# zsc/MOSS-TTSD

Measured on AMD Instinct MI355X. Metric: audio codec tokens/sec/node (decode, bf16, batch 32 @ 4k ctx), higher is better.
Workload: dtype bf16; 1 GPU; configs[2]: batch 32 synthetic dialogues/GPU, 4k-token KV context, top-k/top-p sampling on 8 channels, decode steps at full context; batch_per_gpu=32, context=4096, prompt=512, layers=28, hidden=2048, parallelism=dp1 (batch shard, no per-step collective)

## Files before the change

### include/mtts.h

```cpp
#ifndef MTTS_H
#define MTTS_H

#include <stdint.h>

#ifdef __cplusplus
extern "C" {
#endif

#define MTTS_OK 0
#define MTTS_EINVAL (-1)
#define MTTS_EHIP (-2)
#define MTTS_ENOMEM (-3)
#define MTTS_ESTATE (-4)

#define MTTS_CHANNELS 8

typedef struct MttsConfig {
    int32_t vocab_size;
    int32_t hidden_size;
    int32_t intermediate_size;
    int32_t num_hidden_layers;
    int32_t num_attention_heads;
    int32_t num_key_value_heads;
    int32_t head_dim;
// ... 83 lines not shown
                      const MttsSamplerCfg* sampler, uint64_t seed,
                      int64_t* host_out_ids, int32_t out_capacity, int32_t* out_len,
                      const int64_t* host_forced, int32_t forced_len, int64_t* host_decisions,
                      void* stream);

int32_t mtts_begin(MttsEngine* e, const int64_t* host_input_ids, const uint8_t* host_attention_mask,
                   int32_t B, int32_t T, int32_t max_length,
                   const MttsSamplerCfg* sampler, uint64_t seed, void* stream);
int32_t mtts_step(MttsEngine* e, int32_t n_steps, void* stream);
int32_t mtts_sync_state(MttsEngine* e, int32_t* steps_done, int32_t* all_finished, void* stream);
int32_t mtts_read_generated(MttsEngine* e, int64_t* host_gen, int32_t capacity_steps, int32_t* n_steps);
int32_t mtts_step_begin(MttsEngine* e, float* dev_scores0, float* dev_scores17, void* stream);
int32_t mtts_step_sample(MttsEngine* e, int64_t* dev_tokens, void* stream);
int32_t mtts_step_finish(MttsEngine* e, const uint8_t* host_stop, void* stream);
int32_t mtts_set_output_scores(MttsEngine* e, int32_t on);
int32_t mtts_read_scores(MttsEngine* e, float* host_lp, int32_t capacity_steps, int32_t* n_steps);
int32_t mtts_slot_read_scores(MttsEngine* e, int32_t slot, float* host_rows, int32_t capacity_steps, int32_t* n_steps);
int32_t mtts_set_top_logprobs(MttsEngine* e, int32_t k);
int32_t mtts_read_top_logprobs(MttsEngine* e, float* host_logp, int32_t* host_top_ids, float* host_top_logp,
                               int32_t capacity_steps, int32_t* n_steps);
int32_t mtts_slot_read_top_logprobs(MttsEngine* e, int32_t slot, float* host_logp, int32_t* host_top_ids, float* host_top_logp,
                                    int32_t capacity_steps, int32_t* n_steps);
int32_t mtts_score(MttsEngine* e, const int64_t* host_input_ids, const uint8_t* host_attention_mask,
                   const int64_t* host_labels, int32_t B, int32_t T, float* host_logp, void* stream);
#define MTTS_SCORE_MAX_TOPK 16
#define MTTS_SCORE_TOPK_ROWS 512
int32_t mtts_score_topk(MttsEngine* e, const int64_t* host_input_ids, const uint8_t* host_attention_mask,
                        const int64_t* host_labels, int32_t B, int32_t T, float* host_logp, int32_t k,
                        int32_t* host_top_ids, float* host_top_logp, void* stream);
int32_t mtts_read_logits(MttsEngine* e, uint16_t* host_logits0, uint16_t* host_logits17, void* stream);
int32_t mtts_read_logits_f32(MttsEngine* e, float* host_logits0, float* host_logits17, void* stream);
int32_t mtts_sched_open(MttsEngine* e, int32_t B, int32_t gen_cap, const MttsSamplerCfg* sampler, void* stream);
int32_t mtts_slot_submit(MttsEngine* e, int32_t slot, const int64_t* host_ids, int32_t T, int32_t max_length, uint64_t seed,
                         void* stream);
int32_t mtts_slot_submit_row(MttsEngine* e, int32_t slot, const int64_t* host_ids, int32_t T, int32_t max_length, uint64_t seed,
                             int32_t row_id, void* stream);
int32_t mtts_set_row_ids(MttsEngine* e, const int32_t* host_row_ids, int32_t n);
int32_t mtts_set_takes(MttsEngine* e, int32_t n);
int32_t mtts_set_sampler_floors(MttsEngine* e, const MttsSamplerFloors floors[8] );
int32_t mtts_set_sampler_bans(MttsEngine* e, const MttsSamplerBans bans[8] );
int32_t mtts_set_sampler_typical(MttsEngine* e, const float typical_p[8] );
int64_t mtts_debug_ban_launches(void);
int32_t mtts_set_sampler_bias(MttsEngine* e, const MttsSamplerBias bias[8] );
int64_t mtts_debug_bias_launches(void);
int32_t mtts_slot_fork(MttsEngine* e, int32_t src_slot, int32_t dst_slot, uint64_t seed, int32_t row_id, void* stream);
int32_t mtts_slot_states(MttsEngine* e, int32_t* host_state, void* stream);
int32_t mtts_slot_read(MttsEngine* e, int32_t slot, int64_t* host_rows, int32_t capacity_steps, int32_t* n_steps);
int32_t mtts_read_seq_state(MttsEngine* e, int32_t* host_nas, int32_t* host_unfinished, int32_t* host_kv_len, void* stream);
int32_t mtts_slot_evict(MttsEngine* e, int32_t slot, void* stream);
int32_t mtts_kv_pool_state(MttsEngine* e, int32_t* total_pages, int32_t* free_pages, int32_t* max_pages_per_seq);
int32_t mtts_read_page_table(MttsEngine* e, int32_t* host_table, int32_t* host_n_pages);
int32_t mtts_set_forced_mode(MttsEngine* e, int32_t as_draw);
int32_t mtts_debug_read_device_page_table(MttsEngine* e, int32_t* host_table, void* stream);
int32_t mtts_export_codes(MttsEngine* e, int32_t first, int32_t n, int64_t* dev_codes, void* stream);
int32_t mtts_profile_enable(MttsEngine* e, int32_t on);
int32_t mtts_profile_read(MttsEngine* e, int32_t which, double* total_ms, int64_t* launches, int64_t* bytes);

int32_t mtts_debug_set_kv_len(MttsEngine* e, int32_t kv_len);
int32_t mtts_debug_kv_pack_stats(MttsEngine* e, int64_t* out6);
int32_t mtts_debug_step_plan(MttsEngine* e, int32_t pages_bound, char* buf, int32_t cap);
int32_t mtts_k_attn_bench(MttsEngine* e, int32_t phase, int32_t iters, float* avg_ms, int64_t* bytes_per_launch);
int32_t mtts_k_gemm_bench(int32_t N, int32_t K, int32_t epi, int32_t ksplit, int32_t waves, int32_t copies,
                          int32_t iters, float* avg_us);

int32_t mtts_debug_wseal_stats(MttsEngine* e, int64_t* out12);
int64_t mtts_debug_wseal_launches(void);
int32_t mtts_k_gemm_sealed_bench(const void* dev_w, int32_t N, int32_t K, int32_t epi, int32_t ksplit, int32_t copies,
                                 int32_t iters, int32_t sealed, int32_t head_form, float* avg_us, int64_t* out2);

int32_t mtts_k_wseal(const void* dev_packed, int32_t ntiles, int32_t K, int32_t ktw, void* dev_sealed, void* stream);
int32_t mtts_k_gemm_sealed(const void* dev_w, const void* dev_x, void* dev_out, int32_t M, int32_t N, int32_t K, int32_t epi,
                           int32_t ksplit, int32_t sealed, int32_t head_form, int64_t* out2, void* stream);
int32_t mtts_k_gemm_bf16(const void* dev_w, const void* dev_x, void* dev_y,
                         int32_t M, int32_t N, int32_t K, int32_t ksplit, void* stream);
int64_t mtts_debug_gemm_depth_launches(void);
int64_t mtts_debug_fold_norm_launches(void);
int32_t mtts_k_oproj_resid(const void* dev_wo, const void* dev_attn, void* dev_x, void* dev_x_packed, int32_t R, int32_t N,
                           void* stream);
int32_t mtts_k_fold_pair(const void* dev_wo, const void* dev_attn, void* dev_x, const void* dev_norm_w, const void* dev_wgu,
                         float eps, int32_t R, int32_t N_gu, void* dev_y, void* stream);
int32_t mtts_k_bf16_round_check(int64_t* out2, void* stream);
int32_t mtts_k_fold_bench(int32_t N_gu, int32_t copies, int32_t iters, int32_t mode, float* avg_us);
int64_t mtts_debug_attn_row_launches(void);
int32_t mtts_k_attn_section(const float* dev_slabs, int32_t ksplit, const void* dev_qnw, const void* dev_knw, const void* dev_cos,
                            const void* dev_sin, float eps, const void* dev_k, const void* dev_v, const int32_t* host_lens,
                            const int32_t* host_page_table, int32_t R, int32_t Lmax, int32_t nq, int32_t nkv, int32_t sealed,
                            int32_t path, void* dev_out, void* dev_kcache, void* dev_vcache, void* dev_kpack, void* dev_vpack,
                            void* stream);
int32_t mtts_k_attn_prefill(const float* dev_slabs, int32_t ksplit, const void* dev_qnw, const void* dev_knw, const void* dev_cos,
                            const void* dev_sin, float eps, const void* dev_k, const void* dev_v, const int32_t* host_lens,
                            const int32_t* host_cached, const int32_t* host_page_table, int32_t B, int32_t Lmax, int32_t nq,
                            int32_t nkv, void* dev_out, void* dev_q, void* dev_kcache, void* dev_vcache, void* stream);
int32_t mtts_k_gemm_swiglu_bf16(const void* dev_w, const void* dev_x, void* dev_y,
                                int32_t M, int32_t N, int32_t K, void* stream);
int32_t mtts_k_rmsnorm(const void* dev_x, const void* dev_w, void* dev_y,
                       int32_t rows, int32_t n, float eps, void* stream);
int32_t mtts_k_embed_norm(const int32_t* host_tokens, const int32_t* host_seq, const void* const* host_tables,
                          const int32_t* host_vocab, const void* dev_norm_w, int32_t R, int32_t H, float eps,
                          void* dev_x, void* dev_xn, void* stream);
int32_t mtts_k_resid_norm(const float* dev_slabs, int32_t ksplit, int32_t Npad, void* dev_x, const void* dev_norm_w,
                          const int32_t* host_seq, const int32_t* host_last, int32_t R, int32_t H, int32_t nseq, float eps,
                          void* dev_xn, void* dev_hlast, void* stream);
int32_t mtts_k_gemv_small(int32_t epi, int32_t pro, const void* dev_w, int32_t rows, int32_t N, int32_t K, int32_t want_ksplit,
                          const void* dev_x_in, const float* dev_slabs, int32_t slab_ksplit, const void* dev_norm_w, float eps,
                          void* dev_x_out, const float* dev_opart, const int32_t* host_seq, const int32_t* host_pos, int32_t nq,
                          int32_t nchunks_max, const void* dev_xrows, void* dev_y, int32_t* out_plan, void* stream);
int32_t mtts_k_gemm_tile(int32_t epi, const void* dev_w, const void* dev_x, void* dev_y, int32_t M, int32_t N, int32_t K,
                         int32_t ksplit, void* stream);
int32_t mtts_k_rope_kvwrite(const void* dev_qkv, const int32_t* host_pos, const void* dev_qnorm, const void* dev_knorm,
                            const void* dev_cos, const void* dev_sin, int32_t R, int32_t nq, int32_t nkv, float eps,
                            void* dev_q, void* dev_k, void* dev_v, void* stream);
int32_t mtts_k_paged_attn_decode(const void* dev_q, const void* dev_k, const void* dev_v, const int32_t* host_lens,
                                 const int32_t* host_page_table, int32_t R, int32_t Lmax, int32_t nq, int32_t nkv,
                                 void* dev_out, void* stream);
int32_t mtts_k_kv_seal(const void* dev_pages, int32_t npages, void* dev_sealed, int32_t as_k, void* stream);
int32_t mtts_k_head_ce(const void* dev_w, const void* dev_x, const int32_t* host_labels, int32_t M, int32_t N, int32_t K,
                       int32_t n_valid, int32_t segments, float* dev_logp, void* stream);
int32_t mtts_k_head_topk(const void* dev_w, const void* dev_x, int32_t M, int32_t N, int32_t K, int32_t n_valid,
                         int32_t segments, int32_t k, int32_t* dev_ids, float* dev_logp, void* stream);
int32_t mtts_k_lora_pack(const void* dev_base, int32_t rows, int32_t cols, const float* dev_lora_a, const float* dev_lora_b,
                         int32_t r, float scaling, int32_t rows_pad, int32_t row_mul, int32_t row_off, int32_t dtype,
                         void* dev_out, void* stream);
int32_t mtts_k_lora_delta(const void* dev_x, int32_t R, int32_t K, int32_t Npad, int32_t nseg, const int32_t* host_segs,
                          int32_t n_adapters, const void* const* host_a, const void* const* host_b, const int32_t* host_r,
                          const float* host_scaling, const int32_t* host_row_adapter, float* dev_slabs, int32_t ks, void* stream);
int32_t mtts_k_swiglu_slabs(const void* dev_w, const void* dev_x, const float* dev_delta, void* dev_y, float* dev_slab0_out,
                            int32_t M, int32_t N, int32_t K, void* stream);
int32_t mtts_k_sample(const void* dev_logits_bf16, int32_t rows, int32_t vocab,
                      const void* dev_history_bitmap, const MttsSamplerCfg* cfg,
                      int32_t mask_id, uint64_t seed, int32_t step, int32_t channel,
                      int32_t* dev_tokens, void* stream);
int32_t mtts_k_sample_scores(const void* dev_logits_bf16, int32_t rows, int32_t vocab,
                             const void* dev_history_bitmap, const MttsSamplerCfg* cfg,
                             int32_t mask_id, uint64_t seed, int32_t step, int32_t channel,
                             int32_t* dev_tokens, float* dev_logp, void* stream);
int32_t mtts_k_sample_floors(const void* dev_logits_bf16, int32_t rows, int32_t vocab,
                             const void* dev_history_bitmap, const MttsSamplerCfg* cfg,
                             int32_t mask_id, uint64_t seed, int32_t step, int32_t channel,
                             int32_t* dev_tokens, float* dev_logp, const MttsSamplerFloors* floors, void* stream);
int32_t mtts_k_sample_bans(const void* dev_logits_bf16, int32_t rows, int32_t vocab,
                           const void* dev_history_bitmap, const MttsSamplerCfg* cfg,
                           int32_t mask_id, uint64_t seed, int32_t step, int32_t channel,
                           int32_t* dev_tokens, float* dev_logp, const MttsSamplerFloors* floors, const void* dev_ban,
                           void* stream);
int32_t mtts_k_sample_typical(const void* dev_logits_bf16, int32_t rows, int32_t vocab,
                              const void* dev_history_bitmap, const MttsSamplerCfg* cfg,
                              int32_t mask_id, uint64_t seed, int32_t step, int32_t channel,
                              int32_t* dev_tokens, float* dev_logp, const MttsSamplerFloors* floors, const void* dev_ban,
                              float typical_p, void* stream);
int32_t mtts_k_ngram_ban(const int32_t* dev_hist, const int32_t* dev_lens, int32_t rows, int32_t cap, int32_t n,
                         const int32_t* host_static, int32_t n_static, int32_t vocab, int32_t eos_id, int32_t eos_on,
                         void* dev_ban, void* stream);
int32_t mtts_k_seq_bias(const int32_t* dev_hist, const int32_t* dev_lens, int32_t rows, int32_t cap,
                        const MttsSamplerBias* host_rules, int32_t vocab, void* dev_ban, void* dev_bias_words,
                        MttsBiasTable* dev_bias_tab, void* stream);
int32_t mtts_k_sample_bias(const void* dev_logits_bf16, int32_t rows, int32_t vocab,
                           const void* dev_history_bitmap, const MttsSamplerCfg* cfg,
                           int32_t mask_id, uint64_t seed, int32_t step, int32_t channel,
                           int32_t* dev_tokens, float* dev_logp, const MttsSamplerFloors* floors, const void* dev_ban,
                           float typical_p, const void* dev_bias_words, const MttsBiasTable* dev_bias_tab, void* stream);
int32_t mtts_k_scores_materialize(const void* dev_logits_bf16, int32_t rows, int32_t vocab, const void* dev_history_bitmap,
                                  const MttsSamplerCfg* cfg, int32_t mask_id, int32_t step, int32_t channel, const void* dev_ban,
                                  const void* dev_bias_words, const MttsBiasTable* dev_bias_tab, float* dev_scores, void* stream);
int32_t mtts_k_gen_topk(const void* dev_logits, int32_t is_f32, int32_t rows, int32_t vocab, int32_t mask_id,
                        const int32_t* dev_decisions, int32_t k, float* dev_logp, int32_t* dev_top_ids, float* dev_top_logp,
                        void* stream);

typedef struct MttsCodecConfig {
    int32_t nq, codebook_size, rvq_dim, quant_out_dim;
    int32_t adapter_layers, adapter_dim, adapter_heads, adapter_ffn, adapter_max_pos;
    int32_t up_stride;
    int32_t dec_layers, dec_dim, dec_heads, dec_ffn, dec_max_pos, mel_bins;
    int32_t voc_dim, voc_inter, voc_layers, n_fft, hop;
    int32_t mel_n_fft, mel_hop, mel_frames;
    int32_t enc_layers, enc_dim, enc_heads, enc_ffn, enc_max_pos;
    int32_t sem_adapter_layers, pre_rvq_layers, down_pool;
} MttsCodecConfig;

typedef struct MttsCodec MttsCodec;
const char* mtts_codec_last_error(void);
int32_t mtts_codec_create(const MttsCodecConfig* cfg, int32_t device, MttsCodec** out);
int32_t mtts_codec_destroy(MttsCodec* c);
int32_t mtts_codec_bind(MttsCodec* c, const char* role, const float* dev_f32, int64_t n, void* stream);
int32_t mtts_codec_detokenize(MttsCodec* c, const int64_t* dev_codes, const int32_t* host_lens, int32_t B, int32_t T,
                              float* dev_wav, void* stream);
int32_t mtts_codec_detokenize_async(MttsCodec* c, const int64_t* dev_codes, const int32_t* host_lens, int32_t B, int32_t T,
                                    float* dev_wav, void* stream);
int32_t mtts_codec_check(MttsCodec* c, void* stream);
int32_t mtts_codec_tokenize(MttsCodec* c, const float* dev_wav, const int32_t* host_lens, int32_t B, int32_t nsamp,
                            int64_t* dev_codes, int32_t* host_code_lens, void* stream);
int32_t mtts_k_gemm_f32(const float* dev_a, const float* dev_w, const float* dev_bias, float* dev_c,
                        int32_t M, int32_t N, int32_t K, int32_t act, void* stream);
int32_t mtts_k_gemm_planes_bench(int32_t M, int32_t N, int32_t K, int32_t flags, int32_t tile_code, int32_t iters,
                                 float* avg_us, int32_t* code_used);

int32_t mtts_k_codec_attn(const float* dev_qkv, const int32_t* host_lens, float* dev_att, int32_t B, int32_t T, int32_t heads,
                          int32_t mode, int32_t planes, void* stream);
int32_t mtts_k_codec_gemm_planes(const float* dev_a, const float* dev_w, const float* dev_bias, const float* dev_gamma,
                                 const float* dev_res, float* dev_c, int32_t M, int32_t N, int32_t K, int32_t ldc, int32_t flags,
                                 int32_t tile, int32_t row0, int32_t plane_rows, int32_t nt_out, void* stream);
int32_t mtts_k_codec_vocos_pw(const float* dev_xn, const float* dev_w1, const float* dev_b1, const float* dev_w2,
                              const float* dev_b2, const float* dev_gamma, float* dev_h, int32_t M, void* stream);
int32_t mtts_k_codec_layernorm(const float* dev_x, const float* dev_w, const float* dev_b, float* dev_y, int32_t rows, int32_t C,
                               float eps, const int32_t* host_lens, int32_t T, int32_t ldy, int32_t planes, void* stream);
int32_t mtts_k_codec_layernorm_wide(const float* dev_x, const float* dev_w, const float* dev_b, float* dev_y, int32_t rows,
                                    int32_t C, float eps, void* stream);
int32_t mtts_k_codec_dwconv_ln(const float* dev_h, const float* dev_dw, const float* dev_dwb, const float* dev_lw,
                               const float* dev_lb, float* dev_y, int32_t B, int32_t T, int32_t C, float eps, int32_t kernel,
                               int32_t planes, void* stream);
int32_t mtts_k_codec_softmax_mask(float* dev_s, const int32_t* host_lens, int32_t B, int32_t heads, int32_t T, int32_t ldT,
                                  void* stream);
int32_t mtts_k_codec_vq_argmin_update(const float* dev_dot, const float* dev_cb, const float* dev_cc, float* dev_residual,
                                      int64_t* dev_codes, const int32_t* host_lens, int32_t B, int32_t T, int32_t K, int32_t D,
                                      void* stream);
int32_t mtts_k_codec_gemm_f32_ex(const float* dev_a, const float* dev_w, float* dev_c, const float* dev_bias,
                                 const float* dev_gamma, const float* dev_res, int32_t M, int32_t N, int32_t K, int32_t b_kn,
                                 int64_t lda, int64_t ldw, int64_t ldc, int64_t ldres, int32_t res_rows, int32_t act, float scale,
                                 int32_t batch, int32_t batch_inner, const int64_t* host_strides, void* stream);
// ... 6 lines not shown
```

### moss-ttsd_amd/csrc/attn.hip

```cpp
#include "launch.h"
#include <algorithm>
#include <atomic>
#include <cstdlib>
#ifndef MTTS_PK_WAVES
#define MTTS_PK_WAVES 0
#endif
#if MTTS_PK_WAVES
#define PK_OCC(PK) __attribute__((amdgpu_waves_per_eu((PK) ? MTTS_PK_WAVES : 1, (PK) ? MTTS_PK_WAVES : 8)))
#else
#define PK_OCC(PK)
#endif

#include "seal.h"

__device__ bool seal_lane_k(const u32x4_t* __restrict__ raw, u32x4_t* __restrict__ pk, uint8_t* __restrict__ lds, int lane) {
    u32x4_t v[16];
#pragma unroll
    for (int j = 0; j < 16; ++j) v[j] = raw[j * 64];
    __builtin_amdgcn_wave_barrier();
    uint32_t* row = (uint32_t*)(lds + lane * 128);
#pragma unroll
    for (int j = 0; j < 16; ++j)
#pragma unroll
        for (int c = 0; c < 4; c += 2) {
// ... 60 lines not shown
                cnt += e ? 1u : 0u;
            }
            row[2 * it + h] = sum | (cnt << 16);
        }
    __builtin_amdgcn_wave_barrier();
    int mean;
    {
        const int t = lane, st = (t >> 1) & 1, j = 2 * (t >> 2) + (t & 1);
        uint32_t tot = 0u, cn = 0u;
        for (int d = 0; d < 32; ++d) {
            const uint32_t w = ((const uint32_t*)(lds + (st * 32 + d) * 128))[j];
            tot += w & 0xffffu;
            cn += w >> 16;
        }
        mean = cn ? (int)((tot + cn / 2) / cn) : 0;
    }
    int* means = (int*)(lds + 8192);
    int8_t* sv = (int8_t*)(lds + 8192 + 256);
    means[lane] = mean;
    __builtin_amdgcn_wave_barrier();
    int ref = 255;
    for (int t = 0; t < 64; ++t) { const int m = means[t]; if (m > 0) ref = min(ref, m); }
    const int s_own = mean > 0 ? min((mean - ref) & ~1, 126) : 0;
    sv[lane] = (int8_t)s_own;
    __builtin_amdgcn_wave_barrier();
    bool unfit = false;
#pragma unroll
    for (int it = 0; it < 16; ++it) {
        const int s0 = sv[4 * it + 2 * sub], s1 = sv[4 * it + 2 * sub + 1];
        uint32_t w[4] = {v[it].x, v[it].y, v[it].z, v[it].w};
#pragma unroll
        for (int c = 0; c < 4; ++c) {
            uint32_t out = 0u;
#pragma unroll
            for (int h = 0; h < 2; ++h) {
                uint32_t b = (w[c] >> (16 * h)) & 0xffffu;
                const int sft = h ? s1 : s0;
                const int e = (int)((b >> 7) & 0xffu);
                if (e == 0) {
                    if ((b & 0x7fu) && sft) unfit = true;
                } else {
                    const int e2 = e - sft;
                    if (e == 255 ? sft != 0 : e2 < 1) unfit = true;
                    else b = (b - ((uint32_t)sft << 7)) & 0xffffu;
                }
                out |= b << (16 * h);
            }
            w[c] = out;
        }
        v[it] = u32x4_t{w[0], w[1], w[2], w[3]};
    }
    return seal_encode(v, pk, (uint32_t)s_own & 0xffu, unfit);
}
__device__ __forceinline__ void seal_count(bool fit, unsigned long long* __restrict__ cnt, int layer, int wave, int lane) {
    const bool all = !__any(!fit);
    if (cnt && lane == 0) atomicAdd(cnt + layer * 4 + wave * 2 + (all ? 0 : 1), 1ull);
}

__global__ __launch_bounds__(128) void kv_seal_scan_kernel(const u32x4_t* __restrict__ kcache, const u32x4_t* __restrict__ vcache,
                                                           u32x4_t* __restrict__ kpack, u32x4_t* __restrict__ vpack,
                                                           const int32_t* __restrict__ page_table, const RowMeta* __restrict__ meta, int R,
                                                           int max_pages, int total_pages, size_t raw_layer, size_t pk_layer,
                                                           unsigned long long* __restrict__ cnt) {
    __shared__ __attribute__((aligned(16))) uint8_t klds[8192 + 128];
    __shared__ __attribute__((aligned(16))) uint8_t vlds[8192 + 320];
    const int kvh = blockIdx.y, layer = blockIdx.z, wave = threadIdx.x >> 6, lane = threadIdx.x & 63;
    const int r = blockIdx.x * 64 + lane;
    RowMeta m{-1, 0, 0, 0};
    if (r < R) m = meta[r];
    unsigned long long todo = __ballot(m.seq >= 0 && (m.pos & 63) == 63);
    while (todo) {
        const int i = __ffsll((long long)todo) - 1;
        todo &= todo - 1;
        const int seq = __shfl(m.seq, i, 64), pos = __shfl(m.pos, i, 64);
        const int page = page_table[(size_t)seq * max_pages + (pos >> 6)];
        const size_t pi = (size_t)kvh * total_pages + page;
        const bool fit = wave ? seal_lane_v(vcache + layer * raw_layer + pi * (MTTS_PAGE * MTTS_HD / 8) + lane,
                                            vpack + layer * pk_layer + pi * (MTTS_PKU * 64) + lane, vlds, lane)
                              : seal_lane_k(kcache + layer * raw_layer + pi * (MTTS_PAGE * MTTS_HD / 8) + lane,
                                            kpack + layer * pk_layer + pi * (MTTS_PKU * 64) + lane, klds, lane);
        seal_count(fit, cnt, layer, wave, lane);
    }
}
__global__ __launch_bounds__(128) void kv_seal_all_kernel(const u32x4_t* __restrict__ kcache, const u32x4_t* __restrict__ vcache,
                                                          u32x4_t* __restrict__ kpack, u32x4_t* __restrict__ vpack, int total_pages,
                                                          size_t raw_layer, size_t pk_layer, unsigned long long* __restrict__ cnt) {
    __shared__ __attribute__((aligned(16))) uint8_t klds[8192 + 128];
    __shared__ __attribute__((aligned(16))) uint8_t vlds[8192 + 320];
    const int kvh = blockIdx.y, layer = blockIdx.z, wave = threadIdx.x >> 6, lane = threadIdx.x & 63;
    const size_t pi = (size_t)kvh * total_pages + blockIdx.x;
    const bool fit = wave ? seal_lane_v(vcache + layer * raw_layer + pi * (MTTS_PAGE * MTTS_HD / 8) + lane,
                                        vpack + layer * pk_layer + pi * (MTTS_PKU * 64) + lane, vlds, lane)
                          : seal_lane_k(kcache + layer * raw_layer + pi * (MTTS_PAGE * MTTS_HD / 8) + lane,
                                        kpack + layer * pk_layer + pi * (MTTS_PKU * 64) + lane, klds, lane);
    seal_count(fit, cnt, layer, wave, lane);
}
__global__ __launch_bounds__(64) void kv_seal_pages_kernel(const u32x4_t* __restrict__ raw, u32x4_t* __restrict__ pk, int as_k) {
    __shared__ __attribute__((aligned(16))) uint8_t klds[8192 + 320];
    const u32x4_t* src = raw + (size_t)blockIdx.x * (MTTS_PAGE * MTTS_HD / 8) + threadIdx.x;
    u32x4_t* dst = pk + (size_t)blockIdx.x * (MTTS_PKU * 64) + threadIdx.x;
    if (as_k == 1) seal_lane_k(src, dst, klds, threadIdx.x);
    else if (as_k == 2) seal_lane_v(src, dst, klds, threadIdx.x);
    else seal_lane(src, dst);
}
void launch_kv_seal_pages(const void* raw, void* pk, int npages, int as_k, hipStream_t st) {
    hipLaunchKernelGGL(kv_seal_pages_kernel, dim3(npages), dim3(64), 0, st, (const u32x4_t*)raw, (u32x4_t*)pk, as_k);
}
__global__ __launch_bounds__(64) void kv_pack_count_kernel(const u32x4_t* __restrict__ kpack, const u32x4_t* __restrict__ vpack,
                                                           const int32_t* __restrict__ page_table, const int32_t* __restrict__ complete,
                                                           int max_pages, int total_pages, size_t pk_layer, unsigned long long* __restrict__ out) {
    const int b = blockIdx.x, kvh = blockIdx.y, layer = blockIdx.z, lane = threadIdx.x;
    unsigned long long n = 0, dk = 0, dv = 0;
    for (int pg = 0; pg < complete[b]; ++pg) {
        const size_t pi = (size_t)kvh * total_pages + page_table[(size_t)b * max_pages + pg];
        const u32x4_t fk = kpack[layer * pk_layer + pi * (MTTS_PKU * 64) + 12 * 64 + lane];
        const u32x4_t fv = vpack[layer * pk_layer + pi * (MTTS_PKU * 64) + 12 * 64 + lane];
        n += 1;
        dk += __any(fk.w != 0u) ? 1 : 0;
        dv += __any(fv.w != 0u) ? 1 : 0;
    }
    if (lane == 0 && n) {
        atomicAdd(out + 0, n); atomicAdd(out + 1, dk); atomicAdd(out + 2, n); atomicAdd(out + 3, dv);
    }
}
void launch_kv_pack_count(const void* kpack, const void* vpack, const int32_t* page_table, const int32_t* complete, int B, int max_pages,
                          int total_pages, int nkv, int L, unsigned long long* out, hipStream_t st) {
    const size_t pk_layer = (size_t)total_pages * nkv * (MTTS_PKU * 64);
    hipLaunchKernelGGL(kv_pack_count_kernel, dim3(B, nkv, L), dim3(64), 0, st, (const u32x4_t*)kpack, (const u32x4_t*)vpack, page_table,
                       complete, max_pages, total_pages, pk_layer, out);
}
void launch_kv_seal_rows(const void* kcache, const void* vcache, void* kpack, void* vpack, const int32_t* page_table,
                         const RowMeta* meta, int R, int max_pages, int total_pages, int nkv, int L, unsigned long long* cnt, hipStream_t st) {
    const size_t raw_layer = (size_t)total_pages * nkv * (MTTS_PAGE * MTTS_HD / 8), pk_layer = (size_t)total_pages * nkv * (MTTS_PKU * 64);
    hipLaunchKernelGGL(kv_seal_scan_kernel, dim3((R + 63) / 64, nkv, L), dim3(128), 0, st, (const u32x4_t*)kcache, (const u32x4_t*)vcache,
                       (u32x4_t*)kpack, (u32x4_t*)vpack, page_table, meta, R, max_pages, total_pages, raw_layer, pk_layer, cnt);
}
void launch_kv_seal_all(const void* kcache, const void* vcache, void* kpack, void* vpack, int total_pages, int nkv, int L,
                        unsigned long long* cnt, hipStream_t st) {
    const size_t raw_layer = (size_t)total_pages * nkv * (MTTS_PAGE * MTTS_HD / 8), pk_layer = (size_t)total_pages * nkv * (MTTS_PKU * 64);
    hipLaunchKernelGGL(kv_seal_all_kernel, dim3(total_pages, nkv, L), dim3(128), 0, st, (const u32x4_t*)kcache, (const u32x4_t*)vcache,
                       (u32x4_t*)kpack, (u32x4_t*)vpack, total_pages, raw_layer, pk_layer, cnt);
}


__device__ __forceinline__ void fuse_reduce(const QkvFuse& f, int r, int col, int lane, float& a, float& b) {
    const size_t kstride = (size_t)MTTS_PFCAP * f.Npad;
    const float* p0 = f.partial + (size_t)r * f.Npad + col + lane;
    a = 0.f; b = 0.f;
    for (int k0 = 0; k0 < f.ksplit; k0 += 8) {
        float ta[8], tb[8];
#pragma unroll
        for (int j = 0; j < 8; ++j) {
            const float* pk = p0 + (size_t)min(k0 + j, f.ksplit - 1) * kstride;
            ta[j] = pk[0];
            tb[j] = pk[64];
        }
        if (k0 == 0) { a = ta[0]; b = tb[0]; }
#pragma unroll
        for (int j = 0; j < 8; ++j)
            if (k0 + j < f.ksplit && k0 + j > 0) { a += ta[j]; b += tb[j]; }
    }
    a = rbf(a);
    b = rbf(b);
}

__device__ __forceinline__ void fuse_reduce_request(const QkvFuse& f, int r, int col, int lane, float (&ta)[8], float (&tb)[8]) {
    const size_t kstride = (size_t)MTTS_PFCAP * f.Npad;
    const float* p0 = f.partial + (size_t)r * f.Npad + col + lane;
#pragma unroll
    for (int j = 0; j < 8; ++j) {
        const float* pk = p0 + (size_t)min(j, f.ksplit - 1) * kstride;
        ta[j] = pk[0];
        tb[j] = pk[64];
    }
}
__device__ __forceinline__ void fuse_reduce_sum(const QkvFuse& f, const float (&ta)[8], const float (&tb)[8], float& a, float& b) {
    a = ta[0]; b = tb[0];
#pragma unroll
    for (int j = 1; j < 8; ++j)
        if (j < f.ksplit) { a += ta[j]; b += tb[j]; }
    a = rbf(a);
    b = rbf(b);
}

struct FuseVec { float w0, w1, c, s; };
__device__ __forceinline__ FuseVec fuse_load_vec(const QkvFuse& f, const uint16_t* __restrict__ nw, int pos, int lane) {
    FuseVec v;
    v.w0 = bf2f(nw[lane]);
    v.w1 = bf2f(nw[lane + 64]);
    v.c = bf2f(f.rope_cos[(size_t)pos * 64 + lane]);
    v.s = bf2f(f.rope_sin[(size_t)pos * 64 + lane]);
    return v;
}
__device__ __forceinline__ void fuse_norm_rope(const QkvFuse& f, const FuseVec& v, float a, float b, float& o1, float& o2) {
    const float ss = wave_sum(a * a + b * b);
    const float inv = 1.0f / sqrtf(ss / (float)MTTS_HD + f.eps);
    a = rbf(v.w0 * rbf(a * inv));
    b = rbf(v.w1 * rbf(b * inv));
    o1 = rbf(rbf(a * v.c) + rbf(-b * v.s));
    o2 = rbf(rbf(b * v.c) + rbf(a * v.s));
}

template <int G, bool FUSED, bool PK>
__global__ __launch_bounds__(256) PK_OCC(PK) void attn_scores_kernel(
    const uint16_t* __restrict__ qbuf, u32x4_t* __restrict__ kcache, const int32_t* __restrict__ page_table,
    const RowMeta* __restrict__ meta, uint16_t* __restrict__ scores, float* __restrict__ stats, int max_pages,
    int total_pages, int nq, int nkv, float scale, QkvFuse f, const u32x4_t* __restrict__ kpack) {
    __shared__ __attribute__((aligned(16))) uint32_t qs[G][MTTS_HD / 2];
    __shared__ __attribute__((aligned(16))) uint16_t knew[MTTS_HD];
    __shared__ __attribute__((aligned(16))) uint32_t qw[PK ? 4 : 1][G][MTTS_HD / 2];
    const int r = blockIdx.z, kvh = blockIdx.y;
    const RowMeta m = meta[r];
    if (m.seq < 0) return;
    const int len = m.pos + 1;
    const int npages = (len + MTTS_PAGE - 1) / MTTS_PAGE;
    if ((int)blockIdx.x * 4 >= npages) return;
    const int wave = __builtin_amdgcn_readfirstlane(threadIdx.x >> 6), lane = threadIdx.x & 63;
    const int pg = blockIdx.x * 4 + wave;
// ... 999 lines not shown
```

### moss-ttsd_amd/csrc/engine.h

```cpp
#pragma once
#include <hip/hip_runtime.h>

#include <algorithm>
#include <cstdarg>
#include <cstdio>
#include <cstdlib>
#include <cstring>
#include <memory>
#include <string>
#include <vector>

#include "launch.h"
#include "runstate.h"
#include "stepplan.h"

static_assert(RUN_EINVAL == MTTS_EINVAL, "runstate.h reports with MTTS_EINVAL");

#define MTTS_LOCAL __attribute__((visibility("hidden")))
extern MTTS_LOCAL thread_local char g_err[512];
#define HIPCHK(x)                                                                          \
    do {                                                                                   \
        hipError_t _e = (x);                                                               \
        if (_e != hipSuccess) return fail(MTTS_EHIP, "%s: %s (%s:%d)", #x, hipGetErrorString(_e), __FILE__, __LINE__); \
    } while (0)
// ... 131 lines not shown
    int h16 = 0;
    struct LayerF32 { float *wqkv = nullptr, *wo = nullptr, *wgu = nullptr, *wd = nullptr, *ln_in = nullptr, *ln_post = nullptr, *qn = nullptr, *kn = nullptr; };
    std::vector<LayerF32> lf;
    float* embf[8] = {nullptr};
    const float** d_tables_f = nullptr;
    float* final_norm_f = nullptr;
    float *kcache_f = nullptr, *vcache_f = nullptr;
    float *xf = nullptr, *xnf = nullptr, *qkvf = nullptr, *qbuf_f = nullptr, *attnf = nullptr, *yf = nullptr, *guf = nullptr,
          *actf = nullptr, *hlast_f = nullptr, *scores_f = nullptr;
    SeqState* d_seqs = nullptr;
    RowMeta* d_meta = nullptr;
    LoopState* d_ls = nullptr;
    LoopState* h_ls = nullptr;
    SeqState* h_seqs = nullptr;
    int32_t *d_decisions = nullptr, *d_cur = nullptr, *d_tf = nullptr;
    uint32_t* d_bitmaps = nullptr;
    int bm_words = 0;
    MttsSamplerCfg* d_scfg = nullptr;
    MttsSamplerFloors* d_floors = nullptr;
    int floors_on = 0;
    float* d_typical = nullptr;
    int typical_on = 0;
    BanCfg* d_bancfg = nullptr;
    int bans_on = 0;
    int ban_ngram_on = 0;
    int ban_begin_on = 0;
    int bias_on = 0, bias_terms = 0;
    int hist_on = 0;
    SampleScratch sscr;
    int ch0_sampled = 0;
    int scores_on = 0;
    bool run_open = false;
    int topk_on = 0;
    int32_t* d_sc_labels = nullptr;
    float* d_sc_logp = nullptr;
    size_t sc_cap_rows = 0;
    float* sc_part = nullptr;
    float* sc_logits = nullptr;
    int32_t* d_sc_top_ids = nullptr;
    float* d_sc_top_logp = nullptr;
    size_t sc_top_cap = 0;
    uint32_t* sc_cand = nullptr;
    std::vector<LoraEnt> bank;
    int bank_pairs[MTTS_MAX_ADAPTERS] = {0};
    std::vector<int32_t> seq_adapter = std::vector<int32_t>(MTTS_RCAP, -1);
    int32_t* d_pf_tokens = nullptr;
    RowMeta* d_pf_meta = nullptr;
    size_t pf_cap_rows = 0;
    int B = 0, T = 0, base_length = 0, max_length = 0, max_steps = 0, steps_issued = 0;
    bool continuous = false;
    std::vector<int> join_step;
    std::vector<int> n_real;
    int max_real = 0;
    uint64_t seed = 0;
    bool began = false, has_forced = false;
    int split_phase = 0;
    float *split_scores0 = nullptr, *split_scores17 = nullptr;
    struct DestroyExec { void operator()(hipGraphExec_t g) const { hipGraphExecDestroy(g); } };
    StepGraphs<hipGraphExec_t, DestroyExec> graphs;
    hipStream_t cap_stream = nullptr;
    void *kpack = nullptr, *vpack = nullptr;
    size_t pk_layer_stride = 0;
    unsigned long long *d_seal_cnt = nullptr, *h_seal_cnt = nullptr;
    std::vector<char> pack_k_on, pack_v_on;
    bool prof = false;
    std::vector<std::pair<hipEvent_t, hipEvent_t>> ev[PROF_N];
    int64_t prof_bytes[PROF_N] = {0, 0, 0, 0, 0};
};

static inline bool rows_carry_adapters(const MttsEngine* e) {
    for (int b = 0; b < e->B; ++b)
        if (e->seq_adapter[b] >= 0) return true;
    return false;
}
static inline StepState step_state(const MttsEngine* e, int heads, int R, int pages_bound, bool lora, bool split = false) {
    StepState s;
    s.heads = heads; s.B = e->B; s.R = R; s.pages_bound = pages_bound; s.lora = lora;
    s.forced = e->has_forced; s.ch0_sampled = e->ch0_sampled != 0; s.scores_on = e->scores_on != 0; s.floors_on = e->floors_on != 0; s.typical_on = e->typical_on != 0;
    s.bans_on = e->bans_on != 0; s.bias_on = e->bias_on != 0; s.bias_terms = e->bias_terms != 0;
    s.topk = e->topk_on; s.split = split;
    for (int k = 0; k < WSEAL_KINDS; ++k) s.wseal_on[k] = e->wseal_on[k] != 0;
    if (e->kpack) s.pack_k_on = e->pack_k_on.data();
    if (e->vpack) s.pack_v_on = e->pack_v_on.data();
    return s;
}
static inline StepPlan decode_plan(const MttsEngine* e, int pages_bound, bool split = false) {
    return plan_step(e->knobs, e->caps, step_state(e, 1, round_up(e->B, 32), pages_bound, rows_carry_adapters(e), split));
}

static inline KvPack layer_pack(const MttsEngine* e, const StepPlan& plan, int n) {
    const LayerPlan& l = plan.layers[n];
    return KvPack{l.k_sealed ? (uint8_t*)e->kpack + e->pk_layer_stride * n : nullptr,
                  l.v_sealed ? (uint8_t*)e->vpack + e->pk_layer_stride * n : nullptr};
}
```

### moss-ttsd_amd/csrc/engine.hip

```cpp
#include "engine.h"
#include "staging.h"

#define FLUSH_STEPS 7
#define LINGER_STEPS 14
static inline int linger_bound(int B) { return 6 * B + 8; }

thread_local char g_err[512] = "";
int fail(int code, const char* fmt, ...) {
    va_list ap;
    va_start(ap, fmt);
    vsnprintf(g_err, sizeof(g_err), fmt, ap);
    va_end(ap);
    return code;
}

const char* mtts_last_error(void) { return g_err; }
int32_t mtts_version(void) { return 202; }

static auto ship_on(MttsEngine* e, hipStream_t st) {
    return [e, st](const PageEdits& ed) -> int {
        launch_set_pages(e->d_page_table, ed, st);
        HIPCHK(hipGetLastError());
        return 0;
    };
}

static int create_f32(MttsEngine* e) {
    const size_t H = e->H, I = e->I, D = MTTS_HD;
    e->lf.resize(e->L);
    for (auto& l : e->lf) {
        TRY(e->mem.get(&l.wqkv, (size_t)e->qkv_rows * H, false));
        TRY(e->mem.get(&l.wo, H * e->nq * D, false));
        TRY(e->mem.get(&l.wgu, 2 * I * H, false));
        TRY(e->mem.get(&l.wd, H * I, false));
        TRY(e->mem.get(&l.ln_in, H)); TRY(e->mem.get(&l.ln_post, H)); TRY(e->mem.get(&l.qn, D)); TRY(e->mem.get(&l.kn, D));
    }
    TRY(e->mem.get(&e->embf[0], (size_t)e->V0 * H, false));
    for (int ch = 1; ch < 8; ++ch) TRY(e->mem.get(&e->embf[ch], (size_t)e->Vs * H, false));
    TRY(e->mem.get(&e->final_norm_f, H));
    TRY(e->mem.get(&e->d_tables_f, 8));
    HIPCHK(hipMemcpy((void*)e->d_tables_f, e->embf, 8 * sizeof(void*), hipMemcpyHostToDevice));
    const size_t P = MTTS_PF32CAP;
    TRY(e->mem.get(&e->xf, P * H)); TRY(e->mem.get(&e->xnf, P * H)); TRY(e->mem.get(&e->yf, P * H));
    TRY(e->mem.get(&e->qkvf, P * e->qkv_rows)); TRY(e->mem.get(&e->qbuf_f, P * e->nq * D)); TRY(e->mem.get(&e->attnf, P * e->nq * D));
    TRY(e->mem.get(&e->guf, P * 2 * I)); TRY(e->mem.get(&e->actf, P * I));
    TRY(e->mem.get(&e->hlast_f, (size_t)MTTS_RCAP * H));
    TRY(e->mem.get((float**)&e->logits0, (size_t)MTTS_RCAP * e->V0_pad));
    TRY(e->mem.get((float**)&e->logits17, (size_t)MTTS_RCAP * 7 * e->Vs_pad));
    return 0;
}

static int forward_rows_f32(MttsEngine* e, const int32_t* d_tokens, const RowMeta* d_meta, int R, int heads, hipStream_t st) {
    const int H = e->H, I = e->I, nq = e->nq, nkv = e->nkv;
    const float eps = e->cfg.rms_norm_eps, scale = 1.0f / sqrtf((float)MTTS_HD);
    const int Lmax = e->max_pages * MTTS_PAGE, h16 = e->h16;
    const bool dec = heads == 1;
    launch_f32_embed_norm(d_tokens, d_meta, e->d_tables_f, e->lf[0].ln_in, e->xf, e->xnf, R, H, eps, h16, st);
    for (int n = 0; n < e->L; ++n) {
        auto& l = e->lf[n];
        float* kc = e->kcache_f + e->layer_stride * n;
        float* vc = e->vcache_f + e->layer_stride * n;
        launch_f32_linear(l.wqkv, e->xnf, e->qkvf, R, e->qkv_rows, H, e->qkv_rows, h16, dec, st);
        launch_f32_qkv_post(e->qkvf, e->qkv_rows, d_meta, l.qn, l.kn, e->bufs.rope_cos_f, e->bufs.rope_sin_f, e->qbuf_f, kc, vc,
                            e->d_page_table, e->max_pages, e->total_pages, R, nq, nkv, eps, h16, st);
        launch_f32_attn(e->qbuf_f, kc, vc, e->d_page_table, d_meta, e->scores_f, e->attnf, R, e->max_pages, e->total_pages, nq,
                        nkv, scale, Lmax, h16, st);
        launch_f32_linear(l.wo, e->attnf, e->yf, R, H, nq * MTTS_HD, H, h16, dec, st);
        launch_f32_resid_norm(e->yf, e->xf, l.ln_post, e->xnf, nullptr, d_meta, R, H, eps, h16, st);
        launch_f32_linear(l.wgu, e->xnf, e->guf, R, 2 * I, H, 2 * I, h16, dec, st);
        launch_f32_swiglu(e->guf, e->actf, R, I, h16, st);
        launch_f32_linear(l.wd, e->actf, e->yf, R, H, I, H, h16, dec, st);
        const bool lastl = n == e->L - 1;
        launch_f32_resid_norm(e->yf, e->xf, lastl ? e->final_norm_f : e->lf[n + 1].ln_in, e->xnf, lastl ? e->hlast_f : nullptr,
                              d_meta, R, H, eps, h16, st);
    }
    if (heads) {
        const float* xin = heads == 1 ? e->xnf : e->hlast_f;
        launch_f32_linear(e->embf[0], xin, (float*)e->logits0, e->B, e->V0, H, e->V0_pad, h16, true, st);
        for (int c = 1; c < 8; ++c)
            launch_f32_linear(e->embf[c], xin, (float*)e->logits17 + (size_t)(c - 1) * e->Vs_pad, e->B, e->Vs, H, 7 * e->Vs_pad, h16, true, st);
    }
    HIPCHK(hipGetLastError());
    return MTTS_OK;
// ... 473 lines not shown
    HIPCHK(hipGetLastError());
    HIPCHK(hipMemcpyAsync(e->h_wseal_cnt, e->d_wseal_cnt, WSEAL_KINDS * 2 * sizeof(unsigned long long), hipMemcpyDeviceToHost, nullptr));
    HIPCHK(hipStreamSynchronize(nullptr));
    for (int k = 0; k < WSEAL_KINDS; ++k) {
        const unsigned long long groups = e->h_wseal_cnt[2 * k], bad = e->h_wseal_cnt[2 * k + 1];
        e->wseal_on[k] = e->wseal_ktw[k] && groups && (e->knobs.w_seal == 2 || (double)bad <= WSEAL_MAX_UNSEALED[k] * (double)groups);
    }
    e->wseal_dirty = false;
    return MTTS_OK;
}

int32_t mtts_weights_ready(MttsEngine* e) {
    if (!e) return fail(MTTS_EINVAL, "null engine");
    if (e->emb_bound != 0xff) return fail(MTTS_ESTATE, "embedding tables missing (mask %x)", e->emb_bound);
    if (!e->norm_bound) return fail(MTTS_ESTATE, "final norm missing");
    if (!e->bufs.rope_rows) return fail(MTTS_ESTATE, "rope table missing");
    for (int n = 0; n < e->L; ++n)
        if (e->layers[n].bound != 2047) return fail(MTTS_ESTATE, "layer %d incomplete (mask %x)", n, e->layers[n].bound);
    return wseal_policy(e);
}

static void prof_begin(MttsEngine* e, int which, hipStream_t st, hipEvent_t* a) {
    if (!e->prof) return;
    hipEvent_t s0, s1;
    hipEventCreate(&s0); hipEventCreate(&s1);
    hipEventRecord(s0, st);
    e->ev[which].push_back({s0, s1});
    *a = s1;
}
static void prof_end(MttsEngine* e, hipStream_t st, hipEvent_t a) {
    if (!e->prof) return;
    hipEventRecord(a, st);
}

static int pack_policy_reset(MttsEngine* e, hipStream_t st) {
    if (!e->d_seal_cnt) return 0;
    HIPCHK(hipMemsetAsync(e->d_seal_cnt, 0, (size_t)e->L * 4 * sizeof(unsigned long long), st));
    e->pack_k_on.assign(e->L, 1);
    e->pack_v_on.assign(e->L, 1);
    return 0;
}
static int attend_layer(MttsEngine* e, const StepPlan& plan, int n, const RowMeta* d_meta, int R, int pages_bound, int ks_qkv,
                        hipStream_t st, int64_t kv_tokens_hint) {
    static const AttnPhase decode_ph[3] = {ATTN_SCORES, ATTN_PV, ATTN_COMBINE}, prefill_ph[3] = {ATTN_PF_SCORES, ATTN_PF_PV, ATTN_PF_COMBINE};
    Layer& l = e->layers[n];
    const AttnForm form = plan.layers[n].attn;
    const float eps = e->cfg.rms_norm_eps, scale = 1.0f / sqrtf((float)MTTS_HD);
    uint16_t* kc = (uint16_t*)e->kcache + e->layer_stride * n;
    uint16_t* vc = (uint16_t*)e->vcache + e->layer_stride * n;
    const QkvFuse fz{e->bufs.partial, ks_qkv, e->qkv_rows, (const uint16_t*)l.qn, (const uint16_t*)l.kn, e->bufs.rope_cos, e->bufs.rope_sin, eps};
    const KvPack pk = layer_pack(e, plan, n);
    const KvPack* pkp = (pk.k || pk.v) ? &pk : nullptr;
    if (form == ATTN_FORM_ROW) {
        hipEvent_t ev = nullptr;
        prof_begin(e, PROF_SCORES, st, &ev);
        if (const int rc = launch_attn(e->qbuf, kc, vc, e->d_page_table, d_meta, e->scores, e->stats, e->opart, e->attn_p, R, pages_bound,
                                       e->max_pages, e->total_pages, e->nchunks_max, e->nq, e->nkv, scale, &fz, ATTN_ROW, st, pkp))
            return fail(MTTS_EINVAL, rc == -2 ? "the whole-row attention kernel does not take this launch" : "attention group size not built");
        prof_end(e, st, ev);
        if (e->prof) e->prof_bytes[PROF_SCORES] += 2 * kv_tokens_hint * e->nkv * MTTS_HD * 2;
        return 0;
    }
    const bool fused = form == ATTN_FORM_TWO_PASS_FUSED;
    const AttnPhase* ph = form == ATTN_FORM_PREFILL_MFMA ? prefill_ph : decode_ph;
    const int nphases = plan.path == PATH_SMALL ? 2 : 3;
    if (!fused)
        launch_qkv_post(e->bufs.partial, ks_qkv, e->qkv_rows, d_meta, l.qn, l.kn, e->bufs.rope_cos, e->bufs.rope_sin, e->qbuf,
                        kc, vc, e->d_page_table, e->max_pages, e->total_pages, R, e->nq, e->nkv, eps, st);
    for (int i = 0; i < nphases; ++i) {
        hipEvent_t ev = nullptr;
        if (i < 2) prof_begin(e, i == 0 ? PROF_SCORES : PROF_PV, st, &ev);
        if (launch_attn(e->qbuf, kc, vc, e->d_page_table, d_meta, e->scores, e->stats, e->opart, e->attn_p, R,
                        pages_bound, e->max_pages, e->total_pages, e->nchunks_max, e->nq, e->nkv, scale,
                        fused ? &fz : nullptr, ph[i], st, pkp))
            return fail(MTTS_EINVAL, "attention group size not built");
        if (i < 2) prof_end(e, st, ev);
    }
    if (e->prof) {
        e->prof_bytes[PROF_SCORES] += kv_tokens_hint * e->nkv * MTTS_HD * 2;
        e->prof_bytes[PROF_PV] += kv_tokens_hint * e->nkv * MTTS_HD * 2;
    }
    return 0;
}
static void seal_completed_pages(MttsEngine* e, const RowMeta* d_meta, int R, hipStream_t st) {
    if (e->kpack)
        launch_kv_seal_rows(e->kcache, e->vcache, e->kpack, e->vpack, e->d_page_table, d_meta, R, e->max_pages, e->total_pages, e->nkv, e->L, e->d_seal_cnt, st);
}

static int forward_small(MttsEngine* e, const StepPlan& plan, const RowMeta* d_meta, int pages_bound, hipStream_t st, int64_t kv_tokens_hint) {
    const int H = e->H, I = e->I, nq = e->nq, Hp = round_up(H, 32), R = MTTS_MAXR;
    const float eps = e->cfg.rms_norm_eps;
    uint16_t* xa = (uint16_t*)e->x;
    uint16_t* xb = (uint16_t*)e->x2;
    SmallPro base{};
    base.rows = plan.B; base.eps = eps; base.slab_npad = Hp;
    for (int n = 0; n < e->L; ++n) {
        Layer& l = e->layers[n];
        SmallPro pq = base;
        pq.x_in = xa; pq.x_out = xb; pq.slabs = e->partial2; pq.ksplit = n ? e->p_d.ksplit : 0; pq.norm_w = (const uint16_t*)l.ln_in;
        launch_gemv_small(EPI_PARTIAL, PRO_NORM, e->p_qkv, l.wqkv, H, e->qkv_rows, e->qkv_rows, e->bufs.partial, nullptr, pq, st);
        TRY(attend_layer(e, plan, n, d_meta, R, pages_bound, e->p_qkv.ksplit, st, kv_tokens_hint));
        SmallPro po = base;
        po.opart = e->opart; po.meta = d_meta; po.nchunks_max = e->nchunks_max; po.nq = nq; po.pages_per_chunk = ATT_PB;
        launch_gemv_small(EPI_PARTIAL, PRO_COMBINE, e->p_o, l.wo, nq * MTTS_HD, Hp, Hp, e->partial2, nullptr, po, st);
        SmallPro pg = base;
        pg.x_in = xb; pg.x_out = xa; pg.slabs = e->partial2; pg.ksplit = e->p_o.ksplit; pg.norm_w = (const uint16_t*)l.ln_post;
        launch_gemv_small(EPI_SILU_RM, PRO_NORM, e->p_gu, l.wgu, H, 2 * I, 2 * I, nullptr, (uint16_t*)e->act_rm, pg, st);
        SmallPro pd = base;
        pd.xrows = (const uint16_t*)e->act_rm;
        launch_gemv_small(EPI_PARTIAL, PRO_ROWS, e->p_d, l.wd, I, Hp, Hp, e->partial2, nullptr, pd, st);
    }
    seal_completed_pages(e, d_meta, R, st);
    SmallPro ph = base;
    ph.x_in = xa; ph.x_out = nullptr; ph.slabs = e->partial2; ph.ksplit = e->p_d.ksplit; ph.norm_w = (const uint16_t*)e->final_norm;
    launch_gemv_small(EPI_BF16, PRO_NORM, e->p_h0, e->head0, H, e->V0_pad, e->V0, nullptr, (uint16_t*)e->logits0, ph, st);
    launch_gemv_small(EPI_BF16, PRO_NORM, e->p_h17, e->heads17, H, 7 * e->Vs_pad, 7 * e->Vs_pad, nullptr, (uint16_t*)e->logits17, ph, st);
    HIPCHK(hipGetLastError());
    return MTTS_OK;
}

static int run_gemm(int epi, bool tiled, int R, int ks, bool sealed, int head_form, const GemmPlan& p, const void* Ws, const void* Wp,
                    const void* Xp, int K, int Npad, int n_valid, float* partial, uint16_t* out, hipStream_t st) {
    const int mb = (R + 31) / 32;
    if (tiled) launch_gemm_tile(epi, R, ks, Wp, Xp, K, Npad, n_valid, partial, out, st);
    else if (!sealed) launch_gemm(epi, mb, p, Wp, Xp, K, Npad, n_valid, partial, out, st);
    else if (!launch_gemm_sealed(epi, mb, p, Ws, Wp, Xp, K, Npad, n_valid, partial, out, head_form, st))
        return fail(MTTS_ESTATE, "the plan asks for a sealed weight read that the launcher does not take (K %d, N %d, %d row tiles)", K, Npad, mb);
    return 0;
}

static int forward_rows(MttsEngine* e, const StepPlan& plan, const int32_t* d_tokens, const RowMeta* d_meta, int pages_bound,
                        hipStream_t st, int64_t kv_tokens_hint) {
    const int H = e->H, I = e->I, nq = e->nq, nkv = e->nkv, R = plan.R, mb = plan.mb;
    const float eps = e->cfg.rms_norm_eps;
    const int Hp = round_up(H, 32);
    const bool tiled = plan.tiled, lora = plan.lora;
    if (plan.path == PATH_F32) return forward_rows_f32(e, d_tokens, d_meta, plan.heads == 1 ? plan.B : R, plan.heads, st);
    launch_embed_norm(d_tokens, d_meta, e->d_tables, e->layers[0].ln_in, e->x, e->xn, R, H, eps, st);
    if (plan.path == PATH_SMALL) return forward_small(e, plan, d_meta, pages_bound, st, kv_tokens_hint);
    if (lora && !e->bufs.d_bank) return fail(MTTS_ESTATE, "a pass with adapters on an engine without a bank");
    const int QD = nq * MTTS_HD, KD = nkv * MTTS_HD, EL = e->L * 7;
    const LoraJob j_qkv{3, e->qkv_rows, H, EL, {{0, QD, 1, 0}, {QD, KD, 1, 1}, {QD + KD, KD, 1, 2}}};
    const LoraJob j_o{1, Hp, QD, EL, {{0, H, 1, 3}}}, j_gu{2, 2 * I, H, EL, {{0, I, 2, 4}, {1, I, 2, 5}}}, j_d{1, Hp, I, EL, {{0, H, 1, 6}}};
    const int ks_qkv = tiled ? mtts_tile_ksplit(e->qkv_rows, H, 1024) : e->p_qkv.ksplit;
    const int ks_o = tiled ? mtts_tile_ksplit(Hp, QD, 1024) : e->p_o.ksplit;
    const int ks_d = tiled ? mtts_tile_ksplit(Hp, I, 1024) : e->p_d.ksplit;
    const int ex = lora ? 1 : 0;
    const int gu_epi = lora ? EPI_PARTIAL : EPI_SILU;
    float* gu_slab = lora ? e->bufs.partial : nullptr;
    for (int n = 0; n < e->L; ++n) {
        Layer& l = e->layers[n];
        auto delta = [&](const LoraJob& job, const void* xp, int ks) {
            launch_lora_delta(xp, d_meta, e->bufs.d_seq_adapter, e->bufs.d_bank + (size_t)n * 7, job, e->bufs.partial + (size_t)ks * MTTS_PFCAP * job.Npad, R, st);
        };
        TRY(run_gemm(EPI_PARTIAL, tiled, R, ks_qkv, false, 0, e->p_qkv, nullptr, l.wqkv, e->xn, H, e->qkv_rows, e->qkv_rows, e->bufs.partial, nullptr, st));
        if (lora) delta(j_qkv, e->xn, ks_qkv);
        TRY(attend_layer(e, plan, n, d_meta, R, pages_bound, ks_qkv + ex, st, kv_tokens_hint));
        if (plan.fold) {
            launch_oproj_resid(l.wo, e->attn_p, e->x, e->xres_p, R, Hp, st);
            launch_gateup_norm(l.wgu, e->xres_p, l.ln_post, eps, e->act_p, 2 * I, st);
        } else {
            TRY(run_gemm(EPI_PARTIAL, tiled, R, ks_o, false, 0, e->p_o, nullptr, l.wo, e->attn_p, QD, Hp, Hp, e->bufs.partial, nullptr, st));
            if (lora) delta(j_o, e->attn_p, ks_o);
            launch_resid_norm(e->bufs.partial, ks_o + ex, Hp, e->x, l.ln_post, e->xn, nullptr, d_meta, R, H, eps, st);
            TRY(run_gemm(gu_epi, tiled, R, 1, plan.sealed[WSEAL_GU], 0, e->p_gu, l.wgu_s, l.wgu, e->xn, H, 2 * I, 2 * I, gu_slab, (uint16_t*)e->act_p, st));
        }
        if (lora) {
            delta(j_gu, e->xn, 1);
            launch_swiglu_slabs(e->bufs.partial, e->bufs.partial + (size_t)MTTS_PFCAP * 2 * I, e->act_p, mb * 32, I, st);
        }
        TRY(run_gemm(EPI_PARTIAL, tiled, R, ks_d, plan.sealed[WSEAL_DOWN], 0, e->p_d, l.wd_s, l.wd, e->act_p, I, Hp, Hp, e->bufs.partial, nullptr, st));
        if (lora) delta(j_d, e->act_p, ks_d);
        const bool lastl = (n == e->L - 1);
        const void* nw = lastl ? e->final_norm : e->layers[n + 1].ln_in;
        launch_resid_norm(e->bufs.partial, ks_d + ex, Hp, e->x, nw, e->xn, lastl ? e->hlast : nullptr, d_meta, R, H, eps, st);
    }
    seal_completed_pages(e, d_meta, R, st);
    if (plan.heads) {
        const void* xin = e->xn;
        if (plan.heads == 2) {
            launch_pack_rows(e->hlast, e->xh, plan.B, H, plan.hmb, st);
            xin = e->xh;
        }
        const int hr = plan.hmb * 32, form = plan.head_persistent ? 1 : 0;
        TRY(run_gemm(EPI_BF16, false, hr, 0, plan.sealed[WSEAL_HEAD0], form, e->p_h0, e->head0_s, e->head0, xin, H, e->V0_pad, e->V0, nullptr, (uint16_t*)e->logits0, st));
        TRY(run_gemm(EPI_BF16, false, hr, 0, plan.sealed[WSEAL_HEADS], form, e->p_h17, e->heads17_s, e->heads17, xin, H, 7 * e->Vs_pad, 7 * e->Vs_pad, nullptr, (uint16_t*)e->logits17, st));
    }
    HIPCHK(hipGetLastError());
    return MTTS_OK;
}
static int forward_staged(MttsEngine* e, const int32_t* d_tokens, const RowMeta* d_meta, int R, int pages_bound, int heads, bool lora, hipStream_t st) {
    return forward_rows(e, plan_step(e->knobs, e->caps, step_state(e, heads, R, pages_bound, lora)), d_tokens, d_meta, pages_bound, st, 0);
}

static int prefill_staged(MttsEngine* e, size_t Mpad, int pages_bound, int last_heads, bool lora, hipStream_t st) {
    const size_t pfcap = e->f32 ? MTTS_PF32CAP : MTTS_PFCAP;
    for (size_t off = 0; off < Mpad; off += pfcap) {
        const int rows = (int)std::min<size_t>(pfcap, Mpad - off);
        TRY(forward_staged(e, e->d_pf_tokens + off * 8, e->d_pf_meta + off, rows, pages_bound, off + rows >= Mpad ? last_heads : 0, lora, st));
    }
    return 0;
}

static int start_outputs(MttsEngine* e, int steps, hipStream_t st) {
    StepBufs& b = e->bufs;
    DevBufs& m = e->mem;
    const int k = e->topk_on, rows = e->cfg.max_batch;
    const bool scores = e->scores_on != 0, grown = steps > b.gen_cap, restrided = k && k != b.gt_stride;
    if (grown) b.gen_cap = steps;
    if (restrided) b.gt_stride = k;
    if (scores && !b.sscr_lp) {
        TRY(m.get(&b.sscr_slice_sum, (size_t)rows * SAMP_NS));
        TRY(m.get(&b.sscr_lp, (size_t)rows * 8));
    }
    if (k > b.gt_scr_cap) {
        m.release(b.gt_cand); m.release(b.gt_smax); m.release(b.gt_ssum);
        b.gt_scr_cap = 0;
        TRY(m.get(&b.gt_cand, (size_t)rows * SAMP_NS * k));
        TRY(m.get(&b.gt_smax, (size_t)rows * SAMP_NS));
        TRY(m.get(&b.gt_ssum, (size_t)rows * SAMP_NS));
        b.gt_scr_cap = k;
    }
    const auto store = [&](auto*& p, bool per_k, bool wanted, bool zeroed, bool filled) -> int {
        const size_t n = (size_t)rows * b.gen_cap * 8 * (per_k ? k : 1);
        if (grown || (per_k && restrided)) m.release(p);
        if (wanted && !p) TRY(m.get(&p, n, zeroed));
        if (wanted && filled) HIPCHK(hipMemsetAsync(p, 0xff, n * sizeof(*p), st));
        return 0;
    };
    TRY(store(b.d_gen, false, true, true, false));
    TRY(store(b.d_declog, false, true, true, false));
    TRY(store(b.d_forced, false, true, false, false));
    TRY(store(b.d_lp, false, scores, false, true));
    TRY(store(b.d_gt_logp, false, k > 0, false, true));
    TRY(store(b.d_gt_ids, true, k > 0, false, true));
    TRY(store(b.d_gt_tlp, true, k > 0, false, true));
    return 0;
}

static int start_bans(MttsEngine* e, const RunBans& bans, const RunBias& bias, hipStream_t st) {
    StepBufs& b = e->bufs;
    e->bans_on = (bans.any() || bias.bans()) ? 1 : 0;
    e->ban_ngram_on = bans.ngram() ? 1 : 0;
    e->ban_begin_on = bias.begin() ? 1 : 0;
    e->bias_on = bias.rules() ? 1 : 0;
    e->bias_terms = bias.finite() ? 1 : 0;
    e->hist_on = (e->ban_ngram_on || bias.history()) ? 1 : 0;
    if (!e->bans_on && !e->bias_on) return 0;
    const int rows = e->cfg.max_batch, words = e->bm_words;
    if (e->bans_on && !b.d_ban) {
        TRY(e->mem.get(&b.d_ban, (size_t)rows * 8 * words));
        TRY(e->mem.get(&b.d_ban_static, (size_t)8 * words));
    }
    if (e->ban_begin_on && !b.d_ban_begin) TRY(e->mem.get(&b.d_ban_begin, (size_t)8 * words));
    if (e->bias_on && !b.d_bias_rules) TRY(e->mem.get(&b.d_bias_rules, 8));
    if (e->bias_terms && !b.d_bias_w) {
        TRY(e->mem.get(&b.d_bias_w, (size_t)rows * 8 * words));
        TRY(e->mem.get(&b.d_bias_static, (size_t)8 * words));
        TRY(e->mem.get(&b.d_bias_tab, (size_t)rows * 8));
    }
// ... 212 lines not shown
        TRY(reset_run_state(e, ss, false, sampler, opt.floors, opt.typical, st));
    }
    TRY(prefill_staged(e, sr.Mpad, pages_for(e->max_real), 2, lora, st));
    if (fork.nr) TRY(launch_fork_job(e, fork, false, st));
    e->began = true;
    e->run_open = true;
    return MTTS_OK;
}

int32_t mtts_set_takes(MttsEngine* e, int32_t n) {
    if (!e) return fail(MTTS_EINVAL, "null engine");
    if (n < 1 || n > MTTS_RCAP) return fail(MTTS_EINVAL, "takes must be 1..%d (got %d)", MTTS_RCAP, n);
    e->pending.set_takes(n);
    return MTTS_OK;
}
int32_t mtts_set_sampler_floors(MttsEngine* e, const MttsSamplerFloors* floors) {
    if (!e) return fail(MTTS_EINVAL, "null engine");
    return e->pending.set_floors(floors);
}
int32_t mtts_set_sampler_typical(MttsEngine* e, const float* typical_p) {
    if (!e) return fail(MTTS_EINVAL, "null engine");
    return e->pending.set_typical(typical_p);
}
int32_t mtts_set_sampler_bans(MttsEngine* e, const MttsSamplerBans* bans) {
    if (!e) return fail(MTTS_EINVAL, "null engine");
    return e->pending.set_bans(bans);
}
int32_t mtts_set_sampler_bias(MttsEngine* e, const MttsSamplerBias* bias) {
    if (!e) return fail(MTTS_EINVAL, "null engine");
    return e->pending.set_bias(bias);
}
static int take_options(MttsEngine* e, int B, bool forced, RunOptions* opt) {
    *opt = e->pending.take(B);
    return opt->check(e->cfg.max_batch, forced);
}

int32_t mtts_begin(MttsEngine* e, const int64_t* ids, const uint8_t* mask, int32_t B, int32_t T, int32_t max_length,
                   const MttsSamplerCfg* sampler, uint64_t seed, void* stream) {
    if (!e) return fail(MTTS_EINVAL, "null argument");
    RunOptions opt;
    TRY(take_options(e, B, false, &opt));
    return begin_run(e, ids, mask, B, T, max_length, sampler, seed, opt, stream);
}

static SampleScratch step_front(MttsEngine* e, const StepPlan& plan, hipStream_t st) {
    const StepBufs& b = e->bufs;
    SampleScratch sscr = e->sscr;
    sscr.slice_sum = b.sscr_slice_sum; sscr.lp = b.sscr_lp;
    if (plan.bans_on) {
        launch_ban(b.d_ban, b.d_ban_static, b.d_ban_begin, b.ban_words, e->d_bancfg, b.d_hist, b.hist_cap, b.d_gen, e->V0, e->Vs, e->cfg.eos_token_id,
                   e->d_ls, e->d_seqs, plan.B, st);
        sscr.ban = b.d_ban;
    }
    if (plan.bias_on) {
        launch_bias(plan.bans_on ? b.d_ban : nullptr, plan.bias_terms ? b.d_bias_w : nullptr, b.d_bias_static, plan.bias_terms ? b.d_bias_tab : nullptr,
                    b.ban_words, b.d_bias_rules, b.d_hist, b.hist_cap, b.d_gen, e->V0, e->Vs, e->d_ls, e->d_seqs, plan.B, st);
        if (plan.bias_terms) { sscr.bias_w = b.d_bias_w; sscr.bias_t = b.d_bias_tab; }
    }
    return sscr;
}
static void step_decide(MttsEngine* e, const StepPlan& plan, const SampleScratch& sscr, const void* l0, const void* l17, hipStream_t st) {
    const StepBufs& b = e->bufs;
    launch_sample(l0, l17, e->V0, e->Vs, e->Vs_pad, e->d_bitmaps, e->bm_words, e->d_scfg, e->d_ls,
                  e->d_seqs, e->seed, e->d_decisions, &e->d_ls->error, plan.B, sscr, plan.ch0_sampled,
                  full_cap_for(e->V0), plan.scores_on, (plan.floors_on || plan.typical_on) ? e->d_floors : nullptr,
                  plan.typical_on ? e->d_typical : nullptr, st);
    GenTopkOut gt;
    if (plan.topk) {
        gt = GenTopkOut{plan.topk, b.d_gt_logp, b.d_gt_ids, b.d_gt_tlp};
        launch_gen_topk(e->logits0, e->logits17, e->V0, e->Vs, e->Vs_pad, e->d_scfg, e->d_ls, e->d_seqs, e->d_decisions, plan.B,
                        GenTopkScratch{b.gt_cand, b.gt_smax, b.gt_ssum, b.gt_scr_cap}, gt, st);
    }
    launch_update(e->d_decisions, b.d_declog, plan.forced ? b.d_forced : nullptr, e->d_tf, b.d_gen, e->d_cur,
                  e->d_seqs, e->d_meta, e->d_bitmaps, e->bm_words, e->d_ls, e->cfg.eos_token_id,
                  e->cfg.speech_pad_token, e->cfg.speech_range_lo, e->cfg.speech_range_hi,
                  plan.scores_on ? b.sscr_lp : nullptr, plan.scores_on ? b.d_lp : nullptr, gt, st);
}
static int step_body(MttsEngine* e, const StepPlan& plan, int pages_bound, hipStream_t st, int64_t kvtok) {
    const SampleScratch sscr = step_front(e, plan, st);
    step_decide(e, plan, sscr, e->logits0, e->logits17, st);
    return forward_rows(e, plan, e->d_cur, e->d_meta, pages_bound, st, kvtok);
}

static int step_graph(MttsEngine* e, int pages, hipGraphExec_t* out) {
    StepPlan plan = decode_plan(e, pages);
    if (const hipGraphExec_t* hit = e->graphs.find(plan, pages, e->bufs)) {
        *out = *hit;
        return MTTS_OK;
    }
    if (!e->cap_stream) HIPCHK(hipStreamCreateWithFlags(&e->cap_stream, hipStreamNonBlocking));
    hipGraph_t g = nullptr;
    HIPCHK(hipStreamBeginCapture(e->cap_stream, hipStreamCaptureModeRelaxed));
    int rc = step_body(e, plan, pages, e->cap_stream, 0);
    hipError_t ce = hipStreamEndCapture(e->cap_stream, &g);
    if (rc) { if (g) hipGraphDestroy(g); return rc; }
    HIPCHK(ce);
    hipGraphExec_t exec = nullptr;
    hipError_t ie = hipGraphInstantiate(&exec, g, nullptr, nullptr, 0);
    hipGraphDestroy(g);
    HIPCHK(ie);
    e->graphs.insert(std::move(plan), pages, e->bufs, exec);
    *out = exec;
    return MTTS_OK;
}

static int step_pages(MttsEngine* e, hipStream_t st, int* pages_bound) {
    int len_bound = 1;
    const auto ship = ship_on(e, st);
    for (int b = 0; b < e->B; ++b) {
        if (!e->slot_live[b]) continue;
        const int len = e->n_real[b] + e->steps_issued + 1;
        len_bound = std::max(len_bound, len);
        TRY(e->pool.grow(b, pages_for(len), ship));
    }
    TRY(e->pool.flush(ship));
    *pages_bound = pages_for(len_bound);
    return MTTS_OK;
}

static int issue_steps(MttsEngine* e, int n, hipStream_t st) {
    for (int i = 0; i < n; ++i) {
        if (e->steps_issued >= e->max_steps) break;
        int pages_bound = 0;
        TRY(step_pages(e, st, &pages_bound));
        if (e->knobs.use_graphs && !e->prof) {
            hipGraphExec_t exec = nullptr;
            TRY(step_graph(e, std::min(round_up(pages_bound, ATT_PB), e->max_pages), &exec));
            HIPCHK(hipGraphLaunch(exec, st));
        } else {
            hipEvent_t ev = nullptr;
            prof_begin(e, PROF_STEP, st, &ev);
            int64_t kvtok = 0;
            for (int b = 0; b < e->B; ++b) if (e->slot_live[b]) kvtok += e->n_real[b] + e->steps_issued + 1;
            TRY(step_body(e, decode_plan(e, pages_bound), pages_bound, st, kvtok));
            prof_end(e, st, ev);
        }
        e->steps_issued++;
    }
    return MTTS_OK;
}

int32_t mtts_step(MttsEngine* e, int32_t n_steps, void* stream) {
    if (!e || !e->began) return fail(MTTS_ESTATE, "mtts_begin has not run");
    if (e->split_phase) return fail(MTTS_ESTATE, "mtts_step in the middle of a split step: mtts_step_finish first");
    HIPCHK(hipSetDevice(e->device));
    return issue_steps(e, n_steps, S(stream));
}

static int split_check(MttsEngine* e, const char* who) {
    if (!e || !e->began) return fail(MTTS_ESTATE, "%s: mtts_begin has not run", who);
    if (e->continuous) return fail(MTTS_ESTATE, "%s: the scheduler's steps are not split (mtts_sched_open is running)", who);
    return MTTS_OK;
}
int32_t mtts_step_begin(MttsEngine* e, float* dev_scores0, float* dev_scores17, void* stream) {
    TRY(split_check(e, "mtts_step_begin"));
    if (e->split_phase) return fail(MTTS_ESTATE, "mtts_step_begin: a split step is in flight, mtts_step_finish first");
    if (!dev_scores0 || !dev_scores17 || ((uintptr_t)dev_scores0 & 15) || ((uintptr_t)dev_scores17 & 15))
        return fail(MTTS_EINVAL, "mtts_step_begin: the score buffers are null or not 16-byte aligned");
    if (e->steps_issued >= e->max_steps) return fail(MTTS_ESTATE, "mtts_step_begin: the run has no step left (%d issued)", e->steps_issued);
    HIPCHK(hipSetDevice(e->device));
    hipStream_t st = S(stream);
    const StepPlan plan = decode_plan(e, 1, true);
    const SampleScratch sscr = step_front(e, plan, st);
    launch_scores_materialize(e->logits0, e->logits17, e->V0, e->Vs, e->Vs_pad, e->d_bitmaps, e->bm_words, e->d_scfg, e->d_ls, e->d_seqs,
                              plan.B, sscr, dev_scores0, dev_scores17, st);
    HIPCHK(hipGetLastError());
    e->split_scores0 = dev_scores0; e->split_scores17 = dev_scores17;
    e->split_phase = 1;
    return MTTS_OK;
}
int32_t mtts_step_sample(MttsEngine* e, int64_t* dev_tokens, void* stream) {
    TRY(split_check(e, "mtts_step_sample"));
    if (e->split_phase != 1) return fail(MTTS_ESTATE, "mtts_step_sample: mtts_step_begin has not run for this step");
    HIPCHK(hipSetDevice(e->device));
    hipStream_t st = S(stream);
    const StepPlan plan = decode_plan(e, 1, true);
    SampleScratch sscr = e->sscr;
    sscr.slice_sum = e->bufs.sscr_slice_sum; sscr.lp = e->bufs.sscr_lp;
    sscr.ext = 1;
    step_decide(e, plan, sscr, e->split_scores0, e->split_scores17, st);
    if (dev_tokens) launch_step_tokens(e->d_cur, dev_tokens, e->d_ls, st);
    HIPCHK(hipGetLastError());
    e->split_phase = 2;
    return MTTS_OK;
}
int32_t mtts_step_finish(MttsEngine* e, const uint8_t* host_stop, void* stream) {
    TRY(split_check(e, "mtts_step_finish"));
    if (!e->split_phase) return fail(MTTS_ESTATE, "mtts_step_finish: mtts_step_begin has not run for this step");
    if (e->split_phase == 1) TRY(mtts_step_sample(e, nullptr, stream));
    HIPCHK(hipSetDevice(e->device));
    hipStream_t st = S(stream);
    if (host_stop) {
        StopMask m;
        memset(m.row, 0, sizeof(m.row));
        memcpy(m.row, host_stop, (size_t)e->B);
        launch_stop_rows(m, e->d_seqs, e->d_meta, e->d_ls, st);
    }
    int pages_bound = 0;
    TRY(step_pages(e, st, &pages_bound));
    int64_t kvtok = 0;
    for (int b = 0; b < e->B; ++b) if (e->slot_live[b]) kvtok += e->n_real[b] + e->steps_issued + 1;
    TRY(forward_rows(e, decode_plan(e, pages_bound, true), e->d_cur, e->d_meta, pages_bound, st, kvtok));
    e->steps_issued++;
    e->split_phase = 0;
    return MTTS_OK;
}

int32_t mtts_sync_state(MttsEngine* e, int32_t* steps_done, int32_t* all_finished, void* stream) {
    if (!e || !e->began) return fail(MTTS_ESTATE, "mtts_begin has not run");
    HIPCHK(hipSetDevice(e->device));
    HIPCHK(hipMemcpyAsync(e->h_ls, e->d_ls, sizeof(LoopState), hipMemcpyDeviceToHost, S(stream)));
    if (!e->continuous) HIPCHK(hipMemcpyAsync(e->h_seqs, e->d_seqs, e->B * sizeof(SeqState), hipMemcpyDeviceToHost, S(stream)));
    if (e->d_seal_cnt) HIPCHK(hipMemcpyAsync(e->h_seal_cnt, e->d_seal_cnt, (size_t)e->L * 4 * sizeof(unsigned long long), hipMemcpyDeviceToHost, S(stream)));
    HIPCHK(hipStreamSynchronize(S(stream)));
    if (e->d_seal_cnt && e->knobs.kv_pack == 1) {
        for (int n = 0; n < e->L; ++n) {
            const unsigned long long* c = e->h_seal_cnt + (size_t)n * 4;
            e->pack_k_on[n] = c[0] + c[1] < 16 || c[1] * 8 <= c[0] + c[1];
            e->pack_v_on[n] = c[2] + c[3] < 16 || c[3] * 8 <= c[2] + c[3];
        }
    }
    if (e->h_ls->error) return fail(MTTS_EINVAL, "device sampler error %d: more than 4096 candidate tokens (set top_k so that the k-th score's radix bin holds <= 4096 tokens)", e->h_ls->error);
    if (!e->continuous) {
        const SeqState* ss = e->h_seqs;
        for (int b = 0; b < e->B; ++b)
            if (e->slot_live[b] && ss[b].step > 0 && !ss[b].unfinished && ss[b].active != 2) { e->slot_live[b] = 0; e->pool.release(b); }
    }
    if (steps_done) *steps_done = e->h_ls->step;
    if (all_finished) *all_finished = e->h_ls->done;
    if (e->h_ls->done && !e->continuous) e->run_open = false;
    return MTTS_OK;
}

template <typename Src, typename Dst>
static int read_slots(MttsEngine* e, const Src* d_src, int slot0, int nslots, int steps, Dst* host, int w = 8) {
    std::vector<Src> tmp((size_t)std::max(steps, 1) * w);
    for (int b = 0; b < nslots; ++b) {
        if (steps) HIPCHK(hipMemcpy(tmp.data(), d_src + (size_t)(slot0 + b) * e->bufs.gen_cap * w, (size_t)steps * w * sizeof(Src), hipMemcpyDeviceToHost));
        for (int s = 0; s < steps; ++s)
            for (int c = 0; c < w; ++c) host[((size_t)s * nslots + b) * w + c] = tmp[(size_t)s * w + c];
    }
    return MTTS_OK;
}
template <typename Src, typename Dst>
static int read_rows(MttsEngine* e, const Src* d_src, Dst* host, int capacity_steps, int* n_steps, int w = 8) {
    const int steps = e->h_ls->step;
    if (steps > capacity_steps) return fail(MTTS_EINVAL, "output buffer holds %d steps, need %d", capacity_steps, steps);
    TRY(read_slots(e, d_src, 0, e->B, steps, host, w));
    if (n_steps) *n_steps = steps;
    return MTTS_OK;
}
template <typename Src, typename Dst>
static int slot_read(MttsEngine* e, const Src* d_src, int slot, Dst* host_rows, int capacity_steps, int* n_steps, int w = 8) {
    HIPCHK(hipSetDevice(e->device));
    HIPCHK(hipDeviceSynchronize());
    SeqState cur;
    HIPCHK(hipMemcpy(&cur, e->d_seqs + slot, sizeof(cur), hipMemcpyDeviceToHost));
    if (cur.step > capacity_steps) return fail(MTTS_EINVAL, "buffer holds %d steps, need %d", capacity_steps, cur.step);
    TRY(read_slots(e, d_src, slot, 1, cur.step, host_rows, w));
    if (n_steps) *n_steps = cur.step;
    return MTTS_OK;
}
template <typename T>
static int read_logits(MttsEngine* e, T* l0, T* l17, void* stream) {
    HIPCHK(hipSetDevice(e->device));
    HIPCHK(hipStreamSynchronize(S(stream)));
    if (l0) HIPCHK(hipMemcpy2D(l0, (size_t)e->V0 * sizeof(T), e->logits0, (size_t)e->V0_pad * sizeof(T), (size_t)e->V0 * sizeof(T), e->B, hipMemcpyDeviceToHost));
    if (l17) {
        std::vector<T> tmp((size_t)MTTS_RCAP * 7 * e->Vs_pad);
        HIPCHK(hipMemcpy(tmp.data(), e->logits17, tmp.size() * sizeof(T), hipMemcpyDeviceToHost));
        for (int c = 0; c < 7; ++c)
            for (int b = 0; b < e->B; ++b)
                memcpy(l17 + ((size_t)c * e->B + b) * e->Vs, tmp.data() + ((size_t)b * 7 + c) * e->Vs_pad, (size_t)e->Vs * sizeof(T));
    }
    return MTTS_OK;
}

int32_t mtts_read_generated(MttsEngine* e, int64_t* host_gen, int32_t capacity_steps, int32_t* n_steps) {
    if (!e || !e->began || !host_gen) return fail(MTTS_ESTATE, "nothing generated");
    HIPCHK(hipSetDevice(e->device));
    TRY(mtts_sync_state(e, nullptr, nullptr, nullptr));
    return read_rows(e, e->bufs.d_gen, host_gen, capacity_steps, n_steps);
}

static int run_still_open(MttsEngine* e, bool* open) {
// ... 584 lines not shown
```

### moss-ttsd_amd/csrc/hooks.hip

```cpp
#include "engine.h"
#include "staging.h"

int32_t mtts_k_gemm_bf16(const void* w, const void* x, void* y, int32_t M, int32_t N, int32_t K, int32_t ksplit, void* stream) {
    if (!w || !x || !y || M < 1 || M > MTTS_PFCAP || K % 16 || N < 1) return fail(MTTS_EINVAL, "gemm: need 1<=M<=MTTS_PFCAP, K%%16==0");
    hipStream_t st = S(stream);
    int Npad = round_up(N, 32);
    void *wp = nullptr, *xp = nullptr;
    float* part = nullptr;
    GemmPlan p = mtts_plan_gemm(Npad, K, ksplit);
    p.depth = gemm_depth_env();
    DevBufs hb;
    TRY(hb.get((uint16_t**)&wp, (size_t)Npad * K));
    const bool tiled = M > MTTS_RCAP;
    const int ks = tiled ? (ksplit > 0 ? ksplit : mtts_tile_ksplit(Npad, K, M)) : p.ksplit;
    TRY(hb.get((uint16_t**)&xp, (size_t)MTTS_PFCAP * K));
    TRY(hb.get(&part, (size_t)ks * MTTS_PFCAP * Npad));
    launch_pack_weight(w, wp, N, K, Npad, 1, 0, st);
    const int tiles = (M + 31) / 32;
    launch_pack_rows(x, xp, M, K, tiles == 3 ? 4 : tiles, st);
    if (tiled) launch_gemm_tile(EPI_PARTIAL, M, ks, wp, xp, K, Npad, Npad, part, nullptr, st);
    else launch_gemm(EPI_PARTIAL, tiles, p, wp, xp, K, Npad, Npad, part, nullptr, st);
    launch_reduce_partial_bf16(part, y, ks, Npad, N, M, st);
    HIPCHK(hipGetLastError());
    HIPCHK(hipStreamSynchronize(st));
// ... 259 lines not shown
    if (epi != EPI_PARTIAL && want_ksplit != 1) return fail(MTTS_EINVAL, "gemv_small: only the fp32 slab epilogue takes a split-K");
    if (want_ksplit < 0 || want_ksplit > 16 || want_ksplit > K / 16) return fail(MTTS_EINVAL, "gemv_small: split-K %d outside 0..min(16, K/16)", want_ksplit);
    const int Npad = round_up(N, 32), Kp = round_up(K, 32);
    if (pro == PRO_NORM) {
        if (!dev_x_in || !dev_norm_w || dev_x_in == dev_x_out || slab_ksplit < 0 || slab_ksplit > 16 || (slab_ksplit && !dev_slabs))
            return fail(MTTS_EINVAL, "gemv_small: norm prologue needs x_in != x_out, norm_w, 0<=slab_ksplit<=16 slabs");
    } else if (pro == PRO_COMBINE) {
        if (!dev_opart || !host_seq || !host_pos || nq < 1 || K != nq * MTTS_HD || nchunks_max < 1)
            return fail(MTTS_EINVAL, "gemv_small: combine prologue needs opart, seq, pos, K==nq*128, nchunks_max>=1");
        for (int r = 0; r < rows; ++r) {
            if (host_seq[r] < 0) continue;
            const int npages = host_pos[r] < 0 ? -1 : host_pos[r] / MTTS_PAGE + 1;
            if (npages < 0 || (npages + ATT_PB - 1) / ATT_PB > nchunks_max)
                return fail(MTTS_EINVAL, "gemv_small: row %d: position %d needs more than %d chunks", r, host_pos[r], nchunks_max);
        }
    } else if (!dev_xrows) return fail(MTTS_EINVAL, "gemv_small: rows prologue needs xrows");
    const GemmPlan p0 = mtts_plan_gemm(Npad, K, want_ksplit);
    if (mtts_small_lds_bytes(p0, K, pro) > 64 * 1024 - 33 * 1024)
        return fail(MTTS_EINVAL, "gemv_small: the prologue's %d bytes of LDS exceed the small path's budget", mtts_small_lds_bytes(p0, K, pro));
    hipStream_t st = S(stream);
    uint16_t* wp = nullptr; float *part = nullptr, *slabs = nullptr; RowMeta* meta = nullptr;
    DevBufs hb;
    TRY(hb.get(&wp, (size_t)Npad * K));
    launch_pack_weight(dev_w, wp, N, K, Npad, 1, 0, st);
    SmallPro pr{};
    pr.rows = rows; pr.eps = eps;
    if (pro == PRO_NORM) {
        if (slab_ksplit) TRY(stage_slabs(hb, dev_slabs, slab_ksplit, rows, Kp, &slabs, st));
        pr.x_in = (const uint16_t*)dev_x_in; pr.x_out = (uint16_t*)dev_x_out; pr.slabs = slabs; pr.ksplit = slab_ksplit; pr.slab_npad = Kp;
        pr.norm_w = (const uint16_t*)dev_norm_w;
    } else if (pro == PRO_COMBINE) {
        TRY(hb.get(&meta, SMALL_RP));
        std::vector<RowMeta> hm(SMALL_RP, RowMeta{-1, 0, 0, 0});
        for (int r = 0; r < rows; ++r)
            if (host_seq[r] >= 0) hm[r] = RowMeta{host_seq[r], host_pos[r], 1, 0};
        HIPCHK(hipMemcpyAsync(meta, hm.data(), hm.size() * sizeof(RowMeta), hipMemcpyHostToDevice, st));
        pr.opart = dev_opart; pr.meta = meta; pr.nchunks_max = nchunks_max; pr.nq = nq; pr.pages_per_chunk = ATT_PB;
    } else pr.xrows = (const uint16_t*)dev_xrows;
    if (epi == EPI_PARTIAL) {
        TRY(hb.get(&part, (size_t)p0.ksplit * MTTS_PFCAP * Npad, false));
        for (int k = 0; k < p0.ksplit; ++k) HIPCHK(hipMemsetAsync(part + (size_t)k * MTTS_PFCAP * Npad, 0xff, (size_t)SMALL_RP * Npad * 4, st));
    }
    launch_gemv_small(epi, pro, p0, wp, K, Npad, N, part, epi == EPI_PARTIAL ? nullptr : (uint16_t*)dev_y, pr, st);
    if (epi == EPI_PARTIAL) launch_reduce_partial_bf16(part, dev_y, p0.ksplit, Npad, N, rows, st);
    HIPCHK(hipGetLastError());
    HIPCHK(hipStreamSynchronize(st));
    if (out_plan) { out_plan[0] = std::max(p0.waves, 4); out_plan[1] = p0.ksplit; }
    return MTTS_OK;
}

int32_t mtts_k_gemm_tile(int32_t epi, const void* dev_w, const void* dev_x, void* dev_y, int32_t M, int32_t N, int32_t K,
                         int32_t ksplit, void* stream) {
    if ((epi != EPI_PARTIAL && epi != EPI_SILU) || !dev_w || !dev_x || !dev_y || M < 1 || M > MTTS_PFCAP || N < 1 || K < 16 || K % 16)
        return fail(MTTS_EINVAL, "gemm_tile: need epi 0 or 2, 1<=M<=MTTS_PFCAP, N>=1, K%%16==0");
    if (epi == EPI_SILU && (N % 32 || ksplit < 0 || ksplit > 1)) return fail(MTTS_EINVAL, "gemm_tile: the SwiGLU epilogue needs N%%32==0 and no split-K");
    if (ksplit < 0 || ksplit > 16 || ksplit > K / 16) return fail(MTTS_EINVAL, "gemm_tile: split-K %d outside 0..min(16, K/16)", ksplit);
    hipStream_t st = S(stream);
    const int Npad = round_up(N, 32), tiles = (M + 31) / 32;
    const int ks = epi == EPI_SILU ? 1 : (ksplit > 0 ? ksplit : mtts_tile_ksplit(Npad, K, M));
    uint16_t *wp = nullptr, *xp = nullptr, *op = nullptr;
    float* part = nullptr;
    DevBufs hb;
    TRY(hb.get(&wp, (size_t)Npad * K));
    TRY(hb.get(&xp, (size_t)tiles * 32 * K));
    launch_pack_weight(dev_w, wp, N, K, Npad, 1, 0, st);
    launch_pack_rows(dev_x, xp, M, K, tiles, st);
    if (epi == EPI_PARTIAL) {
        TRY(hb.get(&part, (size_t)ks * MTTS_PFCAP * Npad));
        launch_gemm_tile(EPI_PARTIAL, M, ks, wp, xp, K, Npad, Npad, part, nullptr, st);
        launch_reduce_partial_bf16(part, dev_y, ks, Npad, N, M, st);
    } else {
        TRY(hb.get(&op, (size_t)tiles * 32 * (N / 2)));
        launch_gemm_tile(EPI_SILU, M, 1, wp, xp, K, N, N, nullptr, op, st);
        launch_unpack_rows(op, dev_y, M, N / 2, st);
    }
    HIPCHK(hipGetLastError());
    HIPCHK(hipStreamSynchronize(st));
    return MTTS_OK;
}

static int k_sample(const void* logits, int32_t rows, int32_t vocab, const void* bitmap, const MttsSamplerCfg* cfg,
                    int32_t mask_id, uint64_t seed, int32_t step, int32_t channel, int32_t* dev_tokens, float* dev_logp,
                    const MttsSamplerFloors* floors, const void* ban, float typical_p, void* stream, const void* bias_w = nullptr,
                    const MttsBiasTable* bias_t = nullptr) {
    if ((bias_w == nullptr) != (bias_t == nullptr)) return fail(MTTS_EINVAL, "sample: bias words and bias tables come together");
    if (!logits || !cfg || !dev_tokens || rows < 1 || vocab < 1 || channel < 0 || channel > 7) return fail(MTTS_EINVAL, "sample: bad argument");
    hipStream_t st = S(stream);
    MttsSamplerCfg h[8];
    for (int i = 0; i < 8; ++i) h[i] = *cfg;
    MttsSamplerCfg* d = nullptr;
    int32_t *err = nullptr, *dec = nullptr;
    if (rows > MTTS_RCAP) return fail(MTTS_EINVAL, "sample: at most 128 rows");
    DevBufs hb;
    TRY(hb.get(&d, 8));
    TRY(hb.get(&err, 1));
    TRY(hb.get(&dec, (size_t)rows * 8));
    HIPCHK(hipMemcpy(d, h, sizeof(h), hipMemcpyHostToDevice));
    MttsSamplerFloors* dfl = nullptr;
    if (floors) {
        MttsSamplerFloors hf[8];
        for (int i = 0; i < 8; ++i) hf[i] = *floors;
        PendingRun chk;
        TRY(chk.set_floors(hf));
        if (cfg->do_sample && (floors->min_p > 0.f || floors->epsilon_cutoff > 0.f || floors->eta_cutoff > 0.f)) {
            TRY(hb.get(&dfl, 8));
            HIPCHK(hipMemcpy(dfl, hf, sizeof(hf), hipMemcpyHostToDevice));
        }
    }
    float* dty = nullptr;
    {
        float ht[8];
        for (int i = 0; i < 8; ++i) ht[i] = typical_p;
        PendingRun chk;
        TRY(chk.set_typical(ht));
        if (cfg->do_sample && typical_p > 0.f && typical_p < 1.f) {
            TRY(hb.get(&dty, 8));
            HIPCHK(hipMemcpy(dty, ht, sizeof(ht), hipMemcpyHostToDevice));
        }
    }
    SampleScratch sc;
    TRY(alloc_scratch(hb, sc, rows, vocab));
    sc.ban = (const uint32_t*)ban;
    sc.bias_w = (const uint32_t*)bias_w; sc.bias_t = bias_t;
    if (dev_logp) {
        TRY(hb.get(&sc.slice_sum, (size_t)rows * SAMP_NS));
        TRY(hb.get(&sc.lp, (size_t)rows * 8));
    }
    launch_sample_single(logits, rows, vocab, (const uint32_t*)bitmap, (vocab + 31) / 32, d, mask_id, seed, step, channel, dec, err, sc,
                         full_cap_for(vocab), dev_logp ? 1 : 0, dfl, dty, st);
    HIPCHK(hipGetLastError());
    HIPCHK(hipStreamSynchronize(st));
    std::vector<int32_t> hd((size_t)rows * 8);
    int32_t herr = 0;
    HIPCHK(hipMemcpy(hd.data(), dec, hd.size() * 4, hipMemcpyDeviceToHost));
    HIPCHK(hipMemcpy(&herr, err, 4, hipMemcpyDeviceToHost));
    std::vector<int32_t> outv(rows);
    for (int r = 0; r < rows; ++r) outv[r] = hd[(size_t)r * 8 + channel];
    HIPCHK(hipMemcpy(dev_tokens, outv.data(), rows * 4, hipMemcpyHostToDevice));
    if (dev_logp) {
        std::vector<float> hl((size_t)rows * 8), outl(rows);
        HIPCHK(hipMemcpy(hl.data(), sc.lp, hl.size() * 4, hipMemcpyDeviceToHost));
        for (int r = 0; r < rows; ++r) outl[r] = hl[(size_t)r * 8 + channel];
        HIPCHK(hipMemcpy(dev_logp, outl.data(), rows * 4, hipMemcpyHostToDevice));
    }
    if (herr) return fail(MTTS_EINVAL, "sample: more than 4096 candidate tokens");
    return MTTS_OK;
}

int32_t mtts_k_sample(const void* logits, int32_t rows, int32_t vocab, const void* bitmap, const MttsSamplerCfg* cfg,
                      int32_t mask_id, uint64_t seed, int32_t step, int32_t channel, int32_t* dev_tokens, void* stream) {
    return k_sample(logits, rows, vocab, bitmap, cfg, mask_id, seed, step, channel, dev_tokens, nullptr, nullptr, nullptr, 0.f, stream);
}

int32_t mtts_k_sample_scores(const void* logits, int32_t rows, int32_t vocab, const void* bitmap, const MttsSamplerCfg* cfg,
                             int32_t mask_id, uint64_t seed, int32_t step, int32_t channel, int32_t* dev_tokens, float* dev_logp,
                             void* stream) {
    if (!dev_logp) return fail(MTTS_EINVAL, "sample: null dev_logp");
    return k_sample(logits, rows, vocab, bitmap, cfg, mask_id, seed, step, channel, dev_tokens, dev_logp, nullptr, nullptr, 0.f, stream);
}

int32_t mtts_k_sample_floors(const void* logits, int32_t rows, int32_t vocab, const void* bitmap, const MttsSamplerCfg* cfg,
                             int32_t mask_id, uint64_t seed, int32_t step, int32_t channel, int32_t* dev_tokens, float* dev_logp,
                             const MttsSamplerFloors* floors, void* stream) {
    return k_sample(logits, rows, vocab, bitmap, cfg, mask_id, seed, step, channel, dev_tokens, dev_logp, floors, nullptr, 0.f, stream);
}

int32_t mtts_k_sample_bans(const void* logits, int32_t rows, int32_t vocab, const void* bitmap, const MttsSamplerCfg* cfg,
                           int32_t mask_id, uint64_t seed, int32_t step, int32_t channel, int32_t* dev_tokens, float* dev_logp,
                           const MttsSamplerFloors* floors, const void* dev_ban, void* stream) {
    return k_sample(logits, rows, vocab, bitmap, cfg, mask_id, seed, step, channel, dev_tokens, dev_logp, floors, dev_ban, 0.f, stream);
}

int32_t mtts_k_sample_typical(const void* logits, int32_t rows, int32_t vocab, const void* bitmap, const MttsSamplerCfg* cfg,
                              int32_t mask_id, uint64_t seed, int32_t step, int32_t channel, int32_t* dev_tokens, float* dev_logp,
                              const MttsSamplerFloors* floors, const void* dev_ban, float typical_p, void* stream) {
    return k_sample(logits, rows, vocab, bitmap, cfg, mask_id, seed, step, channel, dev_tokens, dev_logp, floors, dev_ban, typical_p, stream);
}

int32_t mtts_k_sample_bias(const void* logits, int32_t rows, int32_t vocab, const void* bitmap, const MttsSamplerCfg* cfg,
                           int32_t mask_id, uint64_t seed, int32_t step, int32_t channel, int32_t* dev_tokens, float* dev_logp,
                           const MttsSamplerFloors* floors, const void* dev_ban, float typical_p, const void* dev_bias_words,
                           const MttsBiasTable* dev_bias_tab, void* stream) {
    return k_sample(logits, rows, vocab, bitmap, cfg, mask_id, seed, step, channel, dev_tokens, dev_logp, floors, dev_ban, typical_p, stream,
                    dev_bias_words, dev_bias_tab);
}

int32_t mtts_k_scores_materialize(const void* logits, int32_t rows, int32_t vocab, const void* bitmap, const MttsSamplerCfg* cfg,
                                  int32_t mask_id, int32_t step, int32_t channel, const void* dev_ban, const void* dev_bias_words,
                                  const MttsBiasTable* dev_bias_tab, float* dev_scores, void* stream) {
    if (!logits || !cfg || !dev_scores || rows < 1 || rows > MTTS_RCAP || vocab < 1 || channel < 0 || channel > 7 || mask_id >= vocab)
        return fail(MTTS_EINVAL, "scores_materialize: bad argument");
    if ((dev_bias_words == nullptr) != (dev_bias_tab == nullptr)) return fail(MTTS_EINVAL, "scores_materialize: bias words and bias tables come together");
    if ((uintptr_t)dev_scores & 15) return fail(MTTS_EINVAL, "scores_materialize: dev_scores is not 16-byte aligned");
    hipStream_t st = S(stream);
    MttsSamplerCfg h[8];
    for (int i = 0; i < 8; ++i) h[i] = *cfg;
    DevBufs hb;
    MttsSamplerCfg* d = nullptr;
    TRY(hb.get(&d, 8));
    HIPCHK(hipMemcpy(d, h, sizeof(h), hipMemcpyHostToDevice));
    SampleScratch sc;
    sc.ban = (const uint32_t*)dev_ban;
    sc.bias_w = (const uint32_t*)dev_bias_words; sc.bias_t = dev_bias_tab;
    launch_scores_materialize_single(logits, rows, vocab, (const uint32_t*)bitmap, (vocab + 31) / 32, d, mask_id, step, channel, sc, dev_scores, st);
    HIPCHK(hipGetLastError());
    HIPCHK(hipStreamSynchronize(st));
    return MTTS_OK;
}

int32_t mtts_k_ngram_ban(const int32_t* dev_hist, const int32_t* dev_lens, int32_t rows, int32_t cap, int32_t n,
                         const int32_t* host_static, int32_t n_static, int32_t vocab, int32_t eos_id, int32_t eos_on,
                         void* dev_ban, void* stream) {
    if (!dev_lens || !dev_ban || rows < 1 || rows > MTTS_RCAP || cap < 0 || (cap > 0 && !dev_hist) || vocab < 1 || n_static < 0 ||
        (n_static > 0 && !host_static))
        return fail(MTTS_EINVAL, "ngram_ban: bad argument");
    MttsSamplerBans hbans[8];
    for (int i = 0; i < 8; ++i) hbans[i] = MttsSamplerBans{n, 0, n_static, host_static};
    PendingRun chk;
    TRY(chk.set_bans(hbans));
    hipStream_t st = S(stream);
    HIPCHK(hipStreamSynchronize(st));
    std::vector<int32_t> lens(rows);
    HIPCHK(hipMemcpy(lens.data(), dev_lens, (size_t)rows * 4, hipMemcpyDeviceToHost));
    for (int r = 0; r < rows; ++r)
        if (lens[r] < 0 || lens[r] > cap) return fail(MTTS_EINVAL, "ngram_ban: row %d has length %d, the histories hold %d", r, lens[r], cap);
    const int words = (vocab + 31) / 32;
    std::vector<uint32_t> stat(words);
    stage_ban_static(host_static, n_static, vocab, words, stat.data());
    const BanCfg hc{n, eos_on ? 1 : 0};
    DevBufs hb;
    BanCfg* dc = nullptr;
    uint32_t* ds = nullptr;
    TRY(hb.get(&dc, 1));
    TRY(hb.get(&ds, (size_t)words));
    HIPCHK(hipMemcpy(dc, &hc, sizeof(hc), hipMemcpyHostToDevice));
    HIPCHK(hipMemcpy(ds, stat.data(), stat.size() * 4, hipMemcpyHostToDevice));
    launch_ban_single((uint32_t*)dev_ban, ds, dc, dev_hist, dev_lens, rows, cap, vocab, eos_id, st);
    HIPCHK(hipGetLastError());
    HIPCHK(hipStreamSynchronize(st));
    return MTTS_OK;
}
// ... 143 lines not shown
    }
    const float scale = 1.0f / sqrtf((float)MTTS_HD);
    if (launch_attn(dev_q, kc, vc, pt, meta, scores, stats, opart, outp, MTTS_MAXR, pages_bound, max_pages, total_pages, nch, nq, nkv,
                    scale, nullptr, ATTN_ALL, st, pk.k ? &pk : nullptr))
        return fail(MTTS_EINVAL, "attention group size not built (1, 2, 4)");
    launch_unpack_rows(outp, dev_out, R, nq * MTTS_HD, st);
    HIPCHK(hipGetLastError());
    HIPCHK(hipStreamSynchronize(st));
    return MTTS_OK;
}

int32_t mtts_k_attn_section(const float* dev_slabs, int32_t ksplit, const void* dev_qnw, const void* dev_knw, const void* dev_cos,
                            const void* dev_sin, float eps, const void* dev_k, const void* dev_v, const int32_t* host_lens,
                            const int32_t* host_page_table, int32_t R, int32_t Lmax, int32_t nq, int32_t nkv, int32_t sealed,
                            int32_t path, void* dev_out, void* dev_kcache, void* dev_vcache, void* dev_kpack, void* dev_vpack,
                            void* stream) {
    if (!dev_slabs || !dev_qnw || !dev_knw || !dev_cos || !dev_sin || !dev_k || !dev_v || !host_lens || !dev_out || !dev_kcache ||
        !dev_vcache || R < 1 || R > MTTS_MAXR || Lmax < 1 || nq < 1 || nkv < 1 || nq % nkv || ksplit < 1 || (path != 0 && path != 1))
        return fail(MTTS_EINVAL, "attn_section: bad argument (1..32 rows, path 0 or 1)");
    hipStream_t st = S(stream);
    const int max_pages = pages_for(Lmax), total_pages = R * max_pages, nch = (max_pages + ATT_PB - 1) / ATT_PB;
    const int Npad = (nq + 2 * nkv) * MTTS_HD;
    std::vector<int32_t> hpt((size_t)R * max_pages);
    std::vector<char> seen(total_pages, 0);
    for (size_t i = 0; i < hpt.size(); ++i) {
        hpt[i] = host_page_table ? host_page_table[i] : (int32_t)i;
        if (hpt[i] < 0 || hpt[i] >= total_pages || seen[hpt[i]]) return fail(MTTS_EINVAL, "page table must be a permutation of 0..%d", total_pages - 1);
        seen[hpt[i]] = 1;
    }
    std::vector<RowMeta> hm(MTTS_MAXR, RowMeta{-1, 0, 0, 0});
    std::vector<int32_t> cached(R, 0);
    int pages_bound = 1;
    for (int r = 0; r < R; ++r) {
        if (host_lens[r] < 0 || host_lens[r] > Lmax) return fail(MTTS_EINVAL, "row %d: length %d outside 0..%d", r, host_lens[r], Lmax);
        if (!host_lens[r]) continue;
        hm[r] = RowMeta{r, host_lens[r] - 1, 1, 0};
        cached[r] = host_lens[r] - 1;
        pages_bound = std::max(pages_bound, pages_for(host_lens[r]));
    }
    pages_bound = std::min(round_up(pages_bound, ATT_PB), max_pages);
    RowMeta* meta = nullptr; int32_t *pt = nullptr, *lens = nullptr; uint16_t *kc = nullptr, *vc = nullptr, *scores = nullptr, *outp = nullptr;
    float *stats = nullptr, *opart = nullptr, *slabs = nullptr;
    uint8_t *kp = nullptr, *vp = nullptr;
    const size_t cache_n = (size_t)total_pages * nkv * MTTS_PAGE * MTTS_HD, pk_n = (size_t)total_pages * nkv * MTTS_PKU * 64 * 16;
    DevBufs hb;
    TRY(hb.get(&meta, MTTS_MAXR)); TRY(hb.get(&pt, hpt.size())); TRY(hb.get(&lens, R));
    TRY(hb.get(&kc, cache_n)); TRY(hb.get(&vc, cache_n));
    TRY(hb.get(&scores, (size_t)MTTS_MAXR * nq * max_pages * MTTS_PAGE));
    TRY(hb.get(&stats, (size_t)MTTS_MAXR * nq * max_pages * 2));
    TRY(hb.get(&opart, (size_t)MTTS_MAXR * nq * nch * MTTS_HD));
    TRY(hb.get(&outp, (size_t)MTTS_MAXR * nq * MTTS_HD));
    TRY(hb.get(&slabs, (size_t)ksplit * MTTS_PFCAP * Npad, false));
    HIPCHK(hipMemcpyAsync(meta, hm.data(), hm.size() * sizeof(RowMeta), hipMemcpyHostToDevice, st));
    HIPCHK(hipMemcpyAsync(pt, hpt.data(), hpt.size() * 4, hipMemcpyHostToDevice, st));
    HIPCHK(hipMemcpyAsync(lens, cached.data(), R * 4, hipMemcpyHostToDevice, st));
    for (int k = 0; k < ksplit; ++k)
        HIPCHK(hipMemcpyAsync(slabs + (size_t)k * MTTS_PFCAP * Npad, dev_slabs + (size_t)k * R * Npad, (size_t)R * Npad * 4, hipMemcpyDeviceToDevice, st));
    launch_pack_kv_pages(dev_k, dev_v, kc, vc, pt, lens, R, Lmax, nkv, max_pages, total_pages, st);
    KvPack pk{nullptr, nullptr};
    if (sealed) {
        TRY(hb.get(&kp, pk_n)); TRY(hb.get(&vp, pk_n));
        launch_kv_seal_all(kc, vc, kp, vp, total_pages, nkv, 1, nullptr, st);
        pk = KvPack{kp, vp};
    }
    const QkvFuse fz{slabs, ksplit, Npad, (const uint16_t*)dev_qnw, (const uint16_t*)dev_knw, (const uint16_t*)dev_cos, (const uint16_t*)dev_sin, eps};
    const float scale = 1.0f / sqrtf((float)MTTS_HD);
    if (path == 1) {
        if (attn_row_prepare()) return fail(MTTS_EINVAL, "attn_row_kernel: the dynamic LDS limit could not be raised");
        if (!attn_row_fits(nq / nkv, &fz, sealed ? &pk : nullptr, pages_bound)) return fail(MTTS_EINVAL, "attn_section: the whole-row kernel does not take this shape");
    }
    if (const int rc = launch_attn(nullptr, kc, vc, pt, meta, scores, stats, opart, outp, MTTS_MAXR, pages_bound, max_pages, total_pages, nch,
                                   nq, nkv, scale, &fz, path == 1 ? ATTN_ROW : ATTN_ALL, st, sealed ? &pk : nullptr))
        return fail(MTTS_EINVAL, rc == -2 ? "attn_section: the whole-row kernel does not take this shape" : "attention group size not built (1, 2, 4)");
    HIPCHK(hipGetLastError());
    HIPCHK(hipMemcpyAsync(dev_out, outp, (size_t)MTTS_MAXR * nq * MTTS_HD * 2, hipMemcpyDeviceToDevice, st));
    HIPCHK(hipMemcpyAsync(dev_kcache, kc, cache_n * 2, hipMemcpyDeviceToDevice, st));
    HIPCHK(hipMemcpyAsync(dev_vcache, vc, cache_n * 2, hipMemcpyDeviceToDevice, st));
    if (sealed && dev_kpack) HIPCHK(hipMemcpyAsync(dev_kpack, kp, pk_n, hipMemcpyDeviceToDevice, st));
    if (sealed && dev_vpack) HIPCHK(hipMemcpyAsync(dev_vpack, vp, pk_n, hipMemcpyDeviceToDevice, st));
    HIPCHK(hipStreamSynchronize(st));
    return MTTS_OK;
}
int64_t mtts_debug_attn_row_launches(void) { return (int64_t)mtts_attn_row_launches(); }

int32_t mtts_k_attn_prefill(const float* dev_slabs, int32_t ksplit, const void* dev_qnw, const void* dev_knw, const void* dev_cos,
                            const void* dev_sin, float eps, const void* dev_k, const void* dev_v, const int32_t* host_lens,
                            const int32_t* host_cached, const int32_t* host_page_table, int32_t B, int32_t Lmax, int32_t nq,
                            int32_t nkv, void* dev_out, void* dev_q, void* dev_kcache, void* dev_vcache, void* stream) {
    if (!dev_slabs || !dev_qnw || !dev_knw || !dev_cos || !dev_sin || !dev_k || !dev_v || !host_lens || !host_cached || !dev_out ||
        !dev_q || !dev_kcache || !dev_vcache || B < 1 || B > MTTS_RCAP || Lmax < 1 || nq < 1 || nkv < 1 || nq % nkv || ksplit < 1 || ksplit > 8)
        return fail(MTTS_EINVAL, "attn_prefill: bad argument (1..%d dialogues, nq %% nkv == 0, 1 <= ksplit <= 8)", MTTS_RCAP);
    if (const int G = nq / nkv; G != 1 && G != 2 && G != 4) return fail(MTTS_EINVAL, "attention group size not built (1, 2, 4)");
    const int max_pages = pages_for(Lmax), total_pages = B * max_pages, nch = (max_pages + ATT_PB - 1) / ATT_PB;
    const int nch_pf = (max_pages + ATT_PF - 1) / ATT_PF, Npad = (nq + 2 * nkv) * MTTS_HD;
    int64_t M = 0;
    int pages_bound = 1;
    for (int b = 0; b < B; ++b) {
        const int n = host_lens[b], c = host_cached[b];
        if (c < 0 || c % MTTS_MAXR || c >= n || n > Lmax)
            return fail(MTTS_EINVAL, "attn_prefill: dialogue %d: need cached %% 32 == 0 and 0 <= cached (%d) < lens (%d) <= Lmax (%d)", b, c, n, Lmax);
        M += round_up(n - c, MTTS_MAXR);
        pages_bound = std::max(pages_bound, pages_for(n));
    }
    if (M > MTTS_PFCAP) return fail(MTTS_EINVAL, "attn_prefill: %lld staged rows, a pass holds %d", (long long)M, MTTS_PFCAP);
    std::vector<int32_t> hpt((size_t)total_pages);
    std::vector<char> seen(total_pages, 0);
    for (size_t i = 0; i < hpt.size(); ++i) {
        hpt[i] = host_page_table ? host_page_table[i] : (int32_t)i;
        if (hpt[i] < 0 || hpt[i] >= total_pages || seen[hpt[i]]) return fail(MTTS_EINVAL, "page table must be a permutation of 0..%d", total_pages - 1);
        seen[hpt[i]] = 1;
    }
    const int R = round_up((int)M, MTTS_RCAP);
    std::vector<RowMeta> hm(R, RowMeta{-1, 0, 0, 0});
    {
        int r = 0;
        for (int b = 0; b < B; r = round_up(r, MTTS_MAXR), ++b)
            for (int i = host_cached[b]; i < host_lens[b]; ++i, ++r) hm[r] = RowMeta{b, i, i == host_lens[b] - 1 ? 1 : 0, 0};
    }
    hipStream_t st = S(stream);
    RowMeta* meta = nullptr; int32_t *pt = nullptr, *lens = nullptr; uint16_t *kc = nullptr, *vc = nullptr, *qbuf = nullptr, *scores = nullptr, *outp = nullptr;
    float *stats = nullptr, *opart = nullptr, *slabs = nullptr;
    const size_t cache_n = (size_t)total_pages * nkv * MTTS_PAGE * MTTS_HD;
    const size_t q_n = (size_t)R * nq * MTTS_HD, sc_n = (size_t)R * nq * max_pages * MTTS_PAGE, st_n = (size_t)R * nq * max_pages * 2;
    const size_t op_n = (size_t)R * nq * nch_pf * MTTS_HD, sl_n = (size_t)ksplit * MTTS_PFCAP * Npad;
    DevBufs hb;
    TRY(hb.get(&meta, (size_t)R, false)); TRY(hb.get(&pt, hpt.size(), false)); TRY(hb.get(&lens, (size_t)B, false));
    TRY(hb.get(&kc, cache_n)); TRY(hb.get(&vc, cache_n));
    TRY(hb.get(&qbuf, q_n, false)); TRY(hb.get(&scores, sc_n, false)); TRY(hb.get(&stats, st_n, false)); TRY(hb.get(&opart, op_n, false));
    TRY(hb.get(&outp, q_n, false)); TRY(hb.get(&slabs, sl_n, false));
    HIPCHK(hipMemsetAsync(qbuf, 0xff, q_n * 2, st)); HIPCHK(hipMemsetAsync(scores, 0xff, sc_n * 2, st));
    HIPCHK(hipMemsetAsync(stats, 0xff, st_n * 4, st)); HIPCHK(hipMemsetAsync(opart, 0xff, op_n * 4, st));
    HIPCHK(hipMemsetAsync(outp, 0xff, q_n * 2, st)); HIPCHK(hipMemsetAsync(slabs, 0xff, sl_n * 4, st));
    std::vector<int32_t> full(B, Lmax);
    HIPCHK(hipMemcpyAsync(meta, hm.data(), hm.size() * sizeof(RowMeta), hipMemcpyHostToDevice, st));
    HIPCHK(hipMemcpyAsync(pt, hpt.data(), hpt.size() * 4, hipMemcpyHostToDevice, st));
    HIPCHK(hipMemcpyAsync(lens, full.data(), (size_t)B * 4, hipMemcpyHostToDevice, st));
    for (int k = 0; k < ksplit; ++k)
        HIPCHK(hipMemcpyAsync(slabs + (size_t)k * MTTS_PFCAP * Npad, dev_slabs + (size_t)k * M * Npad, (size_t)M * Npad * 4, hipMemcpyDeviceToDevice, st));
    launch_pack_kv_pages(dev_k, dev_v, kc, vc, pt, lens, B, Lmax, nkv, max_pages, total_pages, st);
    const float scale = 1.0f / sqrtf((float)MTTS_HD);
    launch_qkv_post(slabs, ksplit, Npad, meta, dev_qnw, dev_knw, dev_cos, dev_sin, qbuf, kc, vc, pt, max_pages, total_pages, R, nq, nkv, eps, st);
    static const AttnPhase prefill_ph[3] = {ATTN_PF_SCORES, ATTN_PF_PV, ATTN_PF_COMBINE};
    for (int i = 0; i < 3; ++i)
        if (launch_attn(qbuf, kc, vc, pt, meta, scores, stats, opart, outp, R, pages_bound, max_pages, total_pages, nch, nq, nkv, scale,
                        nullptr, prefill_ph[i], st, nullptr))
            return fail(MTTS_EINVAL, "attention group size not built (1, 2, 4)");
    launch_unpack_rows(outp, dev_out, (int)M, nq * MTTS_HD, st);
    HIPCHK(hipGetLastError());
    HIPCHK(hipMemcpyAsync(dev_q, qbuf, (size_t)M * nq * MTTS_HD * 2, hipMemcpyDeviceToDevice, st));
    HIPCHK(hipMemcpyAsync(dev_kcache, kc, cache_n * 2, hipMemcpyDeviceToDevice, st));
    HIPCHK(hipMemcpyAsync(dev_vcache, vc, cache_n * 2, hipMemcpyDeviceToDevice, st));
    HIPCHK(hipStreamSynchronize(st));
    return MTTS_OK;
}

int32_t mtts_k_kv_seal(const void* dev_pages, int32_t npages, void* dev_sealed, int32_t as_k, void* stream) {
    if (!dev_pages || !dev_sealed || npages < 1) return fail(MTTS_EINVAL, "kv_seal: bad argument");
    launch_kv_seal_pages(dev_pages, dev_sealed, npages, as_k, S(stream));
    HIPCHK(hipGetLastError());
    HIPCHK(hipStreamSynchronize(S(stream)));
    return MTTS_OK;
}

int32_t mtts_debug_kv_pack_stats(MttsEngine* e, int64_t* out6) {
    if (!e || !out6) return fail(MTTS_EINVAL, "null argument");
    if (!e->kpack) return fail(MTTS_ESTATE, "the engine keeps no sealed pages (fp32 / fp16 engine, or MTTS_KV_PACK=0)");
// ... 384 lines not shown
```

### moss-ttsd_amd/csrc/launch.h

```cpp
#pragma once
#include <type_traits>

#include "../../include/mtts.h"
#include "common.h"
#include "kvpool.h"

enum { EPI_PARTIAL = 0, EPI_BF16 = 1, EPI_SILU = 2,
       EPI_SILU_RM = 3 };
struct GemmPlan {
    int waves, ksplit, kt_per_split, kt_per_wave;
    int depth;
};
GemmPlan mtts_plan_gemm(int Npad, int K, int want_ksplit);
GemmPlan mtts_plan_gemm_forced(int Npad, int K, int ksplit, int waves);
void launch_gemm(int epi, int mb, const GemmPlan& p, const void* Wp, const void* Xp, int K, int Npad, int n_valid,
                 float* partial, uint16_t* out, hipStream_t st);
int mtts_gemm_form(int epi, int mb, const GemmPlan& p, int K, int Npad, int n_valid);
int mtts_tile_ksplit(int Npad, int K, int R);
void launch_gemm_tile(int epi, int R, int ksplit, const void* Wp, const void* Xp, int K, int Npad, int n_valid,
                      float* partial, uint16_t* out, hipStream_t st);
int mtts_small_lds_bytes(const GemmPlan& p, int K, int pro);
void launch_gemv_small(int epi, int pro, const GemmPlan& p, const void* Wp, int K, int Npad, int n_valid, float* partial,
                       uint16_t* out, const SmallPro& pr, hipStream_t st);
long long mtts_gemm_depth_launches();
void mtts_gemm_depth_note();
void launch_pack_weight(const void* src, void* dst, int rows, int cols, int rows_pad, int row_mul, int row_off, hipStream_t st);
void launch_pack_rows(const void* src, void* dst, int R, int K, int tiles, hipStream_t st);
void launch_reduce_partial_bf16(const float* partial, void* out, int ksplit, int Npad, int n_valid, int R, hipStream_t st);

bool wseal_shape(const GemmPlan& p, int K, int Npad, int epi);
size_t wseal_bytes(int Npad, int K, int ktw);
void launch_wseal(const void* Wp, void* Ws, int K, int ktw, int nt0, int ntiles, hipStream_t st);
void launch_wseal_count(const void* Ws, int Npad, int K, int ktw, unsigned long long* out2, hipStream_t st);
bool launch_gemm_sealed(int epi, int mb, const GemmPlan& p, const void* Ws, const void* Wp, const void* Xp, int K, int Npad,
                        int n_valid, float* partial, uint16_t* out, int head_form, hipStream_t st);
long long mtts_wseal_launches();

bool fold_norm_shape(const GemmPlan& p_o, int K_o, const GemmPlan& p_gu, int H, int N_gu);
void launch_oproj_resid(const void* Wp, const void* Xp, void* x, void* x_packed, int R, int N, hipStream_t st);
void launch_gateup_norm(const void* Wp, const void* x_packed, const void* norm_w, float eps, void* out, int Npad, hipStream_t st);
long long mtts_fold_norm_launches();

void launch_embed_norm(const int32_t* tokens, const RowMeta* meta, const uint16_t* const* tables, const void* norm_w,
                       void* x, void* xn_packed, int R, int H, float eps, hipStream_t st);
void launch_resid_norm(const float* partial, int ksplit, int Npad, void* x, const void* norm_w, void* xn_packed,
                       void* hlast, const RowMeta* meta, int R, int H, float eps, hipStream_t st);
void launch_qkv_post(const float* partial, int ksplit, int Npad, const RowMeta* meta, const void* qnw, const void* knw,
                     const void* cosb, const void* sinb, void* qbuf, void* kcache, void* vcache,
                     const int32_t* page_table, int max_pages, int total_pages, int R, int nq, int nkv, float eps,
                     hipStream_t st);
void launch_rmsnorm_rows(const void* x, const void* w, void* y, int rows, int n, float eps, hipStream_t st);
void launch_fill_random_bf16(void* p, size_t n, uint32_t seed, hipStream_t st);
void launch_set_pages(int32_t* table, const PageEdits& ed, hipStream_t st);
void launch_fork(void* kc, void* vc, size_t layer_bytes, size_t head_bytes, int blk_bytes, int L, int nkv, const ForkJob& job,
                 hipStream_t st);
void launch_pack_kv_pages(const void* K, const void* V, void* kcache, void* vcache, const int32_t* page_table, const int32_t* lens,
                          int S, int Lmax, int nkv, int max_pages, int total_pages, hipStream_t st);
void launch_bf16_to_f32(const void* a, float* b, size_t n, hipStream_t st);
void launch_unpack_rows(const void* packed, void* out, int R, int K, hipStream_t st);
void launch_bf16_round_check(unsigned long long* cnt2, hipStream_t st);

enum AttnPhase { ATTN_ALL = 0, ATTN_SCORES = 1, ATTN_PV = 2, ATTN_COMBINE = 3,
                 ATTN_ROW = 4,
                 ATTN_PF_SCORES = 11, ATTN_PF_PV = 12, ATTN_PF_COMBINE = 13 };
int launch_attn(const void* qbuf, void* kcache, void* vcache, const int32_t* page_table,
                const RowMeta* meta, void* scores, float* stats, float* opart, void* out_packed, int R,
                int pages_bound, int max_pages, int total_pages, int nchunks_max, int nq, int nkv, float scale,
                const QkvFuse* fuse, AttnPhase phase, hipStream_t st, const KvPack* pack = nullptr);
bool attn_row_fits(int G, const QkvFuse* fuse, const KvPack* pack, int pages_bound);
int attn_row_prepare();
int attn_row_lds_limit();
long long mtts_attn_row_launches();
void launch_kv_seal_rows(const void* kcache, const void* vcache, void* kpack, void* vpack, const int32_t* page_table,
                         const RowMeta* meta, int R, int max_pages, int total_pages, int nkv, int L, unsigned long long* cnt, hipStream_t st);
void launch_kv_seal_all(const void* kcache, const void* vcache, void* kpack, void* vpack, int total_pages, int nkv, int L,
                        unsigned long long* cnt, hipStream_t st);
void launch_kv_seal_pages(const void* raw, void* pk, int npages, int as_k, hipStream_t st);
void launch_kv_pack_count(const void* kpack, const void* vpack, const int32_t* page_table, const int32_t* complete, int B, int max_pages,
                          int total_pages, int nkv, int L, unsigned long long* out, hipStream_t st);

struct SeqState {
    int32_t nas;
    int32_t unfinished;
    int32_t kv_len;
    int32_t step;
    int32_t base_length;
    int32_t max_length;
    int32_t row_id;
    int32_t active;
    uint64_t seed;
};

struct LoopState {
    int32_t step;
    int32_t done;
    int32_t continuous;
    int32_t B;
    int32_t error;
    int32_t gen_cap;
    int32_t forced_draw;
    int32_t logits_f32;
};
static_assert(sizeof(SeqState) == 40 && std::is_trivially_copyable<SeqState>::value, "SeqState layout");
static_assert(sizeof(LoopState) == 32 && std::is_trivially_copyable<LoopState>::value, "LoopState layout");

#define SAMP_CAND 4096
#define SAMP_NS 32
struct SampleScratch {
    uint32_t* hist = nullptr;
    float* slice_val = nullptr;
    int32_t* slice_idx = nullptr;
    float* cand_val = nullptr;
    int32_t* cand_idx = nullptr;
    uint32_t* cand_n = nullptr;
    int32_t* overflow = nullptr;
    float* full_val = nullptr;
    int32_t* full_idx = nullptr;
    uint32_t* nuc_cnt = nullptr;
    unsigned long long* nuc_mass = nullptr;
    float* slice_sum = nullptr;
    float* lp = nullptr;
    const uint32_t* ban = nullptr;
    const uint32_t* bias_w = nullptr;
    const MttsBiasTable* bias_t = nullptr;
    int ext = 0;
};
void launch_sample(const void* logits0, const void* logits17, int V0, int Vs, int Vs_pad, const uint32_t* bitmaps,
                   int bm_words, const MttsSamplerCfg* cfgs, const LoopState* ls, const SeqState* seqs, uint64_t seed,
                   int32_t* decisions, int32_t* err, int B, const SampleScratch& sc, int ch0_sampled, int full_cap,
                   int emit_lp, const MttsSamplerFloors* floors ,
                   const float* typical , hipStream_t st);
void launch_sample_single(const void* logits, int rows, int vocab, const uint32_t* bitmap, int bm_words,
                          const MttsSamplerCfg* cfgs8, int mask_id, uint64_t seed, int step, int channel,
                          int32_t* decisions, int32_t* err, const SampleScratch& sc, int full_cap, int emit_lp,
                          const MttsSamplerFloors* floors8, const float* typical8, hipStream_t st);
struct BanCfg { int32_t ngram, eos_below, min_length; };
void launch_ban(uint32_t* ban, const uint32_t* stat, const uint32_t* begin, int words, const BanCfg* cfgs, const int32_t* hist, int hist_cap,
                const int32_t* gen, int V0, int Vs, int eos, const LoopState* ls, const SeqState* seqs, int B, hipStream_t st);
void launch_ban_single(uint32_t* ban, const uint32_t* stat, const BanCfg* cfg1, const int32_t* hist, const int32_t* lens, int rows,
                       int cap, int vocab, int eos, hipStream_t st);
long long mtts_ban_launches();
void launch_bias(uint32_t* ban, uint32_t* bias_w, const uint32_t* bias_stat, MttsBiasTable* tabs, int words, const BiasRules* rules,
                 const int32_t* hist, int hist_cap, const int32_t* gen, int V0, int Vs, const LoopState* ls, const SeqState* seqs,
                 int B, hipStream_t st);
void launch_bias_single(uint32_t* ban, uint32_t* bias_w, const uint32_t* bias_stat, MttsBiasTable* tabs, const BiasRules* rules1,
                        const int32_t* hist, const int32_t* lens, int rows, int cap, int vocab, hipStream_t st);
long long mtts_bias_launches();
struct GenTopkOut {
    int32_t k = 0;
    float* logp = nullptr;
    int32_t* ids = nullptr;
    float* tlp = nullptr;
};
void launch_update(const int32_t* decisions, int32_t* dec_log, const int32_t* forced, const int32_t* tf_tail,
                   int32_t* gen, int32_t* cur_tokens, SeqState* seqs, RowMeta* meta, uint32_t* bitmaps, int bm_words,
                   LoopState* ls, int eos, int spad, int sp_lo, int sp_hi, const float* lp_in, float* lp_out,
// ... 72 lines not shown
```

### moss-ttsd_amd/csrc/sampler.hip

```cpp
#include "launch.h"
#include "sample_ctx.h"

__device__ __forceinline__ void philox4x32_10(uint32_t c0, uint32_t c1, uint32_t c2, uint32_t c3, uint32_t k0,
                                              uint32_t k1, uint32_t* out) {
#pragma unroll
    for (int i = 0; i < 10; ++i) {
        uint64_t p0 = (uint64_t)0xD2511F53u * c0;
        uint64_t p1 = (uint64_t)0xCD9E8D57u * c2;
        uint32_t n0 = (uint32_t)(p1 >> 32) ^ c1 ^ k0;
        uint32_t n1 = (uint32_t)p1;
        uint32_t n2 = (uint32_t)(p0 >> 32) ^ c3 ^ k1;
        uint32_t n3 = (uint32_t)p0;
        c0 = n0; c1 = n1; c2 = n2; c3 = n3;
        k0 += 0x9E3779B9u;
        k1 += 0xBB67AE85u;
    }
    out[0] = c0; out[1] = c1; out[2] = c2; out[3] = c3;
}

__device__ __forceinline__ uint32_t fkey(float f) {
    uint32_t u = __float_as_uint(f);
    return (u & 0x80000000u) ? ~u : (u | 0x80000000u);
}

__device__ __forceinline__ float bias_term(const MttsBiasTable* __restrict__ t, int i) {
    int lo = 0, hi = min(t->n, MTTS_BIAS_RULES_MAX);
    while (lo < hi) {
        const int mid = (lo + hi) >> 1;
        if (t->ids[mid] < i) lo = mid + 1; else hi = mid;
    }
    return (lo < MTTS_BIAS_RULES_MAX && lo < t->n && t->ids[lo] == i) ? t->term[lo] : 0.f;
}
__device__ __forceinline__ float proc_score(const SampleCtx& x, int i) {
    if (i == x.mask_id) return -INFINITY;
    if (x.ban && (x.ban[i >> 5] >> (i & 31)) & 1u) return -INFINITY;
    float s = x.lg.f32 ? ((const float*)x.lg.p)[i] : bf2f(((const uint16_t*)x.lg.p)[i]);
    if (x.bias_w && (x.bias_w[i >> 5] >> (i & 31)) & 1u) s = s + bias_term(x.bias_t, i);
    if (x.penalty > 0.f && (x.bm[i >> 5] >> (i & 31)) & 1u) s = (s < 0.f) ? s * x.penalty : s / x.penalty;
    if (x.temp > 0.f) s = s / x.temp;
    return s;
}

#define SAMP_T 256

__device__ __forceinline__ void argmax_merge(float& bv, int& bi, float ov, int oi) {
    if (ov > bv || (ov == bv && oi < bi)) { bv = ov; bi = oi; }
}

__device__ __forceinline__ void block_argmax(float& bv, int& bi, float* shf, int* shi) {
#pragma unroll
    for (int o = 32; o > 0; o >>= 1) argmax_merge(bv, bi, __shfl_xor(bv, o, 64), __shfl_xor(bi, o, 64));
    const int wid = threadIdx.x >> 6, nw = blockDim.x >> 6;
    __syncthreads();
    if ((threadIdx.x & 63) == 0) { shf[wid] = bv; shi[wid] = bi; }
    __syncthreads();
    bv = shf[0]; bi = shi[0];
    for (int w = 1; w < nw; ++w) argmax_merge(bv, bi, shf[w], shi[w]);
    __syncthreads();
}

template <int NT>
__device__ __forceinline__ double block_excl_scan(double v, double* sh, double& total) {
    const int lane = threadIdx.x & 63, wid = threadIdx.x >> 6;
    double inc = v;
#pragma unroll
    for (int o = 1; o < 64; o <<= 1) {
        double t = __shfl_up(inc, o, 64);
        if (lane >= o) inc += t;
    }
    __syncthreads();
    if (lane == 63) sh[wid] = inc;
    __syncthreads();
    double base = 0.0, tot = 0.0;
    for (int w = 0; w < NT / 64; ++w) { if (w < wid) base += sh[w]; tot += sh[w]; }
    total = tot;
    __syncthreads();
    return base + inc - v;
}

template <bool LP>
__global__ __launch_bounds__(SAMP_T) void sample_scan_kernel(
    const uint16_t* __restrict__ logits0, int V0, const uint32_t* __restrict__ bitmaps, int bm_words,
    const MttsSamplerCfg* __restrict__ cfgs, const LoopState* __restrict__ ls, const SeqState* __restrict__ seqs,
    SampleScratch sc, int single_vocab,
    int single_mask, int single_step, int single_channel) {
    __shared__ uint32_t hist[2048];
    __shared__ float shf[SAMP_T / 64];
    __shared__ int shi[SAMP_T / 64];
    __shared__ double shd[SAMP_T / 64];
    const int b = blockIdx.y, slice = blockIdx.x, tid = threadIdx.x;
    SampleCtx x;
    if (!sample_ctx(x, b, 0, logits0, nullptr, V0, 0, 0, bitmaps, bm_words, cfgs, ls, seqs, single_vocab, single_mask,
                    single_step, single_channel, sc.ban, sc.bias_w, sc.bias_t, sc.ext)) return;
    const MttsSamplerCfg cfg = cfgs[x.c];
    const bool want_hist = cfg.do_sample && cfg.top_k > 0 && cfg.top_k < x.V;
    for (int i = tid; i < 2048; i += SAMP_T) hist[i] = 0;
    __syncthreads();
    const int per = (x.V + SAMP_NS - 1) / SAMP_NS;
    const int i0 = slice * per, i1 = min(x.V, i0 + per);
    float bv = -INFINITY;
    int bi = 0x7fffffff;
    for (int i = i0 + tid; i < i1; i += SAMP_T) {
        float s = proc_score(x, i);
        argmax_merge(bv, bi, s, i);
        if (want_hist) atomicAdd(&hist[fkey(s) >> 21], 1u);
    }
    block_argmax(bv, bi, shf, shi);
    if (tid == 0) { sc.slice_val[b * SAMP_NS + slice] = bv; sc.slice_idx[b * SAMP_NS + slice] = bi; }
    if (LP && !cfg.do_sample) {
        float loc = 0.f;
        if (bv > -INFINITY)
            for (int i = i0 + tid; i < i1; i += SAMP_T) {
                const float s = proc_score(x, i);
                if (s > -INFINITY) loc += expf(s - bv);
            }
        double tot;
        (void)block_excl_scan<SAMP_T>((double)loc, shd, tot);
        if (tid == 0) sc.slice_sum[b * SAMP_NS + slice] = (float)tot;
    }
    if (want_hist)
        for (int i = tid; i < 2048; i += SAMP_T)
            if (hist[i]) atomicAdd(&sc.hist[(size_t)b * 2048 + i], hist[i]);
}

#define SAMP_FT 1024
#define NUC_BINS 2048
#define NUC_SCALE 35184372088832.0
typedef unsigned long long u64;

struct NucSel {
    uint32_t kmin;
    uint32_t kp;
    int idp;
    uint32_t kmax = 0xffffffffu;
};
__device__ __forceinline__ float unfkey(uint32_t k) { return __uint_as_float((k & 0x80000000u) ? (k & 0x7fffffffu) : ~k); }
__device__ __forceinline__ bool nuc_in(const NucSel& z, uint32_t key, int id) {
    return key > 0x007fffffu  && key >= z.kmin && key <= z.kmax && (key > z.kp || (key == z.kp && id >= z.idp));
}
__device__ __forceinline__ int nuc_bin(uint32_t key, float lo) {
    const int b = (int)((unfkey(key) - lo) * ((float)(NUC_BINS - 1) / 32.0f));
    return min(max(b, 0), NUC_BINS - 1);
}

__device__ __forceinline__ u64 nuc_q(uint32_t key, float smax) { return (u64)((double)expf(unfkey(key) - smax) * NUC_SCALE); }

__device__ __forceinline__ void nuc_pass_a(const SampleCtx& x, float smax, float lo, uint32_t* __restrict__ keys,
                                           uint16_t* __restrict__ bins, unsigned int* cnt, u64* mass, int i0, int i1, int step) {
    for (int i = i0; i < i1; i += step) {
        const float s = proc_score(x, i) + 0.0f;
        const uint32_t key = fkey(s);
        keys[i] = key;
        if (s > -INFINITY) {
            const int d = nuc_bin(key, lo);
            bins[i] = (uint16_t)d;
            atomicAdd(&cnt[d], 1u);
            atomicAdd(&mass[d], nuc_q(key, smax));
        } else bins[i] = 0xffffu;
    }
}


__device__ __forceinline__ int topk_bin(const uint32_t* hist, uint32_t k, uint32_t* wsum, int* sh_b0) {
    const int tid = threadIdx.x, lane = tid & 63, wid = tid >> 6;
    const uint32_t* h = hist + tid * 8;
    uint32_t cnt[8], mine = 0;
#pragma unroll
    for (int j = 0; j < 8; ++j) { cnt[j] = h[j]; mine += cnt[j]; }
    uint32_t suf = mine;
#pragma unroll
    for (int o = 1; o < 64; o <<= 1) {
        uint32_t t = __shfl_down(suf, o, 64);
        if (lane + o < 64) suf += t;
    }
    if (lane == 0) wsum[wid] = suf;
    if (tid == 0) *sh_b0 = 0;
    __syncthreads();
    uint32_t above_waves = 0;
    for (int w = wid + 1; w < SAMP_T / 64; ++w) above_waves += wsum[w];
    const uint32_t above = above_waves + suf - mine;
    if (above < k && above + mine >= k) {
        uint32_t run = above;
        for (int j = 7; j >= 0; --j) {
            run += cnt[j];
            if (run >= k) { *sh_b0 = tid * 8 + j; break; }
        }
    }
    __syncthreads();
    return *sh_b0;
}

__global__ __launch_bounds__(SAMP_T) void sample_collect_kernel(
    const uint16_t* __restrict__ logits0, int V0, const uint32_t* __restrict__ bitmaps, int bm_words,
    const MttsSamplerCfg* __restrict__ cfgs, const LoopState* __restrict__ ls, const SeqState* __restrict__ seqs,
    SampleScratch sc, int full_cap, int single_vocab,
    int single_mask, int single_step, int single_channel) {
    __shared__ uint32_t wsum[SAMP_T / 64];
    __shared__ int sh_b0;
    const int b = blockIdx.y, slice = blockIdx.x, tid = threadIdx.x, lane = tid & 63, wid = tid >> 6;
    SampleCtx x;
    if (!sample_ctx(x, b, 0, logits0, nullptr, V0, 0, 0, bitmaps, bm_words, cfgs, ls, seqs, single_vocab, single_mask,
                    single_step, single_channel, sc.ban, sc.bias_w, sc.bias_t, sc.ext)) return;
    const MttsSamplerCfg cfg = cfgs[x.c];
    if (!cfg.do_sample) return;
    if (!(cfg.top_k > 0 && cfg.top_k < x.V) || cfg.top_k > SAMP_CAND) {
        __shared__ unsigned int a_cnt[2048];
        __shared__ unsigned long long a_mass[2048];
        float smax = sc.slice_val[b * SAMP_NS + (lane & (SAMP_NS - 1))];
        smax = wave_max(smax);
        for (int i = tid; i < 2048; i += SAMP_T) { a_cnt[i] = 0; a_mass[i] = 0; }
        __syncthreads();
        const int per = (x.V + SAMP_NS - 1) / SAMP_NS;
        const int i0 = slice * per, i1 = min(x.V, i0 + per);
        nuc_pass_a(x, smax, smax - 32.0f, (uint32_t*)(sc.full_idx + (size_t)b * full_cap), (uint16_t*)(sc.full_val + (size_t)b * full_cap),
                   a_cnt, a_mass, i0 + tid, i1, SAMP_T);
        __syncthreads();
        for (int i = tid; i < 2048; i += SAMP_T)
            if (a_cnt[i]) { atomicAdd(&sc.nuc_cnt[(size_t)b * 2048 + i], a_cnt[i]); atomicAdd(&sc.nuc_mass[(size_t)b * 2048 + i], a_mass[i]); }
        if (slice == 0 && tid == 0) { sc.cand_n[b] = SAMP_CAND + 1; sc.overflow[b] = 2; }
        return;
    }
    const int b0 = topk_bin(sc.hist + (size_t)b * 2048, (uint32_t)cfg.top_k, wsum, &sh_b0);
    const uint32_t ninf_key = fkey(-INFINITY);
    const int per = (x.V + SAMP_NS - 1) / SAMP_NS;
    const int i0 = slice * per, i1 = min(x.V, i0 + per);
    for (int i = i0 + tid; i < i1; i += SAMP_T) {
        float s = proc_score(x, i);
        uint32_t key = fkey(s);
        if ((int)(key >> 21) >= b0 && key > ninf_key) {
            uint32_t slot = atomicAdd(&sc.cand_n[b], 1u);
            if (slot < SAMP_CAND) { sc.cand_val[(size_t)b * SAMP_CAND + slot] = s; sc.cand_idx[(size_t)b * SAMP_CAND + slot] = i; }
        }
    }
}

__device__ __forceinline__ uint32_t typ_shift_bits(float d, double dc) { return __float_as_uint((float)fabs((double)d - dc)); }

template <int NT>
__device__ __forceinline__ double block_sum_alt(double v, double (*sh)[NT / 64], int it) {
#pragma unroll
    for (int o = 32; o > 0; o >>= 1) v += __shfl_xor(v, o, 64);
    if ((threadIdx.x & 63) == 0) sh[it & 1][threadIdx.x >> 6] = v;
    __syncthreads();
    double s = 0.0;
#pragma unroll
    for (int w = 0; w < NT / 64; ++w) s += sh[it & 1][w];
    return s;
}

template <int NT>
__device__ void typical_cut(const float* __restrict__ cval, float smax, float typ, int& first_keep, int& hi_keep, double* shd) {
    constexpr int TPT = SAMP_CAND / NT;
    __shared__ double alt[2][NT / 64];
    const int tid = threadIdx.x;
    const int mk = hi_keep - first_keep;
    const int perf = (mk + NT - 1) / NT;
    const int a0 = first_keep + tid * perf, a1 = min(hi_keep, a0 + perf);
    float dd[TPT], ee[TPT];
    double loc = 0.0, loc1 = 0.0;
#pragma unroll
    for (int j = 0; j < TPT; ++j) {
        const bool on = j < perf && a0 + j < a1;
        dd[j] = on ? cval[a0 + j] - smax : 0.f;
        ee[j] = on ? expf(dd[j]) : 0.f;
        loc += (double)ee[j];
        loc1 += (double)ee[j] * (double)dd[j];
    }
    double tot, tot1;
    (void)block_excl_scan<NT>(loc, shd, tot);
    (void)block_excl_scan<NT>(loc1, shd, tot1);
    const double dc = tot1 / tot, need = (double)typ * tot;
    uint32_t sb[TPT];
#pragma unroll
    for (int j = 0; j < TPT; ++j) sb[j] = (j < perf && a0 + j < a1) ? typ_shift_bits(dd[j], dc) : 0xffffffffu;
    uint32_t lo = 0u, hi = 0x7f800000u;
    for (int it = 0; lo < hi; ++it) {
        const uint32_t mid = lo + ((hi - lo) >> 1);
        double m = 0.0;
#pragma unroll
        for (int j = 0; j < TPT; ++j) m += sb[j] <= mid ? (double)ee[j] : 0.0;
        if (block_sum_alt<NT>(m, alt, it) >= need) hi = mid; else lo = mid + 1;
    }
    int below = 0, above = 0;
#pragma unroll
    for (int j = 0; j < TPT; ++j)
        if (sb[j] != 0xffffffffu && sb[j] > lo) { if ((double)dd[j] < dc) ++below; else ++above; }
    double nb, na;
    (void)block_excl_scan<NT>((double)below, shd, nb);
    (void)block_excl_scan<NT>((double)above, shd, na);
    first_keep += (int)nb;
    hi_keep -= (int)na;
}

template <int NT, bool FL, bool TY>
__device__ int finish_sample(float* __restrict__ cval, int* __restrict__ cidx, int n, const MttsSamplerCfg& cfg, float smax,
                             uint32_t step, uint32_t b, uint32_t c, uint64_t seed, double* shd, int* sh_i, float* lp,
                             const MttsSamplerFloors& fl, float typ) {
    const int tid = threadIdx.x;
    int P = 1;
    while (P < n) P <<= 1;
    for (int i = n + tid; i < P; i += NT) { cval[i] = INFINITY; cidx[i] = 0x7fffffff; }
    __syncthreads();
    for (int kk = 2; kk <= P; kk <<= 1) {
        for (int j = kk >> 1; j > 0; j >>= 1) {
            for (int t = tid; t < P; t += NT) {
                int ixj = t ^ j;
                if (ixj > t) {
                    bool up = ((t & kk) == 0);
                    float a = cval[t], bb = cval[ixj];
                    int ai = cidx[t], bi2 = cidx[ixj];
                    bool gt = (a > bb) || (a == bb && ai > bi2);
                    if (gt == up) { cval[t] = bb; cval[ixj] = a; cidx[t] = bi2; cidx[ixj] = ai; }
                }
            }
            __syncthreads();
        }
// ... 1128 lines not shown
```

### moss-ttsd_amd/csrc/stepplan.h

```cpp
#pragma once
#include <algorithm>
#include <cstdio>
#include <cstdlib>
#include <string>
#include <vector>

#include "shapes.h"

#define MTTS_FOLD_NORM_DEFAULT 0
struct StepKnobs {
    int small_rows = SMALL_RP;
    int fuse_qkv_max = 2560;
    int pack_min_work = 512;
    int attn_row = 1;
    int pf_mfma_pages = 0;
    int gemm_depth = 1;
    int fold_norm = MTTS_FOLD_NORM_DEFAULT;
    int w_seal = 1;
    int w_seal_head = 1;
    int kv_pack = 1;
    bool use_graphs = true;
};
static inline StepKnobs step_knobs_from_env() {
    StepKnobs k;
    const auto clamp = [](const char* g, int lo, int hi) { return std::min(std::max(atoi(g), lo), hi); };
    if (const char* g = getenv("MTTS_GRAPHS")) k.use_graphs = atoi(g) != 0;
    if (const char* g = getenv("MTTS_FUSE_QKV_MAX")) k.fuse_qkv_max = atoi(g);
    if (const char* g = getenv("MTTS_KV_PACK")) k.kv_pack = atoi(g);
    if (const char* g = getenv("MTTS_KV_PACK_MIN")) k.pack_min_work = atoi(g);
    if (const char* g = getenv("MTTS_PREFILL_MFMA_PAGES")) k.pf_mfma_pages = atoi(g);
    if (const char* g = getenv("MTTS_ATTN_ROW")) k.attn_row = clamp(g, 0, 2);
    if (const char* g = getenv("MTTS_SMALL_ROWS")) k.small_rows = clamp(g, 0, SMALL_RP);
    if (const char* g = getenv("MTTS_GEMM_DEPTH")) k.gemm_depth = atoi(g) != 0;
    if (const char* g = getenv("MTTS_FOLD_NORM")) k.fold_norm = atoi(g) != 0;
    if (const char* g = getenv("MTTS_W_SEAL")) k.w_seal = clamp(g, 0, 2);
    if (const char* g = getenv("MTTS_W_SEAL_HEAD")) k.w_seal_head = atoi(g) != 0;
    return k;
}
static inline int fold_norm_env() { return step_knobs_from_env().fold_norm; }
static inline int gemm_depth_env() { return step_knobs_from_env().gemm_depth; }

enum { GEMM_QKV = 0, GEMM_O = 1, GEMM_GU = 2, GEMM_DOWN = 3, GEMM_HEAD0 = 4, GEMM_HEADS = 5,
       GEMM_GU_SLAB = 6,
       GEMM_KINDS = 7 };
struct StepCaps {
    int G = 1, nkv = 1, L = 0;
    int n_cus = 0;
    bool f32 = false;
    bool small_fits = false;
    bool fold_shape = false;
    int row_lds_limit = 0;
    bool wseal_kind[WSEAL_KINDS] = {false, false, false, false};
    int gemm_form[GEMM_KINDS] = {0, 0, 0, 0, 0, 0, 0};
};

struct StepState {
    int heads = 1;
    int B = 0, R = 0;
    int pages_bound = 0;
    bool lora = false;
    bool forced = false, ch0_sampled = false, scores_on = false;
    bool floors_on = false;
    bool typical_on = false;
    bool bans_on = false;
    bool bias_on = false;
    bool bias_terms = false;
    int topk = 0;
    bool split = false;
    bool wseal_on[WSEAL_KINDS] = {false, false, false, false};
    const char* pack_k_on = nullptr;
    const char* pack_v_on = nullptr;
};

enum StepPath { PATH_F32 = 0, PATH_SMALL = 1, PATH_ROWS = 2 };
enum AttnForm { ATTN_FORM_ROW = 0,
                ATTN_FORM_TWO_PASS_FUSED = 1,
                ATTN_FORM_TWO_PASS_EPILOGUE = 2,
                ATTN_FORM_PREFILL_MFMA = 3 };
struct LayerPlan {
    AttnForm attn;
    bool k_sealed, v_sealed;
    bool operator==(const LayerPlan& o) const { return attn == o.attn && k_sealed == o.k_sealed && v_sealed == o.v_sealed; }
};
struct StepPlan {
    StepPath path = PATH_ROWS;
    int heads = 1, B = 0, R = 0;
    int mb = 1, hmb = 1;
    bool tiled = false;
    bool lora = false, fold = false;
    bool sealed[WSEAL_KINDS] = {false, false, false, false};
    bool head_persistent = false;
    std::vector<LayerPlan> layers;
    bool forced = false, ch0_sampled = false, scores_on = false, floors_on = false, typical_on = false, bans_on = false, bias_on = false, bias_terms = false;
    int topk = 0;
    bool split = false;
    int gemm_form[GEMM_KINDS] = {0, 0, 0, 0, 0, 0, 0};
    bool operator==(const StepPlan& o) const {
        return path == o.path && heads == o.heads && B == o.B && R == o.R && mb == o.mb && hmb == o.hmb && tiled == o.tiled &&
               lora == o.lora && fold == o.fold && std::equal(sealed, sealed + WSEAL_KINDS, o.sealed) &&
               head_persistent == o.head_persistent && layers == o.layers && forced == o.forced && ch0_sampled == o.ch0_sampled &&
               scores_on == o.scores_on && floors_on == o.floors_on && typical_on == o.typical_on && bans_on == o.bans_on && bias_on == o.bias_on && bias_terms == o.bias_terms && topk == o.topk && split == o.split && std::equal(gemm_form, gemm_form + GEMM_KINDS, o.gemm_form);
    }
    bool operator!=(const StepPlan& o) const { return !(*this == o); }
};

static inline bool attn_row_auto(int rows, int nkv, int n_cus) { return n_cus > 0 && rows * nkv >= n_cus; }

static inline StepPlan plan_step(const StepKnobs& k, const StepCaps& c, const StepState& s) {
    StepPlan p;
    const bool decode = s.heads == 1;
    p.heads = s.heads; p.B = s.B; p.R = s.R;
    if (decode) { p.forced = s.forced; p.ch0_sampled = s.ch0_sampled; p.scores_on = s.scores_on; p.floors_on = s.floors_on; p.typical_on = s.typical_on; p.bans_on = s.bans_on; p.bias_on = s.bias_on; p.bias_terms = s.bias_on && s.bias_terms; p.topk = s.topk; p.split = s.split; }
    if (c.f32) { p.path = PATH_F32; return p; }
    const bool small = decode && !s.lora && s.B <= k.small_rows && c.small_fits;
    p.path = small ? PATH_SMALL : PATH_ROWS;
    const int work = s.B * s.pages_bound;
    const bool fused = decode && work <= k.fuse_qkv_max;
    const bool pack = decode && work >= k.pack_min_work;
    const bool row_shape = !small && decode && k.attn_row != 0 && (k.attn_row == 2 || attn_row_auto(s.B, c.nkv, c.n_cus));
    p.layers.resize(c.L);
    for (int n = 0; n < c.L; ++n) {
        LayerPlan& l = p.layers[n];
        l.k_sealed = pack && s.pack_k_on && s.pack_k_on[n];
        l.v_sealed = pack && s.pack_v_on && s.pack_v_on[n];
        const bool row = row_shape && l.k_sealed == l.v_sealed && attn_row_lds_bytes(c.G, l.k_sealed, s.pages_bound) <= c.row_lds_limit;
        l.attn = row ? ATTN_FORM_ROW : fused ? ATTN_FORM_TWO_PASS_FUSED :
                 (!decode && s.pages_bound >= k.pf_mfma_pages) ? ATTN_FORM_PREFILL_MFMA : ATTN_FORM_TWO_PASS_EPILOGUE;
    }
    if (small) return p;
    p.mb = (s.R + 31) / 32;
    p.hmb = s.heads == 2 ? (s.B + 31) / 32 : p.mb;
    p.tiled = !decode;
    p.lora = s.lora;
    const auto sealed = [&](int kind, int tiles) { return !s.lora && tiles == 1 && k.gemm_depth && c.wseal_kind[kind] && s.wseal_on[kind]; };
    p.sealed[WSEAL_GU] = !p.tiled && sealed(WSEAL_GU, p.mb);
    p.sealed[WSEAL_DOWN] = !p.tiled && sealed(WSEAL_DOWN, p.mb);
    p.sealed[WSEAL_HEAD0] = s.heads != 0 && sealed(WSEAL_HEAD0, p.hmb);
    p.sealed[WSEAL_HEADS] = s.heads != 0 && sealed(WSEAL_HEADS, p.hmb);
    p.head_persistent = (p.sealed[WSEAL_HEAD0] || p.sealed[WSEAL_HEADS]) && k.w_seal_head;
    p.fold = k.fold_norm && decode && p.mb == 1 && !s.lora && k.gemm_depth && !s.wseal_on[WSEAL_GU] && c.fold_shape;
    for (int g = 0; g < GEMM_KINDS; ++g) {
        const int tiles = (g == GEMM_HEAD0 || g == GEMM_HEADS) ? p.hmb : p.mb;
        p.gemm_form[g] = tiles == 1 ? c.gemm_form[g] : GEMM_SKINNY;
    }
    return p;
}

static inline std::string describe(const StepPlan& p) {
    static const char* const paths[] = {"f32", "small", "rows"};
    static const char* const forms[] = {"skinny", "depth", "gateup48"};
    static const char* const attn[] = {"row", "two_pass fused", "two_pass epilogue", "prefill mfma"};
    char buf[160];
    snprintf(buf, sizeof(buf), "pass: %s B=%d R=%d heads=%d layers=%d\n", paths[p.path], p.B, p.R, p.heads, (int)p.layers.size());
    std::string out = buf;
    if (p.heads == 1) {
        snprintf(buf, sizeof(buf), "sample:%s%s%s%s%s%s%s topk=%d%s\n", p.ch0_sampled ? " ch0_sampled" : " ch0_greedy", p.scores_on ? " scores" : "",
                 p.floors_on ? " floors" : "", p.typical_on ? " typical" : "", p.bans_on ? " bans" : "", p.bias_terms ? " bias" : p.bias_on ? " rules" : "", p.forced ? " forced" : "", p.topk, p.split ? " split" : "");
        out += buf;
    }
    if (p.path == PATH_F32) return out;
    const auto gemm = [&](const char* name, int g, int tiles, bool sealed, const char* more) {
        std::string s = std::string(name) + ": ";
        if (p.path == PATH_SMALL) s += "small";
        else if (p.tiled && g != GEMM_HEAD0 && g != GEMM_HEADS) s += "tile";
        else {
            if (sealed) s += p.gemm_form[g] == GEMM_SKINNY ? "sealed" : std::string(forms[p.gemm_form[g]]) + " sealed";
            else s += forms[p.gemm_form[g]];
            if (tiles > 1) s += " x" + std::to_string(tiles);
        }
        return s + more + "\n";
    };
    const char* lora = p.lora ? " +lora" : "";
    out += gemm("qkv", GEMM_QKV, p.mb, false, lora);
    for (size_t a = 0; a < p.layers.size();) {
        size_t b = a;
        while (b + 1 < p.layers.size() && p.layers[b + 1] == p.layers[a]) ++b;
        const LayerPlan& l = p.layers[a];
        snprintf(buf, sizeof(buf), "attn[%d..%d]: %s%s\n", (int)a, (int)b, attn[l.attn],
                 l.k_sealed && l.v_sealed ? " sealed" : l.k_sealed ? " k_sealed" : l.v_sealed ? " v_sealed" : "");
        out += buf;
        a = b + 1;
    }
    if (p.fold) out += "o_proj+gate_up: fold\n";
    else {
        out += gemm("o_proj", GEMM_O, p.mb, false, lora);
        out += gemm("gate_up", p.lora ? GEMM_GU_SLAB : GEMM_GU, p.mb, p.sealed[WSEAL_GU], p.lora ? " slab +lora" : "");
    }
    out += gemm("down", GEMM_DOWN, p.mb, p.sealed[WSEAL_DOWN], lora);
    if (p.heads) {
        out += gemm("head0", GEMM_HEAD0, p.hmb, p.sealed[WSEAL_HEAD0], p.sealed[WSEAL_HEAD0] && p.head_persistent ? " persistent" : "");
        out += gemm("heads1_7", GEMM_HEADS, p.hmb, p.sealed[WSEAL_HEADS], p.sealed[WSEAL_HEADS] && p.head_persistent ? " persistent" : "");
    }
    return out;
}
```

### moss-ttsd_amd/mtts/capi.py

```python
from __future__ import annotations

import ctypes as C
import os

_HERE = os.path.dirname(os.path.abspath(__file__))
LIB_PATH = os.path.join(os.path.dirname(_HERE), "lib", "libmtts.so")


class MttsConfig(C.Structure):
    _fields_ = [(n, C.c_int32) for n in (
        "vocab_size", "hidden_size", "intermediate_size", "num_hidden_layers", "num_attention_heads",
        "num_key_value_heads", "head_dim", "channels", "speech_vocab_size", "speech_pad_token",
        "speech_range_lo", "speech_range_hi", "eos_token_id", "max_position")] + [
        ("rms_norm_eps", C.c_float), ("max_batch", C.c_int32), ("max_seq_len", C.c_int32), ("kv_pool_pages", C.c_int32), ("dtype", C.c_int32)]


class MttsSamplerCfg(C.Structure):
    _fields_ = [("do_sample", C.c_int32), ("top_k", C.c_int32), ("top_p", C.c_float),
                ("one_minus_top_p", C.c_float), ("temperature", C.c_float), ("repetition_penalty", C.c_float)]


class MttsSamplerFloors(C.Structure):
    _fields_ = [("min_p", C.c_float), ("epsilon_cutoff", C.c_float), ("eta_cutoff", C.c_float), ("sqrt_eta_cutoff", C.c_float)]

# ... 42 lines not shown
    "mtts_engine_create": (C.c_int32, [C.POINTER(MttsConfig), C.c_int32, C.POINTER(C.c_void_p)]),
    "mtts_engine_destroy": (C.c_int32, [C.c_void_p]),
    "mtts_bind_weight": (C.c_int32, [C.c_void_p, C.c_char_p, C.c_void_p, C.c_int64, C.c_int64, C.c_void_p]),
    "mtts_bind_weight_lora": (C.c_int32, [C.c_void_p, C.c_char_p, C.c_void_p, C.c_int64, C.c_int64, C.c_void_p, C.c_void_p,
                                          C.c_int32, C.c_float, C.c_void_p]),
    "mtts_k_lora_pack": (C.c_int32, [C.c_void_p, C.c_int32, C.c_int32, C.c_void_p, C.c_void_p, C.c_int32, C.c_float,
                                     C.c_int32, C.c_int32, C.c_int32, C.c_int32, C.c_void_p, C.c_void_p]),
    "mtts_adapter_load": (C.c_int32, [C.c_void_p, C.c_int32, C.c_char_p, C.c_void_p, C.c_void_p, C.c_int64, C.c_int64, C.c_int32,
                                      C.c_float, C.c_void_p]),
    "mtts_adapter_clear": (C.c_int32, [C.c_void_p, C.c_int32]),
    "mtts_set_row_adapters": (C.c_int32, [C.c_void_p, C.c_void_p, C.c_int32]),
    "mtts_set_slot_adapter": (C.c_int32, [C.c_void_p, C.c_int32, C.c_int32]),
    "mtts_k_lora_delta": (C.c_int32, [C.c_void_p, C.c_int32, C.c_int32, C.c_int32, C.c_int32, C.c_void_p, C.c_int32] +
                          [C.c_void_p] * 6 + [C.c_int32, C.c_void_p]),
    "mtts_k_swiglu_slabs": (C.c_int32, [C.c_void_p] * 5 + [C.c_int32] * 3 + [C.c_void_p]),
    "mtts_bind_rope": (C.c_int32, [C.c_void_p, C.c_void_p, C.c_void_p, C.c_int32, C.c_void_p]),
    "mtts_weights_ready": (C.c_int32, [C.c_void_p]),
    "mtts_generate": (C.c_int32, [C.c_void_p, C.c_void_p, C.c_void_p, C.c_int32, C.c_int32, C.c_int32,
                                  C.POINTER(MttsSamplerCfg), C.c_uint64, C.c_void_p, C.c_int32,
                                  C.POINTER(C.c_int32), C.c_void_p, C.c_int32, C.c_void_p, C.c_void_p]),
    "mtts_begin": (C.c_int32, [C.c_void_p, C.c_void_p, C.c_void_p, C.c_int32, C.c_int32, C.c_int32,
                               C.POINTER(MttsSamplerCfg), C.c_uint64, C.c_void_p]),
    "mtts_step": (C.c_int32, [C.c_void_p, C.c_int32, C.c_void_p]),
    "mtts_step_begin": (C.c_int32, [C.c_void_p, C.c_void_p, C.c_void_p, C.c_void_p]),
    "mtts_step_sample": (C.c_int32, [C.c_void_p, C.c_void_p, C.c_void_p]),
    "mtts_step_finish": (C.c_int32, [C.c_void_p, C.c_void_p, C.c_void_p]),
    "mtts_k_scores_materialize": (C.c_int32, [C.c_void_p, C.c_int32, C.c_int32, C.c_void_p, C.POINTER(MttsSamplerCfg), C.c_int32,
                                              C.c_int32, C.c_int32, C.c_void_p, C.c_void_p, C.c_void_p, C.c_void_p, C.c_void_p]),
    "mtts_sync_state": (C.c_int32, [C.c_void_p, C.POINTER(C.c_int32), C.POINTER(C.c_int32), C.c_void_p]),
    "mtts_read_generated": (C.c_int32, [C.c_void_p, C.c_void_p, C.c_int32, C.POINTER(C.c_int32)]),
    "mtts_set_output_scores": (C.c_int32, [C.c_void_p, C.c_int32]),
    "mtts_read_scores": (C.c_int32, [C.c_void_p, C.c_void_p, C.c_int32, C.POINTER(C.c_int32)]),
    "mtts_slot_read_scores": (C.c_int32, [C.c_void_p, C.c_int32, C.c_void_p, C.c_int32, C.POINTER(C.c_int32)]),
    "mtts_set_top_logprobs": (C.c_int32, [C.c_void_p, C.c_int32]),
    "mtts_read_top_logprobs": (C.c_int32, [C.c_void_p, C.c_void_p, C.c_void_p, C.c_void_p, C.c_int32, C.POINTER(C.c_int32)]),
    "mtts_slot_read_top_logprobs": (C.c_int32, [C.c_void_p, C.c_int32, C.c_void_p, C.c_void_p, C.c_void_p, C.c_int32,
                                                C.POINTER(C.c_int32)]),
    "mtts_k_gen_topk": (C.c_int32, [C.c_void_p, C.c_int32, C.c_int32, C.c_int32, C.c_int32, C.c_void_p, C.c_int32, C.c_void_p,
                                    C.c_void_p, C.c_void_p, C.c_void_p]),
    "mtts_score": (C.c_int32, [C.c_void_p, C.c_void_p, C.c_void_p, C.c_void_p, C.c_int32, C.c_int32, C.c_void_p, C.c_void_p]),
    "mtts_score_topk": (C.c_int32, [C.c_void_p, C.c_void_p, C.c_void_p, C.c_void_p, C.c_int32, C.c_int32, C.c_void_p, C.c_int32,
                                    C.c_void_p, C.c_void_p, C.c_void_p]),
    "mtts_read_logits": (C.c_int32, [C.c_void_p, C.c_void_p, C.c_void_p, C.c_void_p]),
    "mtts_read_logits_f32": (C.c_int32, [C.c_void_p, C.c_void_p, C.c_void_p, C.c_void_p]),
    "mtts_sched_open": (C.c_int32, [C.c_void_p, C.c_int32, C.c_int32, C.POINTER(MttsSamplerCfg), C.c_void_p]),
    "mtts_slot_submit": (C.c_int32, [C.c_void_p, C.c_int32, C.c_void_p, C.c_int32, C.c_int32, C.c_uint64, C.c_void_p]),
    "mtts_slot_submit_row": (C.c_int32, [C.c_void_p, C.c_int32, C.c_void_p, C.c_int32, C.c_int32, C.c_uint64, C.c_int32, C.c_void_p]),
    "mtts_set_row_ids": (C.c_int32, [C.c_void_p, C.c_void_p, C.c_int32]),
    "mtts_set_takes": (C.c_int32, [C.c_void_p, C.c_int32]),
    "mtts_set_sampler_floors": (C.c_int32, [C.c_void_p, C.POINTER(MttsSamplerFloors)]),
    "mtts_set_sampler_bans": (C.c_int32, [C.c_void_p, C.POINTER(MttsSamplerBans)]),
    "mtts_set_sampler_typical": (C.c_int32, [C.c_void_p, C.POINTER(C.c_float)]),
    "mtts_debug_ban_launches": (C.c_int64, []),
    "mtts_set_sampler_bias": (C.c_int32, [C.c_void_p, C.POINTER(MttsSamplerBias)]),
    "mtts_debug_bias_launches": (C.c_int64, []),
    "mtts_slot_fork": (C.c_int32, [C.c_void_p, C.c_int32, C.c_int32, C.c_uint64, C.c_int32, C.c_void_p]),
    "mtts_slot_states": (C.c_int32, [C.c_void_p, C.c_void_p, C.c_void_p]),
    "mtts_slot_read": (C.c_int32, [C.c_void_p, C.c_int32, C.c_void_p, C.c_int32, C.POINTER(C.c_int32)]),
    "mtts_read_seq_state": (C.c_int32, [C.c_void_p, C.c_void_p, C.c_void_p, C.c_void_p, C.c_void_p]),
    "mtts_slot_evict": (C.c_int32, [C.c_void_p, C.c_int32, C.c_void_p]),
    "mtts_kv_pool_state": (C.c_int32, [C.c_void_p, C.POINTER(C.c_int32), C.POINTER(C.c_int32), C.POINTER(C.c_int32)]),
    "mtts_read_page_table": (C.c_int32, [C.c_void_p, C.c_void_p, C.c_void_p]),
    "mtts_set_forced_mode": (C.c_int32, [C.c_void_p, C.c_int32]),
    "mtts_debug_read_device_page_table": (C.c_int32, [C.c_void_p, C.c_void_p, C.c_void_p]),
    "mtts_export_codes": (C.c_int32, [C.c_void_p, C.c_int32, C.c_int32, C.c_void_p, C.c_void_p]),
    "mtts_profile_enable": (C.c_int32, [C.c_void_p, C.c_int32]),
    "mtts_profile_read": (C.c_int32, [C.c_void_p, C.c_int32, C.POINTER(C.c_double), C.POINTER(C.c_int64),
                                      C.POINTER(C.c_int64)]),
    "mtts_debug_set_kv_len": (C.c_int32, [C.c_void_p, C.c_int32]),
    "mtts_debug_kv_pack_stats": (C.c_int32, [C.c_void_p, C.c_void_p]),
    "mtts_debug_step_plan": (C.c_int32, [C.c_void_p, C.c_int32, C.c_char_p, C.c_int32]),
    "mtts_k_kv_seal": (C.c_int32, [C.c_void_p, C.c_int32, C.c_void_p, C.c_int32, C.c_void_p]),
    "mtts_k_attn_bench": (C.c_int32, [C.c_void_p, C.c_int32, C.c_int32, C.POINTER(C.c_float), C.POINTER(C.c_int64)]),
    "mtts_k_gemm_bench": (C.c_int32, [C.c_int32] * 7 + [C.POINTER(C.c_float)]),
    "mtts_k_gemm_bf16": (C.c_int32, [C.c_void_p, C.c_void_p, C.c_void_p, C.c_int32, C.c_int32, C.c_int32,
                                     C.c_int32, C.c_void_p]),
    "mtts_debug_gemm_depth_launches": (C.c_int64, []),
    "mtts_debug_wseal_launches": (C.c_int64, []),
    "mtts_debug_wseal_stats": (C.c_int32, [C.c_void_p, C.c_void_p]),
    "mtts_k_wseal": (C.c_int32, [C.c_void_p, C.c_int32, C.c_int32, C.c_int32, C.c_void_p, C.c_void_p]),
    "mtts_k_gemm_sealed": (C.c_int32, [C.c_void_p, C.c_void_p, C.c_void_p] + [C.c_int32] * 7 + [C.c_void_p, C.c_void_p]),
    "mtts_k_gemm_sealed_bench": (C.c_int32, [C.c_void_p] + [C.c_int32] * 8 + [C.POINTER(C.c_float), C.c_void_p]),
    "mtts_debug_attn_row_launches": (C.c_int64, []),
    "mtts_debug_fold_norm_launches": (C.c_int64, []),
    "mtts_k_oproj_resid": (C.c_int32, [C.c_void_p] * 4 + [C.c_int32] * 2 + [C.c_void_p]),
    "mtts_k_fold_pair": (C.c_int32, [C.c_void_p] * 5 + [C.c_float] + [C.c_int32] * 2 + [C.c_void_p, C.c_void_p]),
    "mtts_k_bf16_round_check": (C.c_int32, [C.c_void_p, C.c_void_p]),
    "mtts_k_fold_bench": (C.c_int32, [C.c_int32] * 4 + [C.POINTER(C.c_float)]),
    "mtts_k_attn_section": (C.c_int32, [C.c_void_p, C.c_int32] + [C.c_void_p] * 4 + [C.c_float] + [C.c_void_p] * 4 +
                            [C.c_int32] * 6 + [C.c_void_p] * 6),
    "mtts_k_attn_prefill": (C.c_int32, [C.c_void_p, C.c_int32] + [C.c_void_p] * 4 + [C.c_float] + [C.c_void_p] * 5 +
                            [C.c_int32] * 4 + [C.c_void_p] * 5),
    "mtts_k_gemm_swiglu_bf16": (C.c_int32, [C.c_void_p, C.c_void_p, C.c_void_p, C.c_int32, C.c_int32, C.c_int32, C.c_void_p]),
    "mtts_k_rmsnorm": (C.c_int32, [C.c_void_p, C.c_void_p, C.c_void_p, C.c_int32, C.c_int32, C.c_float, C.c_void_p]),
    "mtts_k_embed_norm": (C.c_int32, [C.c_void_p] * 5 + [C.c_int32, C.c_int32, C.c_float] + [C.c_void_p] * 3),
    "mtts_k_resid_norm": (C.c_int32, [C.c_void_p, C.c_int32, C.c_int32] + [C.c_void_p] * 4 + [C.c_int32] * 3 + [C.c_float] +
                          [C.c_void_p] * 3),
    "mtts_k_gemv_small": (C.c_int32, [C.c_int32, C.c_int32, C.c_void_p] + [C.c_int32] * 4 + [C.c_void_p, C.c_void_p, C.c_int32,
                                      C.c_void_p, C.c_float] + [C.c_void_p] * 4 + [C.c_int32, C.c_int32] + [C.c_void_p] * 4),
    "mtts_k_gemm_tile": (C.c_int32, [C.c_int32] + [C.c_void_p] * 3 + [C.c_int32] * 4 + [C.c_void_p]),
    "mtts_k_rope_kvwrite": (C.c_int32, [C.c_void_p] * 6 + [C.c_int32, C.c_int32, C.c_int32, C.c_float] + [C.c_void_p] * 4),
    "mtts_k_paged_attn_decode": (C.c_int32, [C.c_void_p] * 5 + [C.c_int32] * 4 + [C.c_void_p, C.c_void_p]),
    "mtts_k_head_ce": (C.c_int32, [C.c_void_p, C.c_void_p, C.c_void_p] + [C.c_int32] * 5 + [C.c_void_p, C.c_void_p]),
    "mtts_k_head_topk": (C.c_int32, [C.c_void_p, C.c_void_p] + [C.c_int32] * 6 + [C.c_void_p, C.c_void_p, C.c_void_p]),
    "mtts_k_sample": (C.c_int32, [C.c_void_p, C.c_int32, C.c_int32, C.c_void_p, C.POINTER(MttsSamplerCfg),
                                  C.c_int32, C.c_uint64, C.c_int32, C.c_int32, C.c_void_p, C.c_void_p]),
    "mtts_k_sample_scores": (C.c_int32, [C.c_void_p, C.c_int32, C.c_int32, C.c_void_p, C.POINTER(MttsSamplerCfg),
                                         C.c_int32, C.c_uint64, C.c_int32, C.c_int32, C.c_void_p, C.c_void_p, C.c_void_p]),
    "mtts_k_sample_floors": (C.c_int32, [C.c_void_p, C.c_int32, C.c_int32, C.c_void_p, C.POINTER(MttsSamplerCfg),
                                         C.c_int32, C.c_uint64, C.c_int32, C.c_int32, C.c_void_p, C.c_void_p,
                                         C.POINTER(MttsSamplerFloors), C.c_void_p]),
    "mtts_k_sample_bans": (C.c_int32, [C.c_void_p, C.c_int32, C.c_int32, C.c_void_p, C.POINTER(MttsSamplerCfg),
                                       C.c_int32, C.c_uint64, C.c_int32, C.c_int32, C.c_void_p, C.c_void_p,
                                       C.POINTER(MttsSamplerFloors), C.c_void_p, C.c_void_p]),
    "mtts_k_sample_typical": (C.c_int32, [C.c_void_p, C.c_int32, C.c_int32, C.c_void_p, C.POINTER(MttsSamplerCfg),
                                          C.c_int32, C.c_uint64, C.c_int32, C.c_int32, C.c_void_p, C.c_void_p,
                                          C.POINTER(MttsSamplerFloors), C.c_void_p, C.c_float, C.c_void_p]),
    "mtts_k_sample_bias": (C.c_int32, [C.c_void_p, C.c_int32, C.c_int32, C.c_void_p, C.POINTER(MttsSamplerCfg),
                                       C.c_int32, C.c_uint64, C.c_int32, C.c_int32, C.c_void_p, C.c_void_p,
                                       C.POINTER(MttsSamplerFloors), C.c_void_p, C.c_float, C.c_void_p, C.c_void_p, C.c_void_p]),
    "mtts_k_seq_bias": (C.c_int32, [C.c_void_p, C.c_void_p, C.c_int32, C.c_int32, C.POINTER(MttsSamplerBias), C.c_int32,
                                    C.c_void_p, C.c_void_p, C.c_void_p, C.c_void_p]),
    "mtts_k_ngram_ban": (C.c_int32, [C.c_void_p, C.c_void_p, C.c_int32, C.c_int32, C.c_int32, C.c_void_p, C.c_int32, C.c_int32,
                                     C.c_int32, C.c_int32, C.c_void_p, C.c_void_p]),
    "mtts_codec_last_error": (C.c_char_p, []),
    "mtts_codec_create": (C.c_int32, [C.POINTER(MttsCodecConfig), C.c_int32, C.POINTER(C.c_void_p)]),
    "mtts_codec_destroy": (C.c_int32, [C.c_void_p]),
    "mtts_codec_bind": (C.c_int32, [C.c_void_p, C.c_char_p, C.c_void_p, C.c_int64, C.c_void_p]),
    "mtts_codec_detokenize": (C.c_int32, [C.c_void_p, C.c_void_p, C.c_void_p, C.c_int32, C.c_int32, C.c_void_p, C.c_void_p]),
    "mtts_codec_detokenize_async": (C.c_int32, [C.c_void_p, C.c_void_p, C.c_void_p, C.c_int32, C.c_int32, C.c_void_p, C.c_void_p]),
    "mtts_codec_check": (C.c_int32, [C.c_void_p, C.c_void_p]),
    "mtts_codec_tokenize": (C.c_int32, [C.c_void_p, C.c_void_p, C.c_void_p, C.c_int32, C.c_int32, C.c_void_p, C.c_void_p, C.c_void_p]),
    "mtts_k_gemm_f32": (C.c_int32, [C.c_void_p, C.c_void_p, C.c_void_p, C.c_void_p, C.c_int32, C.c_int32, C.c_int32,
                                    C.c_int32, C.c_void_p]),
    "mtts_k_gemm_planes_bench": (C.c_int32, [C.c_int32, C.c_int32, C.c_int32, C.c_int32, C.c_int32, C.c_int32,
                                             C.POINTER(C.c_float), C.POINTER(C.c_int32)]),
    "mtts_k_codec_attn": (C.c_int32, [C.c_void_p] * 3 + [C.c_int32] * 5 + [C.c_void_p]),
    "mtts_k_codec_gemm_planes": (C.c_int32, [C.c_void_p] * 6 + [C.c_int32] * 9 + [C.c_void_p]),
    "mtts_k_codec_vocos_pw": (C.c_int32, [C.c_void_p] * 7 + [C.c_int32, C.c_void_p]),
    "mtts_k_codec_layernorm": (C.c_int32, [C.c_void_p] * 4 + [C.c_int32, C.c_int32, C.c_float, C.c_void_p] + [C.c_int32] * 3 +
                               [C.c_void_p]),
    "mtts_k_codec_layernorm_wide": (C.c_int32, [C.c_void_p] * 4 + [C.c_int32, C.c_int32, C.c_float, C.c_void_p]),
    "mtts_k_codec_dwconv_ln": (C.c_int32, [C.c_void_p] * 6 + [C.c_int32] * 3 + [C.c_float, C.c_int32, C.c_int32, C.c_void_p]),
    "mtts_k_codec_softmax_mask": (C.c_int32, [C.c_void_p, C.c_void_p] + [C.c_int32] * 4 + [C.c_void_p]),
    "mtts_k_codec_vq_argmin_update": (C.c_int32, [C.c_void_p] * 6 + [C.c_int32] * 4 + [C.c_void_p]),
    "mtts_k_codec_gemm_f32_ex": (C.c_int32, [C.c_void_p] * 6 + [C.c_int32] * 4 + [C.c_int64] * 4 + [C.c_int32, C.c_int32, C.c_float,
                                                                                                   C.c_int32, C.c_int32, C.c_void_p,
                                                                                                   C.c_void_p]),
}


def exported_symbols():
    return sorted(_SIGS)


def lib():
    global _lib
    if _lib is None:
        if not os.path.exists(LIB_PATH):
            raise MttsError(f"{LIB_PATH} is missing: build it with `python moss-ttsd_amd/build.py` "
                            "(hipcc --offload-arch=gfx950); there is no CPU fallback")
        L = C.CDLL(LIB_PATH)
        for name, (res, args) in _SIGS.items():
            fn = getattr(L, name)
            fn.restype = res
            fn.argtypes = args
        _lib = L
    return _lib


def check(rc):
    if rc != 0:
        raise MttsError(f"libmtts error {rc}: {lib().mtts_last_error().decode()}", rc)
```

Baseline: 83750 codec_tokens/s.

## Seal KV pages only on page-end steps and vectorize sampler score walk

Decode steps now record in the step plan whether any live row finishes a KV page. Sealing runs through a per-row kernel only on those steps, instead of a scan launch on every step. The plan flag becomes part of graph-cache identity, so two graph variants exist. The sampler's logit walk now reads bf16 scores eight at a time with unrolled wide loads and pulls mask bits in bulk. An f32 sampling entry point and a seal-step counter are also added.

```diff
diff --git a/include/mtts.h b/include/mtts.h
--- a/include/mtts.h
+++ b/include/mtts.h
@@ -189,6 +189,7 @@
 int32_t mtts_k_bf16_round_check(int64_t* out2, void* stream);
 int32_t mtts_k_fold_bench(int32_t N_gu, int32_t copies, int32_t iters, int32_t mode, float* avg_us);
 int64_t mtts_debug_attn_row_launches(void);
+int64_t mtts_debug_kv_seal_launches(void);
 int32_t mtts_k_attn_section(const float* dev_slabs, int32_t ksplit, const void* dev_qnw, const void* dev_knw, const void* dev_cos,
                             const void* dev_sin, float eps, const void* dev_k, const void* dev_v, const int32_t* host_lens,
                             const int32_t* host_page_table, int32_t R, int32_t Lmax, int32_t nq, int32_t nkv, int32_t sealed,
@@ -241,6 +242,8 @@
                              const void* dev_history_bitmap, const MttsSamplerCfg* cfg,
                              int32_t mask_id, uint64_t seed, int32_t step, int32_t channel,
                              int32_t* dev_tokens, float* dev_logp, void* stream);
+int32_t mtts_k_sample_rows_f32(const float* dev_scores, int32_t rows, int32_t vocab, const MttsSamplerCfg* cfg, uint64_t seed,
+                               int32_t step, int32_t channel, int32_t* dev_tokens, float* dev_logp, void* stream);
 int32_t mtts_k_sample_floors(const void* dev_logits_bf16, int32_t rows, int32_t vocab,
                              const void* dev_history_bitmap, const MttsSamplerCfg* cfg,
                              int32_t mask_id, uint64_t seed, int32_t step, int32_t channel,
diff --git a/moss-ttsd_amd/csrc/attn.hip b/moss-ttsd_amd/csrc/attn.hip
--- a/moss-ttsd_amd/csrc/attn.hip
+++ b/moss-ttsd_amd/csrc/attn.hip
@@ -166,6 +166,25 @@
         seal_count(fit, cnt, layer, wave, lane);
     }
 }
+__global__ __launch_bounds__(128) void kv_seal_row_kernel(const u32x4_t* __restrict__ kcache, const u32x4_t* __restrict__ vcache,
+                                                          u32x4_t* __restrict__ kpack, u32x4_t* __restrict__ vpack,
+                                                          const int32_t* __restrict__ page_table, const RowMeta* __restrict__ meta,
+                                                          int max_pages, int total_pages, size_t raw_layer, size_t pk_layer,
+                                                          unsigned long long* __restrict__ cnt) {
+    __shared__ __attribute__((aligned(16))) uint8_t klds[8192 + 128];
+    __shared__ __attribute__((aligned(16))) uint8_t vlds[8192 + 320];
+    const int kvh = blockIdx.y, layer = blockIdx.z, wave = threadIdx.x >> 6, lane = threadIdx.x & 63;
+    const RowMeta m = meta[blockIdx.x];
+    const int seq = __builtin_amdgcn_readfirstlane(m.seq), pos = __builtin_amdgcn_readfirstlane(m.pos);
+    if (seq < 0 || (pos & 63) != 63) return;
+    const int page = page_table[(size_t)seq * max_pages + (pos >> 6)];
+    const size_t pi = (size_t)kvh * total_pages + page;
+    const bool fit = wave ? seal_lane_v(vcache + layer * raw_layer + pi * (MTTS_PAGE * MTTS_HD / 8) + lane,
+                                        vpack + layer * pk_layer + pi * (MTTS_PKU * 64) + lane, vlds, lane)
+                          : seal_lane_k(kcache + layer * raw_layer + pi * (MTTS_PAGE * MTTS_HD / 8) + lane,
+                                        kpack + layer * pk_layer + pi * (MTTS_PKU * 64) + lane, klds, lane);
+    seal_count(fit, cnt, layer, wave, lane);
+}
 __global__ __launch_bounds__(128) void kv_seal_all_kernel(const u32x4_t* __restrict__ kcache, const u32x4_t* __restrict__ vcache,
                                                           u32x4_t* __restrict__ kpack, u32x4_t* __restrict__ vpack, int total_pages,
                                                           size_t raw_layer, size_t pk_layer, unsigned long long* __restrict__ cnt) {
@@ -218,6 +237,12 @@
     const size_t raw_layer = (size_t)total_pages * nkv * (MTTS_PAGE * MTTS_HD / 8), pk_layer = (size_t)total_pages * nkv * (MTTS_PKU * 64);
     hipLaunchKernelGGL(kv_seal_scan_kernel, dim3((R + 63) / 64, nkv, L), dim3(128), 0, st, (const u32x4_t*)kcache, (const u32x4_t*)vcache,
                        (u32x4_t*)kpack, (u32x4_t*)vpack, page_table, meta, R, max_pages, total_pages, raw_layer, pk_layer, cnt);
+}
+void launch_kv_seal_step(const void* kcache, const void* vcache, void* kpack, void* vpack, const int32_t* page_table,
+                         const RowMeta* meta, int R, int max_pages, int total_pages, int nkv, int L, unsigned long long* cnt, hipStream_t st) {
+    const size_t raw_layer = (size_t)total_pages * nkv * (MTTS_PAGE * MTTS_HD / 8), pk_layer = (size_t)total_pages * nkv * (MTTS_PKU * 64);
+    hipLaunchKernelGGL(kv_seal_row_kernel, dim3(R, nkv, L), dim3(128), 0, st, (const u32x4_t*)kcache, (const u32x4_t*)vcache,
+                       (u32x4_t*)kpack, (u32x4_t*)vpack, page_table, meta, max_pages, total_pages, raw_layer, pk_layer, cnt);
 }
 void launch_kv_seal_all(const void* kcache, const void* vcache, void* kpack, void* vpack, int total_pages, int nkv, int L,
                         unsigned long long* cnt, hipStream_t st) {
diff --git a/moss-ttsd_amd/csrc/engine.h b/moss-ttsd_amd/csrc/engine.h
--- a/moss-ttsd_amd/csrc/engine.h
+++ b/moss-ttsd_amd/csrc/engine.h
@@ -237,11 +237,16 @@
     for (int k = 0; k < WSEAL_KINDS; ++k) s.wseal_on[k] = e->wseal_on[k] != 0;
     if (e->kpack) s.pack_k_on = e->pack_k_on.data();
     if (e->vpack) s.pack_v_on = e->pack_v_on.data();
+    if (heads == 1 && e->kpack)
+        for (int b = 0; b < e->B; ++b)
+            if (e->slot_live[b] && (e->n_real[b] + e->steps_issued + 1) % MTTS_PAGE == 0) s.page_end = true;
     return s;
 }
 static inline StepPlan decode_plan(const MttsEngine* e, int pages_bound, bool split = false) {
     return plan_step(e->knobs, e->caps, step_state(e, 1, round_up(e->B, 32), pages_bound, rows_carry_adapters(e), split));
 }
+
+long long mtts_kv_seal_steps();
 
 static inline KvPack layer_pack(const MttsEngine* e, const StepPlan& plan, int n) {
     const LayerPlan& l = plan.layers[n];
diff --git a/moss-ttsd_amd/csrc/engine.hip b/moss-ttsd_amd/csrc/engine.hip
--- a/moss-ttsd_amd/csrc/engine.hip
+++ b/moss-ttsd_amd/csrc/engine.hip
@@ -1,4 +1,5 @@
 #include "engine.h"
+#include <atomic>
 #include "staging.h"
 
 #define FLUSH_STEPS 7
@@ -638,10 +639,18 @@
     }
     return 0;
 }
-static void seal_completed_pages(MttsEngine* e, const RowMeta* d_meta, int R, hipStream_t st) {
-    if (e->kpack)
+#ifndef MTTS_SEAL_BY_PLAN
+#define MTTS_SEAL_BY_PLAN 1
+#endif
+static void seal_completed_pages(MttsEngine* e, const StepPlan& plan, const RowMeta* d_meta, int R, hipStream_t st) {
+    if (!e->kpack) return;
+    if (plan.heads != 1 || !MTTS_SEAL_BY_PLAN)
         launch_kv_seal_rows(e->kcache, e->vcache, e->kpack, e->vpack, e->d_page_table, d_meta, R, e->max_pages, e->total_pages, e->nkv, e->L, e->d_seal_cnt, st);
-}
+    else if (plan.seal)
+        launch_kv_seal_step(e->kcache, e->vcache, e->kpack, e->vpack, e->d_page_table, d_meta, R, e->max_pages, e->total_pages, e->nkv, e->L, e->d_seal_cnt, st);
+}
+static std::atomic<long long> g_seal_steps{0};
+long long mtts_kv_seal_steps() { return g_seal_steps.load(); }
 
 static int forward_small(MttsEngine* e, const StepPlan& plan, const RowMeta* d_meta, int pages_bound, hipStream_t st, int64_t kv_tokens_hint) {
     const int H = e->H, I = e->I, nq = e->nq, Hp = round_up(H, 32), R = MTTS_MAXR;
@@ -666,7 +675,7 @@
         pd.xrows = (const uint16_t*)e->act_rm;
         launch_gemv_small(EPI_PARTIAL, PRO_ROWS, e->p_d, l.wd, I, Hp, Hp, e->partial2, nullptr, pd, st);
     }
-    seal_completed_pages(e, d_meta, R, st);
+    seal_completed_pages(e, plan, d_meta, R, st);
     SmallPro ph = base;
     ph.x_in = xa; ph.x_out = nullptr; ph.slabs = e->partial2; ph.ksplit = e->p_d.ksplit; ph.norm_w = (const uint16_t*)e->final_norm;
     launch_gemv_small(EPI_BF16, PRO_NORM, e->p_h0, e->head0, H, e->V0_pad, e->V0, nullptr, (uint16_t*)e->logits0, ph, st);
@@ -731,7 +740,7 @@
         const void* nw = lastl ? e->final_norm : e->layers[n + 1].ln_in;
         launch_resid_norm(e->bufs.partial, ks_d + ex, Hp, e->x, nw, e->xn, lastl ? e->hlast : nullptr, d_meta, R, H, eps, st);
     }
-    seal_completed_pages(e, d_meta, R, st);
+    seal_completed_pages(e, plan, d_meta, R, st);
     if (plan.heads) {
         const void* xin = e->xn;
         if (plan.heads == 2) {
@@ -1110,8 +1119,7 @@
     return forward_rows(e, plan, e->d_cur, e->d_meta, pages_bound, st, kvtok);
 }
 
-static int step_graph(MttsEngine* e, int pages, hipGraphExec_t* out) {
-    StepPlan plan = decode_plan(e, pages);
+static int step_graph(MttsEngine* e, StepPlan plan, int pages, hipGraphExec_t* out) {
     if (const hipGraphExec_t* hit = e->graphs.find(plan, pages, e->bufs)) {
         *out = *hit;
         return MTTS_OK;
@@ -1153,15 +1161,21 @@
         TRY(step_pages(e, st, &pages_bound));
         if (e->knobs.use_graphs && !e->prof) {
             hipGraphExec_t exec = nullptr;
-            TRY(step_graph(e, std::min(round_up(pages_bound, ATT_PB), e->max_pages), &exec));
+            const int pages = std::min(round_up(pages_bound, ATT_PB), e->max_pages);
+            StepPlan plan = decode_plan(e, pages);
+            const bool seal = plan.seal;
+            TRY(step_graph(e, std::move(plan), pages, &exec));
             HIPCHK(hipGraphLaunch(exec, st));
+            if (seal) g_seal_steps++;
         } else {
             hipEvent_t ev = nullptr;
             prof_begin(e, PROF_STEP, st, &ev);
             int64_t kvtok = 0;
             for (int b = 0; b < e->B; ++b) if (e->slot_live[b]) kvtok += e->n_real[b] + e->steps_issued + 1;
-            TRY(step_body(e, decode_plan(e, pages_bound), pages_bound, st, kvtok));
+            const StepPlan plan = decode_plan(e, pages_bound);
+            TRY(step_body(e, plan, pages_bound, st, kvtok));
             prof_end(e, st, ev);
+            if (plan.seal) g_seal_steps++;
         }
         e->steps_issued++;
     }
@@ -1228,7 +1242,9 @@
     TRY(step_pages(e, st, &pages_bound));
     int64_t kvtok = 0;
     for (int b = 0; b < e->B; ++b) if (e->slot_live[b]) kvtok += e->n_real[b] + e->steps_issued + 1;
-    TRY(forward_rows(e, decode_plan(e, pages_bound, true), e->d_cur, e->d_meta, pages_bound, st, kvtok));
+    const StepPlan plan = decode_plan(e, pages_bound, true);
+    TRY(forward_rows(e, plan, e->d_cur, e->d_meta, pages_bound, st, kvtok));
+    if (plan.seal) g_seal_steps++;
     e->steps_issued++;
     e->split_phase = 0;
     return MTTS_OK;
diff --git a/moss-ttsd_amd/csrc/hooks.hip b/moss-ttsd_amd/csrc/hooks.hip
--- a/moss-ttsd_amd/csrc/hooks.hip
+++ b/moss-ttsd_amd/csrc/hooks.hip
@@ -365,7 +365,7 @@
 static int k_sample(const void* logits, int32_t rows, int32_t vocab, const void* bitmap, const MttsSamplerCfg* cfg,
                     int32_t mask_id, uint64_t seed, int32_t step, int32_t channel, int32_t* dev_tokens, float* dev_logp,
                     const MttsSamplerFloors* floors, const void* ban, float typical_p, void* stream, const void* bias_w = nullptr,
-                    const MttsBiasTable* bias_t = nullptr) {
+                    const MttsBiasTable* bias_t = nullptr, int ext = 0) {
     if ((bias_w == nullptr) != (bias_t == nullptr)) return fail(MTTS_EINVAL, "sample: bias words and bias tables come together");
     if (!logits || !cfg || !dev_tokens || rows < 1 || vocab < 1 || channel < 0 || channel > 7) return fail(MTTS_EINVAL, "sample: bad argument");
     hipStream_t st = S(stream);
@@ -405,6 +405,7 @@
     TRY(alloc_scratch(hb, sc, rows, vocab));
     sc.ban = (const uint32_t*)ban;
     sc.bias_w = (const uint32_t*)bias_w; sc.bias_t = bias_t;
+    sc.ext = ext;
     if (dev_logp) {
         TRY(hb.get(&sc.slice_sum, (size_t)rows * SAMP_NS));
         TRY(hb.get(&sc.lp, (size_t)rows * 8));
@@ -440,6 +441,11 @@
                              void* stream) {
     if (!dev_logp) return fail(MTTS_EINVAL, "sample: null dev_logp");
     return k_sample(logits, rows, vocab, bitmap, cfg, mask_id, seed, step, channel, dev_tokens, dev_logp, nullptr, nullptr, 0.f, stream);
+}
+
+int32_t mtts_k_sample_rows_f32(const float* dev_scores, int32_t rows, int32_t vocab, const MttsSamplerCfg* cfg, uint64_t seed,
+                               int32_t step, int32_t channel, int32_t* dev_tokens, float* dev_logp, void* stream) {
+    return k_sample(dev_scores, rows, vocab, nullptr, cfg, -1, seed, step, channel, dev_tokens, dev_logp, nullptr, nullptr, 0.f, stream, nullptr, nullptr, 1);
 }
 
 int32_t mtts_k_sample_floors(const void* logits, int32_t rows, int32_t vocab, const void* bitmap, const MttsSamplerCfg* cfg,
@@ -749,6 +755,7 @@
     return MTTS_OK;
 }
 int64_t mtts_debug_attn_row_launches(void) { return (int64_t)mtts_attn_row_launches(); }
+int64_t mtts_debug_kv_seal_launches(void) { return (int64_t)mtts_kv_seal_steps(); }
 
 int32_t mtts_k_attn_prefill(const float* dev_slabs, int32_t ksplit, const void* dev_qnw, const void* dev_knw, const void* dev_cos,
                             const void* dev_sin, float eps, const void* dev_k, const void* dev_v, const int32_t* host_lens,
diff --git a/moss-ttsd_amd/csrc/launch.h b/moss-ttsd_amd/csrc/launch.h
--- a/moss-ttsd_amd/csrc/launch.h
+++ b/moss-ttsd_amd/csrc/launch.h
@@ -72,6 +72,8 @@
 int attn_row_lds_limit();
 long long mtts_attn_row_launches();
 void launch_kv_seal_rows(const void* kcache, const void* vcache, void* kpack, void* vpack, const int32_t* page_table,
+                         const RowMeta* meta, int R, int max_pages, int total_pages, int nkv, int L, unsigned long long* cnt, hipStream_t st);
+void launch_kv_seal_step(const void* kcache, const void* vcache, void* kpack, void* vpack, const int32_t* page_table,
                          const RowMeta* meta, int R, int max_pages, int total_pages, int nkv, int L, unsigned long long* cnt, hipStream_t st);
 void launch_kv_seal_all(const void* kcache, const void* vcache, void* kpack, void* vpack, int total_pages, int nkv, int L,
                         unsigned long long* cnt, hipStream_t st);
diff --git a/moss-ttsd_amd/csrc/sampler.hip b/moss-ttsd_amd/csrc/sampler.hip
--- a/moss-ttsd_amd/csrc/sampler.hip
+++ b/moss-ttsd_amd/csrc/sampler.hip
@@ -31,14 +31,18 @@
     }
     return (lo < MTTS_BIAS_RULES_MAX && lo < t->n && t->ids[lo] == i) ? t->term[lo] : 0.f;
 }
+__device__ __forceinline__ float proc_value(const SampleCtx& x, int i, float s, bool ban, bool bias, bool pen) {
+    if (i == x.mask_id || ban) return -INFINITY;
+    if (bias) s = s + bias_term(x.bias_t, i);
+    if (pen) s = (s < 0.f) ? s * x.penalty : s / x.penalty;
+    if (x.temp > 0.f) s = s / x.temp;
+    return s;
+}
 __device__ __forceinline__ float proc_score(const SampleCtx& x, int i) {
     if (i == x.mask_id) return -INFINITY;
     if (x.ban && (x.ban[i >> 5] >> (i & 31)) & 1u) return -INFINITY;
-    float s = x.lg.f32 ? ((const float*)x.lg.p)[i] : bf2f(((const uint16_t*)x.lg.p)[i]);
-    if (x.bias_w && (x.bias_w[i >> 5] >> (i & 31)) & 1u) s = s + bias_term(x.bias_t, i);
-    if (x.penalty > 0.f && (x.bm[i >> 5] >> (i & 31)) & 1u) s = (s < 0.f) ? s * x.penalty : s / x.penalty;
-    if (x.temp > 0.f) s = s / x.temp;
-    return s;
+    const float s = x.lg.f32 ? ((const float*)x.lg.p)[i] : bf2f(((const uint16_t*)x.lg.p)[i]);
+    return proc_value(x, i, s, false, x.bias_w && ((x.bias_w[i >> 5] >> (i & 31)) & 1u), x.penalty > 0.f && ((x.bm[i >> 5] >> (i & 31)) & 1u));
 }
 
 #define SAMP_T 256
@@ -76,6 +80,56 @@
     total = tot;
     __syncthreads();
     return base + inc - v;
+}
+
+#ifndef MTTS_SAMPLER_VEC
+#define MTTS_SAMPLER_VEC 1
+#endif
+#define WALK_U 3
+
+__device__ __forceinline__ uint32_t bits8(const uint32_t* __restrict__ w, int i) {
+    const int sh = i & 31;
+    const uint32_t lo = w[i >> 5], hi = sh > 24 ? w[(i >> 5) + 1] : 0u;
+    return (uint32_t)(((((uint64_t)hi) << 32) | lo) >> sh) & 0xffu;
+}
+template <typename F>
+__device__ __forceinline__ void walk_scores(const SampleCtx& x, int i0, int i1, F f) {
+    const int tid = threadIdx.x;
+    if (x.lg.f32 || !MTTS_SAMPLER_VEC) {
+        for (int i = i0 + tid; i < i1; i += SAMP_T) f(i, proc_score(x, i));
+        return;
+    }
+    const uint16_t* __restrict__ p = (const uint16_t*)x.lg.p;
+    const int mis = (int)(((uintptr_t)(p + i0) >> 1) & 7);
+    const int a0 = min(i1, i0 + ((8 - mis) & 7));
+    const int nvec = (i1 - a0) >> 3, a1 = a0 + 8 * nvec;
+    const bool pen = x.penalty > 0.f;
+    for (int v0 = tid; v0 < nvec; v0 += SAMP_T * WALK_U) {
+        u32x4_t w[WALK_U];
+        uint32_t wb[WALK_U], wt[WALK_U], wp[WALK_U];
+#pragma unroll
+        for (int u = 0; u < WALK_U; ++u) {
+            const int v = v0 + u * SAMP_T, i = a0 + 8 * (v < nvec ? v : v0);
+            w[u] = *(const u32x4_t*)(p + i);
+            wb[u] = x.ban ? bits8(x.ban, i) : 0u;
+            wt[u] = x.bias_w ? bits8(x.bias_w, i) : 0u;
+            wp[u] = pen ? bits8(x.bm, i) : 0u;
+        }
+#pragma unroll
+        for (int u = 0; u < WALK_U; ++u) {
+            const int v = v0 + u * SAMP_T, i = a0 + 8 * v;
+            if (v >= nvec) break;
+            const uint32_t ww[4] = {w[u].x, w[u].y, w[u].z, w[u].w};
+#pragma unroll
+            for (int k = 0; k < 8; ++k) {
+                const float s = bf2f((uint16_t)(ww[k >> 1] >> (16 * (k & 1))));
+                f(i + k, proc_value(x, i + k, s, (wb[u] >> k) & 1u, (wt[u] >> k) & 1u, (wp[u] >> k) & 1u));
+            }
+        }
+    }
+    if (tid < a0 - i0) f(i0 + tid, proc_score(x, i0 + tid));
+    const int t = tid - (SAMP_T - 8);
+    if (t >= 0 && a1 + t < i1) f(a1 + t, proc_score(x, a1 + t));
 }
 
 template <bool LP>
@@ -100,11 +154,10 @@
     const int i0 = slice * per, i1 = min(x.V, i0 + per);
     float bv = -INFINITY;
     int bi = 0x7fffffff;
-    for (int i = i0 + tid; i < i1; i += SAMP_T) {
-        float s = proc_score(x, i);
+    walk_scores(x, i0, i1, [&](int i, float s) {
         argmax_merge(bv, bi, s, i);
         if (want_hist) atomicAdd(&hist[fkey(s) >> 21], 1u);
-    }
+    });
     block_argmax(bv, bi, shf, shi);
     if (tid == 0) { sc.slice_val[b * SAMP_NS + slice] = bv; sc.slice_idx[b * SAMP_NS + slice] = bi; }
     if (LP && !cfg.do_sample) {
@@ -224,14 +277,13 @@
     const uint32_t ninf_key = fkey(-INFINITY);
     const int per = (x.V + SAMP_NS - 1) / SAMP_NS;
     const int i0 = slice * per, i1 = min(x.V, i0 + per);
-    for (int i = i0 + tid; i < i1; i += SAMP_T) {
-        float s = proc_score(x, i);
-        uint32_t key = fkey(s);
+    walk_scores(x, i0, i1, [&](int i, float s) {
+        const uint32_t key = fkey(s);
         if ((int)(key >> 21) >= b0 && key > ninf_key) {
-            uint32_t slot = atomicAdd(&sc.cand_n[b], 1u);
+            const uint32_t slot = atomicAdd(&sc.cand_n[b], 1u);
             if (slot < SAMP_CAND) { sc.cand_val[(size_t)b * SAMP_CAND + slot] = s; sc.cand_idx[(size_t)b * SAMP_CAND + slot] = i; }
         }
-    }
+    });
 }
 
 __device__ __forceinline__ uint32_t typ_shift_bits(float d, double dc) { return __float_as_uint((float)fabs((double)d - dc)); }
diff --git a/moss-ttsd_amd/csrc/stepplan.h b/moss-ttsd_amd/csrc/stepplan.h
--- a/moss-ttsd_amd/csrc/stepplan.h
+++ b/moss-ttsd_amd/csrc/stepplan.h
@@ -67,6 +67,7 @@
     bool bias_terms = false;
     int topk = 0;
     bool split = false;
+    bool page_end = false;
     bool wseal_on[WSEAL_KINDS] = {false, false, false, false};
     const char* pack_k_on = nullptr;
     const char* pack_v_on = nullptr;
@@ -94,12 +95,13 @@
     bool forced = false, ch0_sampled = false, scores_on = false, floors_on = false, typical_on = false, bans_on = false, bias_on = false, bias_terms = false;
     int topk = 0;
     bool split = false;
+    bool seal = false;
     int gemm_form[GEMM_KINDS] = {0, 0, 0, 0, 0, 0, 0};
     bool operator==(const StepPlan& o) const {
         return path == o.path && heads == o.heads && B == o.B && R == o.R && mb == o.mb && hmb == o.hmb && tiled == o.tiled &&
                lora == o.lora && fold == o.fold && std::equal(sealed, sealed + WSEAL_KINDS, o.sealed) &&
                head_persistent == o.head_persistent && layers == o.layers && forced == o.forced && ch0_sampled == o.ch0_sampled &&
-               scores_on == o.scores_on && floors_on == o.floors_on && typical_on == o.typical_on && bans_on == o.bans_on && bias_on == o.bias_on && bias_terms == o.bias_terms && topk == o.topk && split == o.split && std::equal(gemm_form, gemm_form + GEMM_KINDS, o.gemm_form);
+               scores_on == o.scores_on && floors_on == o.floors_on && typical_on == o.typical_on && bans_on == o.bans_on && bias_on == o.bias_on && bias_terms == o.bias_terms && topk == o.topk && split == o.split && seal == o.seal && std::equal(gemm_form, gemm_form + GEMM_KINDS, o.gemm_form);
     }
     bool operator!=(const StepPlan& o) const { return !(*this == o); }
 };
@@ -110,7 +112,7 @@
     StepPlan p;
     const bool decode = s.heads == 1;
     p.heads = s.heads; p.B = s.B; p.R = s.R;
-    if (decode) { p.forced = s.forced; p.ch0_sampled = s.ch0_sampled; p.scores_on = s.scores_on; p.floors_on = s.floors_on; p.typical_on = s.typical_on; p.bans_on = s.bans_on; p.bias_on = s.bias_on; p.bias_terms = s.bias_on && s.bias_terms; p.topk = s.topk; p.split = s.split; }
+    if (decode) { p.forced = s.forced; p.ch0_sampled = s.ch0_sampled; p.scores_on = s.scores_on; p.floors_on = s.floors_on; p.typical_on = s.typical_on; p.bans_on = s.bans_on; p.bias_on = s.bias_on; p.bias_terms = s.bias_on && s.bias_terms; p.topk = s.topk; p.split = s.split; p.seal = s.page_end; }
     if (c.f32) { p.path = PATH_F32; return p; }
     const bool small = decode && !s.lora && s.B <= k.small_rows && c.small_fits;
     p.path = small ? PATH_SMALL : PATH_ROWS;
@@ -151,7 +153,8 @@
     static const char* const forms[] = {"skinny", "depth", "gateup48"};
     static const char* const attn[] = {"row", "two_pass fused", "two_pass epilogue", "prefill mfma"};
     char buf[160];
-    snprintf(buf, sizeof(buf), "pass: %s B=%d R=%d heads=%d layers=%d\n", paths[p.path], p.B, p.R, p.heads, (int)p.layers.size());
+    snprintf(buf, sizeof(buf), "pass: %s B=%d R=%d heads=%d layers=%d%s\n", paths[p.path], p.B, p.R, p.heads, (int)p.layers.size(),
+             p.heads == 1 && p.seal ? " seal" : "");
     std::string out = buf;
     if (p.heads == 1) {
         snprintf(buf, sizeof(buf), "sample:%s%s%s%s%s%s%s topk=%d%s\n", p.ch0_sampled ? " ch0_sampled" : " ch0_greedy", p.scores_on ? " scores" : "",
diff --git a/moss-ttsd_amd/mtts/capi.py b/moss-ttsd_amd/mtts/capi.py
--- a/moss-ttsd_amd/mtts/capi.py
+++ b/moss-ttsd_amd/mtts/capi.py
@@ -148,6 +148,7 @@
     "mtts_k_gemm_sealed": (C.c_int32, [C.c_void_p, C.c_void_p, C.c_void_p] + [C.c_int32] * 7 + [C.c_void_p, C.c_void_p]),
     "mtts_k_gemm_sealed_bench": (C.c_int32, [C.c_void_p] + [C.c_int32] * 8 + [C.POINTER(C.c_float), C.c_void_p]),
     "mtts_debug_attn_row_launches": (C.c_int64, []),
+    "mtts_debug_kv_seal_launches": (C.c_int64, []),
     "mtts_debug_fold_norm_launches": (C.c_int64, []),
     "mtts_k_oproj_resid": (C.c_int32, [C.c_void_p] * 4 + [C.c_int32] * 2 + [C.c_void_p]),
     "mtts_k_fold_pair": (C.c_int32, [C.c_void_p] * 5 + [C.c_float] + [C.c_int32] * 2 + [C.c_void_p, C.c_void_p]),
@@ -173,6 +174,8 @@
                                   C.c_int32, C.c_uint64, C.c_int32, C.c_int32, C.c_void_p, C.c_void_p]),
     "mtts_k_sample_scores": (C.c_int32, [C.c_void_p, C.c_int32, C.c_int32, C.c_void_p, C.POINTER(MttsSamplerCfg),
                                          C.c_int32, C.c_uint64, C.c_int32, C.c_int32, C.c_void_p, C.c_void_p, C.c_void_p]),
+    "mtts_k_sample_rows_f32": (C.c_int32, [C.c_void_p, C.c_int32, C.c_int32, C.POINTER(MttsSamplerCfg), C.c_uint64, C.c_int32, C.c_int32,
+                                          C.c_void_p, C.c_void_p, C.c_void_p]),
     "mtts_k_sample_floors": (C.c_int32, [C.c_void_p, C.c_int32, C.c_int32, C.c_void_p, C.POINTER(MttsSamplerCfg),
                                          C.c_int32, C.c_uint64, C.c_int32, C.c_int32, C.c_void_p, C.c_void_p,
                                          C.POINTER(MttsSamplerFloors), C.c_void_p]),
```

Result: no change. 84080 codec_tokens/s (median of 6 runs) (+0.4%).
